# zsc/ARTalk

Hardware: AMD Instinct MI355X
Metric: motion frames/sec (25 fps clips) at batch=32 per GPU (higher is better)
Workload: dtype f32 (operands split into 2 fp16, 3 fp16 MFMA products per fp32 product, fp32 accumulate)

## Files before the change

### artalk_amd/capi.py

```python
from __future__ import annotations

import ctypes as C
import os

from .config import ARTalkConfig

_HERE = os.path.dirname(os.path.abspath(__file__))
LIB_PATH = os.environ.get("ARTALK_LIB") or os.path.join(_HERE, "libartalk_hip.so")

OK, EINVAL, EKEY, EMISSING, EHIP, ESTATE, ECAPACITY, EBUSY = 0, -1, -2, -3, -4, -5, -6, -7
DTYPE_F32, DTYPE_I64 = 0, 1

SYMBOLS = [
    "artalk_create", "artalk_destroy", "artalk_last_error", "artalk_set_tensor", "artalk_finalize_weights",
    "artalk_reserve", "artalk_workspace_bytes", "artalk_weight_bytes", "artalk_infer", "artalk_get_status", "artalk_poll_status", "artalk_last_ticket", "artalk_get_status_of", "artalk_style_encode", "artalk_stream_begin", "artalk_stream_chunk", "artalk_stream_end", "artalk_savgol", "artalk_flame_create", "artalk_flame_verts", "artalk_flame_destroy", "artalk_flame_last_error",
    "artalk_set_profiling", "artalk_get_profile", "artalk_get_kernel_sums", "artalk_set_graphs", "artalk_graph_count", "artalk_set_cu_mask", "artalk_set_audit", "artalk_get_audit", "artalk_calibrate", "artalk_reset_scales", "artalk_get_scales", "artalk_scale_sites", "artalk_get_site_scales", "artalk_set_site_scales", "artalk_set_tap", "artalk_tap_layout", "artalk_set_precision",
    "artalk_op_gemm", "artalk_op_gemm_ex", "artalk_op_gemm_bf16", "artalk_op_gemm_f16s", "artalk_op_pack_split", "artalk_op_gemm_f16s_packed", "artalk_op_release_scratch", "artalk_op_gemm_p8_plan", "artalk_op_create_masked_stream", "artalk_op_destroy_stream", "artalk_op_mfma_f32_peak", "artalk_op_layernorm", "artalk_op_attention", "artalk_op_w2v_front", "artalk_op_resample_mean", "artalk_op_pool_silu",
    "artalk_op_bsq_history",
    "artalk_sessions_reserve", "artalk_session_open", "artalk_session_step", "artalk_session_close", "artalk_session_count",
    "artalk_session_smooth", "artalk_op_savgol_stream", "artalk_op_session_smooth_check",
    "artalk_op_pack_split_ex", "artalk_op_layernorm_ex", "artalk_op_gemm_f16s_packed_ex", "artalk_op_gemm_f16s_ex", "artalk_op_attention_ex", "artalk_op_w2v_front_ex", "artalk_op_pool_silu_ex", "artalk_op_posconv_p8_ex",
    "artalk_op_bsq_history_ex", "artalk_op_ar_bits_next", "artalk_op_vq_embed", "artalk_op_ar_begin", "artalk_op_dec_input", "artalk_op_dec_finish", "artalk_op_enc_input_zero", "artalk_op_style_input", "artalk_op_add_row", "artalk_op_style_finish", "artalk_op_broadcast16", "artalk_op_session_gather", "artalk_op_session_scatter", "artalk_op_absmax",
    "artalk_op_gemm_rows", "artalk_op_layernorm_rows", "artalk_op_attention_rows", "artalk_op_gemm_rows_layout", "artalk_op_rows_dry_run",
    "artalk_op_w2v_front_rows", "artalk_op_pool_silu_rows", "artalk_op_posconv_rows",
    "artalk_op_attention_plan", "artalk_op_attention_rows_cus",
    "artalk_infer_samples", "artalk_set_tail_skip", "artalk_conv_tail_geometry", "artalk_conv_tail_class",
]

(ATTN_F32_64, ATTN_F32_32, ATTN_SHORT, ATTN_F16, ATTN_F16_P8, ATTN_F16_WIDE, ATTN_F16_PP, ATTN_F16_WIDE_AR,
 ATTN_F16_WIDE_AR_P8) = range(9)
ATTN_KERNELS = {
    ATTN_F32_64: "attention_kernel<64>", ATTN_F32_32: "attention_kernel<32>", ATTN_SHORT: "attention_short_kernel",
    ATTN_F16: "attention_f16_kernel<1>", ATTN_F16_P8: "attention_f16_kernel<1,1>", ATTN_F16_WIDE: "attention_f16_wide_kernel",
    ATTN_F16_PP: "attention_f16_pp_kernel", ATTN_F16_WIDE_AR: "attention_f16_wide_ar_kernel<1>",
    ATTN_F16_WIDE_AR_P8: "attention_f16_wide_ar_kernel<1,1,7,128>",
}


class ArtalkConfigStruct(C.Structure):
    _fields_ = [
        ("ar_depth", C.c_int32), ("ar_heads", C.c_int32),
        ("vae_depth", C.c_int32), ("vae_heads", C.c_int32), ("vae_hidden", C.c_int32),
        ("code_dim", C.c_int32), ("motion_dim", C.c_int32),
        ("n_levels", C.c_int32), ("patch_nums", C.c_int32 * 8),
        ("w2v_layers", C.c_int32), ("w2v_hidden", C.c_int32), ("w2v_heads", C.c_int32), ("w2v_ffn", C.c_int32),
        ("w2v_n_conv", C.c_int32), ("w2v_conv_kernel", C.c_int32 * 8), ("w2v_conv_stride", C.c_int32 * 8),
        ("w2v_conv_dim", C.c_int32),
        ("w2v_pos_kernel", C.c_int32), ("w2v_pos_groups", C.c_int32),
        ("w2v_ln_eps", C.c_float),
        ("style_dim", C.c_int32), ("style_heads", C.c_int32), ("style_layers", C.c_int32), ("style_ffn", C.c_int32),
        ("style_len", C.c_int32),
    ]


ROWMAP_IDENTITY = (2 ** 31 - 1, 0, 0)


class GemmRowsArgs(C.Structure):
    _fields_ = [
        ("mode", C.c_int32), ("M", C.c_int32), ("N", C.c_int32), ("K", C.c_int32), ("act", C.c_int32),
        ("A", C.c_void_p), ("lda", C.c_int64), ("a_elems", C.c_int64), ("a_exp", C.c_int32),
        ("W", C.c_void_p), ("ldw", C.c_int64), ("w_elems", C.c_int64),
        ("bias", C.c_void_p), ("bias_elems", C.c_int64),
        ("C", C.c_void_p), ("ldc", C.c_int64), ("c_elems", C.c_int64), ("cmap", C.c_int32 * 3),
        ("gate", C.c_void_p), ("ldg", C.c_int64), ("gate_elems", C.c_int64), ("gmap", C.c_int32 * 3),
        ("R", C.c_void_p), ("ldr", C.c_int64), ("r_elems", C.c_int64),
        ("c_p8", C.c_int32), ("c_exp", C.c_int32),
        ("force_cfg", C.c_int32), ("splitk", C.c_int32),
        ("ngrp", C.c_int32), ("grpW", C.c_int64), ("grpB", C.c_int64), ("grpC", C.c_int64),
        ("status_dev", C.c_void_p),
        ("ln_Y", C.c_void_p), ("ln_ldy", C.c_int64), ("ln_y_elems", C.c_int64),
        ("ln_scale", C.c_void_p), ("ln_shift", C.c_void_p), ("ln_ldm", C.c_int64), ("ln_mod_elems", C.c_int64), ("ln_mmap", C.c_int32 * 3),
        ("ln_eps", C.c_float), ("ln_out_p8", C.c_int32), ("ln_p8_exp", C.c_int32),
        ("used_cfg", C.POINTER(C.c_int32)), ("used_splitk", C.POINTER(C.c_int32)), ("fused_ln", C.POINTER(C.c_int32)),
        ("cus", C.c_int32),
    ]

    def __init__(self, **kw):
        super().__init__()
        self.a_exp = self.c_exp = self.ln_p8_exp = 4
        self.force_cfg, self.splitk, self.ln_eps = -1, 1, 1e-6
        for name in ("cmap", "gmap", "ln_mmap"):
            setattr(self, name, (C.c_int32 * 3)(*ROWMAP_IDENTITY))
        for k, v in kw.items():
            setattr(self, k, (C.c_int32 * 3)(*v) if k in ("cmap", "gmap", "ln_mmap") else v)


def config_struct(cfg: ARTalkConfig) -> ArtalkConfigStruct:
    w = cfg.w2v
    if w.get("feat_extract_norm", "layer") != "layer" or not w.get("do_stable_layer_norm", True) or not w.get("conv_bias", True):
        raise ValueError("only the XLS-R style wav2vec2 (layer-norm conv stack, stable layer norm, conv bias) is supported")
    if len(set(w["conv_dim"])) != 1:
        raise ValueError("conv_dim must be uniform")
    s = ArtalkConfigStruct()
    s.ar_depth, s.ar_heads = cfg.ar_depth, cfg.ar_heads
    s.vae_depth, s.vae_heads, s.vae_hidden = cfg.vae_depth, cfg.vae_heads, cfg.vae_hidden
    s.code_dim, s.motion_dim = cfg.code_dim, cfg.motion_dim
    s.n_levels = len(cfg.patch_nums)
    for i, p in enumerate(cfg.patch_nums):
        s.patch_nums[i] = p
    s.w2v_layers, s.w2v_hidden = w["num_hidden_layers"], w["hidden_size"]
    s.w2v_heads, s.w2v_ffn = w["num_attention_heads"], w["intermediate_size"]
    s.w2v_n_conv = len(w["conv_kernel"])
    for i, (k, st) in enumerate(zip(w["conv_kernel"], w["conv_stride"])):
        s.w2v_conv_kernel[i], s.w2v_conv_stride[i] = k, st
    s.w2v_conv_dim = w["conv_dim"][0]
    s.w2v_pos_kernel, s.w2v_pos_groups = w["num_conv_pos_embeddings"], w["num_conv_pos_embedding_groups"]
    s.w2v_ln_eps = w["layer_norm_eps"]
    s.style_dim, s.style_heads, s.style_layers = cfg.style_dim, cfg.style_heads, cfg.style_layers
    s.style_ffn, s.style_len = cfg.style_ffn, cfg.style_len
    return s


_lib = None


def lib() -> C.CDLL:
    global _lib
    if _lib is not None:
        return _lib
    if not os.path.exists(LIB_PATH):
        raise RuntimeError(
            f"{LIB_PATH} is missing: the HIP extension has not been built "
            "(run `python -c 'import __graft_entry__ as g; g.build()'`). There is no CPU fallback.")
    L = C.CDLL(LIB_PATH)
    vp, i32, i64, f32 = C.c_void_p, C.c_int, C.c_int64, C.c_float
    L.artalk_create.argtypes = [i32, C.POINTER(ArtalkConfigStruct), C.POINTER(vp)]
    L.artalk_create.restype = i32
    L.artalk_destroy.argtypes = [vp]
    L.artalk_destroy.restype = None
    L.artalk_last_error.argtypes = [vp]
    L.artalk_last_error.restype = C.c_char_p
    L.artalk_set_tensor.argtypes = [vp, C.c_char_p, vp, i32, i32, C.POINTER(i64)]
    L.artalk_set_tensor.restype = i32
    L.artalk_finalize_weights.argtypes = [vp]
    L.artalk_finalize_weights.restype = i32
    L.artalk_reserve.argtypes = [vp, i32, i32]
    L.artalk_reserve.restype = i32
    L.artalk_workspace_bytes.argtypes = [vp]
    L.artalk_workspace_bytes.restype = i64
    L.artalk_weight_bytes.argtypes = [vp]
    L.artalk_weight_bytes.restype = i64
    L.artalk_infer.argtypes = [vp, vp, i64, C.POINTER(i64), i32, vp, vp, vp, i64, vp, vp, vp, vp]
    L.artalk_infer.restype = i32
    if hasattr(L, "artalk_infer_samples"):
        L.artalk_infer_samples.argtypes = [vp, vp, i64, C.POINTER(i64), C.POINTER(i64), i32, vp, vp, vp, i64, vp, vp, vp, vp]
        L.artalk_infer_samples.restype = i32
        L.artalk_set_tail_skip.argtypes = [vp, i32]
        L.artalk_set_tail_skip.restype = i32
        pi = C.POINTER(i32)
        L.artalk_conv_tail_geometry.argtypes = [i64, i32, i32, pi, pi, pi, pi, pi, pi]
        L.artalk_conv_tail_geometry.restype = i32
        L.artalk_conv_tail_class.argtypes = [i64, i32]
        L.artalk_conv_tail_class.restype = i64
    L.artalk_get_status.argtypes = [vp, C.POINTER(C.c_int), vp]
    L.artalk_get_status.restype = i32
    L.artalk_poll_status.argtypes = [vp, C.POINTER(C.c_int)]
    L.artalk_poll_status.restype = i32
    L.artalk_last_ticket.argtypes = [vp]
    L.artalk_last_ticket.restype = C.c_longlong
    L.artalk_get_status_of.argtypes = [vp, C.c_longlong, C.POINTER(C.c_int)]
    L.artalk_get_status_of.restype = i32
    L.artalk_style_encode.argtypes = [vp, vp, i32, vp, vp]
    L.artalk_style_encode.restype = i32
    L.artalk_stream_begin.argtypes = [vp, i32, vp, vp, vp]
    L.artalk_stream_begin.restype = i32
    L.artalk_stream_end.argtypes = [vp]
    L.artalk_stream_end.restype = i32
    L.artalk_stream_chunk.argtypes = [vp, vp, i64, vp, i64, vp]
    L.artalk_stream_chunk.restype = i32
    if hasattr(L, "artalk_session_open"):
        L.artalk_sessions_reserve.argtypes = [vp, i32]
        L.artalk_sessions_reserve.restype = i32
        L.artalk_session_open.argtypes = [vp, i32, vp, vp, C.POINTER(i64), vp]
        L.artalk_session_open.restype = i32
        L.artalk_session_step.argtypes = [vp, C.POINTER(i64), i32, vp, i64, vp, i64, vp, vp, vp]
        L.artalk_session_step.restype = i32
        L.artalk_session_close.argtypes = [vp, C.POINTER(i64), i32]
        L.artalk_session_close.restype = i32
        L.artalk_session_count.argtypes = [vp]
        L.artalk_session_count.restype = i32
    if hasattr(L, "artalk_session_smooth"):
        pi32, pu8 = C.POINTER(i32), C.POINTER(C.c_uint8)
        L.artalk_session_smooth.argtypes = [vp, C.POINTER(i64), i32, vp, i64, pi32, pu8, vp, i64, pi32, pi32, vp]
        L.artalk_session_smooth.restype = i32
        L.artalk_op_savgol_stream.argtypes = [vp, vp, i64, pi32, pi32, pu8, vp, i64, i32, vp]
        L.artalk_op_savgol_stream.restype = i32
        L.artalk_op_session_smooth_check.argtypes = [C.POINTER(i64), C.POINTER(i64), pu8, i32, C.POINTER(i64), i32, C.POINTER(i64), i32, i32, i64,
                                                     pi32, pu8, i64, pi32, pi32, C.c_char_p, i32]
        L.artalk_op_session_smooth_check.restype = i32
    L.artalk_flame_create.argtypes = [i32, i32, i32, i32, vp, vp, vp, vp, vp, vp, f32, C.POINTER(vp)]
    L.artalk_flame_create.restype = i32
    L.artalk_flame_verts.argtypes = [vp, vp, vp, i32, vp, vp]
    L.artalk_flame_verts.restype = i32
    L.artalk_flame_destroy.argtypes = [vp]
    L.artalk_flame_destroy.restype = None
    L.artalk_flame_last_error.argtypes = [vp]
    L.artalk_flame_last_error.restype = C.c_char_p
    L.artalk_savgol.argtypes = [vp, vp, vp, i32, vp]
    L.artalk_savgol.restype = i32
    L.artalk_set_profiling.argtypes = [vp, i32]
    L.artalk_set_profiling.restype = i32
    L.artalk_get_profile.argtypes = [vp, C.POINTER(C.c_double), i32]
    L.artalk_get_profile.restype = i32
    if hasattr(L, "artalk_get_kernel_sums"):
        L.artalk_get_kernel_sums.argtypes = [vp, C.POINTER(C.c_double), i32]
        L.artalk_get_kernel_sums.restype = i32
    L.artalk_set_graphs.argtypes = [vp, i32]
    L.artalk_set_graphs.restype = i32
    if hasattr(L, "artalk_graph_count"):
        L.artalk_graph_count.argtypes = [vp, C.POINTER(C.c_longlong)]
        L.artalk_graph_count.restype = i32
    if hasattr(L, "artalk_set_audit"):
        L.artalk_set_audit.argtypes = [vp, i32]
        L.artalk_set_audit.restype = i32
        L.artalk_get_audit.argtypes = [vp, C.c_char_p, i32, C.POINTER(C.c_float), i32]
        L.artalk_get_audit.restype = i32
    if hasattr(L, "artalk_calibrate"):
        L.artalk_calibrate.argtypes = [vp, f32]
        L.artalk_calibrate.restype = i32
        L.artalk_reset_scales.argtypes = [vp]
        L.artalk_reset_scales.restype = i32
        L.artalk_get_scales.argtypes = [vp, C.POINTER(C.c_int), i32]
        L.artalk_get_scales.restype = i32
    if hasattr(L, "artalk_set_site_scales"):
        L.artalk_scale_sites.argtypes = [vp, C.c_char_p, i32]
        L.artalk_scale_sites.restype = i32
        L.artalk_get_site_scales.argtypes = [vp, C.POINTER(C.c_int), i32]
        L.artalk_get_site_scales.restype = i32
        L.artalk_set_site_scales.argtypes = [vp, C.POINTER(C.c_int), i32]
        L.artalk_set_site_scales.restype = i32
    L.artalk_op_gemm.argtypes = [vp, i64, vp, vp, vp, vp, vp, i32, i32, i32, i32, vp]
    L.artalk_op_gemm.restype = i32
    L.artalk_set_precision.argtypes = [vp, i32]
    L.artalk_set_precision.restype = i32
    if hasattr(L, "artalk_op_gemm_bf16"):
        L.artalk_op_gemm_bf16.argtypes = [vp, i64, vp, vp, vp, vp, vp, i32, i32, i32, i32, i32, vp]
        L.artalk_op_gemm_bf16.restype = i32
    L.artalk_op_gemm_f16s.argtypes = [vp, i64, vp, vp, vp, i32, i32, i32, i32, i32, vp]
    L.artalk_op_gemm_f16s.restype = i32
    L.artalk_op_pack_split.argtypes = [vp, vp, i64, i32, vp]
    L.artalk_op_pack_split.restype = i32
    L.artalk_op_gemm_f16s_packed.argtypes = [vp, i32, i64, vp, vp, vp, i32, i32, i32, i32, i32, vp]
    L.artalk_op_gemm_f16s_packed.restype = i32
    if hasattr(L, "artalk_set_tap"):
        L.artalk_set_tap.argtypes = [vp, vp, i32, i32]
        L.artalk_set_tap.restype = i32
        L.artalk_tap_layout.argtypes = [C.POINTER(C.c_int64), i32]
        L.artalk_tap_layout.restype = i32
        L.artalk_op_release_scratch.argtypes = []
        L.artalk_op_release_scratch.restype = i32
    L.artalk_set_cu_mask.argtypes = [vp, vp, i32]
    L.artalk_set_cu_mask.restype = i32
    L.artalk_op_create_masked_stream.argtypes = [vp, i32, C.POINTER(vp)]
    L.artalk_op_create_masked_stream.restype = i32
    L.artalk_op_destroy_stream.argtypes = [vp]
    L.artalk_op_destroy_stream.restype = i32
    L.artalk_op_gemm_p8_plan.argtypes = [i32, i32, i32, i32]
    L.artalk_op_gemm_p8_plan.restype = i32
    L.artalk_op_gemm_ex.argtypes = [vp, i64, vp, vp, vp, i32, i32, i32, i32, i32, vp]
    L.artalk_op_gemm_ex.restype = i32
    L.artalk_op_mfma_f32_peak.argtypes = [vp, i32, i32, i32, C.POINTER(C.c_double), vp]
    L.artalk_op_mfma_f32_peak.restype = i32
    L.artalk_op_layernorm.argtypes = [vp, vp, vp, vp, vp, vp, i32, i32, f32, i32, vp]
    L.artalk_op_layernorm.restype = i32
    L.artalk_op_attention.argtypes = [vp, vp, vp, vp, i32, i32, i32, i32, i32, f32, i32, vp, i32, vp]
    L.artalk_op_attention.restype = i32
    L.artalk_op_w2v_front.argtypes = [vp, i32, i32, vp, vp, vp, vp, vp, vp, vp]
    L.artalk_op_w2v_front.restype = i32
    L.artalk_op_resample_mean.argtypes = [vp, i32, i32, vp, i32, i32, i32, vp, i32, vp]
    L.artalk_op_resample_mean.restype = i32
    L.artalk_op_pool_silu.argtypes = [vp, i32, i32, i32, vp, vp]
    L.artalk_op_pool_silu.restype = i32
    L.artalk_op_bsq_history.argtypes = [vp, vp, vp, vp, i32, vp]
    L.artalk_op_bsq_history.restype = i32
    if hasattr(L, "artalk_op_pack_split_ex"):
        L.artalk_op_pack_split_ex.argtypes = [vp, vp, i64, i32, i32, vp, vp]
        L.artalk_op_pack_split_ex.restype = i32
        L.artalk_op_layernorm_ex.argtypes = [vp, vp, vp, vp, vp, vp, i32, i32, f32, i32, i32, i32, i32, vp, vp]
        L.artalk_op_layernorm_ex.restype = i32
        L.artalk_op_gemm_f16s_packed_ex.argtypes = [vp, i32, i64, vp, vp, vp, i32, i32, i32, i32, i32, i32, i32, vp, vp, vp]
        L.artalk_op_gemm_f16s_packed_ex.restype = i32
        L.artalk_op_gemm_f16s_ex.argtypes = [vp, i64, vp, vp, vp, i32, i32, i32, i32, i32, i32, vp, vp]
        L.artalk_op_gemm_f16s_ex.restype = i32
        L.artalk_op_attention_ex.argtypes = [vp, vp, vp, vp, i32, i32, i32, i32, i32, f32, i32, vp, i32, i32, i32, i32, vp, vp]
        L.artalk_op_attention_ex.restype = i32
        L.artalk_op_w2v_front_ex.argtypes = [vp, i32, i32, vp, vp, vp, vp, vp, vp, i32, i32, vp, vp]
        L.artalk_op_w2v_front_ex.restype = i32
        L.artalk_op_pool_silu_ex.argtypes = [vp, i32, i32, i32, vp, i32, i32, vp, vp]
        L.artalk_op_pool_silu_ex.restype = i32
        L.artalk_op_posconv_p8_ex.argtypes = [vp, vp, vp, vp, vp, i32, i32, i32, i32, i32, vp, vp]
        L.artalk_op_posconv_p8_ex.restype = i32
    if hasattr(L, "artalk_op_ar_bits_next"):
        for name, args in (
                ("bsq_history_ex", [vp, vp, vp, vp, i32, vp, vp]),
                ("ar_bits_next", [vp, vp, vp, vp, i32, i32, vp, vp]),
                ("vq_embed", [vp, i32, vp, vp, vp, vp, i32, i32, vp, vp, i32, vp]),
                ("ar_begin", [vp, vp, vp, vp, i32, vp]),
                ("dec_input", [vp, vp, vp, vp, vp, i32, vp]),
                ("dec_finish", [vp, vp, vp, vp, vp, i64, i32, vp, i32, vp, vp]),
                ("enc_input_zero", [vp, vp, vp, vp, i32, vp]),
                ("style_input", [vp, vp, vp, vp, i32, vp]),
                ("add_row", [vp, vp, i32, i32, vp]),
                ("style_finish", [vp, vp, vp, vp, vp, vp, i32, vp, i64, vp]),
                ("broadcast16", [vp, vp, i64, i32, vp]),
                ("session_gather", [vp, vp, vp, vp, i32, i32, i32, i32, vp]),
                ("session_scatter", [vp, vp, vp, vp, i32, i32, i32, i32, i32, vp]),
# ... 60 lines not shown
```

### artalk_amd/csrc/ar_glue.hip

```cpp
#include "common.h"
#include <cmath>
#include <mutex>
#include <set>

namespace artalk {

constexpr int T100 = 100;
constexpr int CD = 32;
constexpr int NLV = 5;
__constant__ int c_pn[NLV];
__constant__ int c_off[NLV + 1];
__constant__ int c_up_i0[4][T100];
__constant__ int c_up_i1[4][T100];
__constant__ float c_up_w1[4][T100];
__constant__ float c_hq;

static const int h_pn[NLV] = {1, 5, 25, 50, 100};

int init_ms_tables() {
    static std::mutex mu;
    static std::set<int> ready;
    int dev = -1;
    if (hipGetDevice(&dev) != hipSuccess) return -1;
    std::lock_guard<std::mutex> lock(mu);
// ... 38 lines not shown
}

__global__ __launch_bounds__(256) void absmax_kernel(const float* __restrict__ buf, int rows, int cols, long ld, int is_p8,
                                                     unsigned int* __restrict__ slot, int junk_period, int junk_from, float inv_scale) {
    float m = 0.f;
    const long groups = (long)rows * (cols / 8);
    for (long i = (long)blockIdx.x * 256 + threadIdx.x; i < groups; i += (long)gridDim.x * 256) {
        const long r = i / (cols / 8), g8 = i - r * (cols / 8);
        if (junk_period && r % junk_period >= junk_from) continue;
        const float* p = buf + r * ld + g8 * 8;
        if (is_p8) {
            const _Float16* h = reinterpret_cast<const _Float16*>(p);
#pragma unroll
            for (int e = 0; e < 8; ++e) {
                const float v = fabsf((float)h[e]) * inv_scale;
                m = (v != v) ? INFINITY : fmaxf(m, v);
            }
        } else {
#pragma unroll
            for (int e = 0; e < 8; ++e) {
                const float v = fabsf(p[e]);
                m = (v != v) ? INFINITY : fmaxf(m, v);
            }
        }
    }
    m = wave_max(m);
    if ((threadIdx.x & 63) == 0) atomicMax(slot, __float_as_uint(m));
}
void launch_absmax(const float* buf, int rows, int cols, long ld, int is_p8, unsigned int* slot, hipStream_t s, int junk_period, int junk_from, int p8_exp) {
    if (rows <= 0 || cols < 8) return;
    const long groups = (long)rows * (cols / 8);
    const long blocks = (groups + 255) / 256;
    ARTALK_LAUNCH(absmax_kernel, dim3((unsigned)(blocks < 1024 ? blocks : 1024)), dim3(256), 0, s, buf, rows, cols, ld, is_p8, slot, junk_period,
                       junk_from, p8_scale_of(-p8_exp));
}

__global__ __launch_bounds__(256) void ar_begin_kernel(const float* __restrict__ style_cond, const float* __restrict__ lvlpos,
                                                       float* __restrict__ x0, float* __restrict__ fhat, int E) {
    const int b = blockIdx.x;
    for (int n = threadIdx.x; n < E; n += 256) x0[(long)b * E + n] = style_cond[(long)b * E + n] + lvlpos[n];
    for (int i = threadIdx.x; i < T100 * CD; i += 256) fhat[(long)b * T100 * CD + i] = 0.f;
}
void launch_ar_begin(const float* style_cond, const float* lvlpos, float* x0, float* fhat, int B, hipStream_t s) {
    ARTALK_LAUNCH(ar_begin_kernel, dim3(B), dim3(256), 0, s, style_cond, lvlpos, x0, fhat, 768);
}

constexpr int BITS_NT = 1024;
__global__ __launch_bounds__(BITS_NT) void ar_bits_kernel(const float* __restrict__ logits, uint8_t* __restrict__ bits,
                                                      float* __restrict__ fhat, float* __restrict__ nextfeat, int p, int* __restrict__ status) {
    __shared__ float hs[T100 * CD];
    __shared__ float fs[T100 * CD];
    const int b = blockIdx.x, tid = threadIdx.x;
    const int pn = c_pn[p], off = c_off[p];
    for (int idx = tid; idx < pn * CD; idx += BITS_NT) {
        const int i = idx / CD, c = idx % CD;
        const float* l = logits + ((long)b * pn + i) * (2 * CD) + 2 * c;
        const int bit = l[1] > l[0];
        if (status && !(isfinite(l[0]) && isfinite(l[1]))) atomicOr(status, 1);
        bits[((long)b * 181 + off + i) * CD + c] = (uint8_t)bit;
        hs[idx] = bit ? c_hq : -c_hq;
    }
    if (p >= NLV - 1) return;
    __syncthreads();
    float* fg = fhat + (long)b * T100 * CD;
    for (int idx = tid; idx < T100 * CD; idx += BITS_NT) {
        const int t = idx / CD, c = idx % CD;
        const float v = fg[idx] + up_lin(hs, p, t, c);
        fg[idx] = v;
        fs[idx] = v;
    }
    __syncthreads();
    const int pn2 = c_pn[p + 1];
    for (int idx = tid; idx < pn2 * CD; idx += BITS_NT)
        nextfeat[(long)b * pn2 * CD + idx] = area_pool(fs, pn2, idx / CD, idx % CD);
}
void launch_ar_bits_next(const float* logits, uint8_t* bits, float* fhat, float* nextfeat, int B, int level, hipStream_t s, int* status) {
    ARTALK_LAUNCH(ar_bits_kernel, dim3(B), dim3(BITS_NT), 0, s, logits, bits, fhat, nextfeat, level, status);
}

constexpr int VQ_TOK = 16;
__global__ __launch_bounds__(256) void vq_embed_kernel(const float* __restrict__ feat, int n, const float* __restrict__ We,
                                                       const float* __restrict__ be, const float* __restrict__ pos,
                                                       float* __restrict__ X, int xrows, int xoff,
                                                       const float* __restrict__ style_cond, const float* __restrict__ pos0, int E) {
    __shared__ float f[VQ_TOK][CD];
    const int i0 = blockIdx.x * VQ_TOK, b = blockIdx.y, tid = threadIdx.x;
    if (blockIdx.x == 0 && style_cond) {
        for (int e = tid; e < E; e += 256) X[((long)b * xrows) * E + e] = style_cond[(long)b * E + e] + pos0[e];
    }
    const int nt = min(VQ_TOK, n - i0);
    for (int idx = tid; idx < VQ_TOK * CD; idx += 256) f[idx / CD][idx % CD] = idx < nt * CD ? feat[((long)b * n + i0) * CD + idx] : 0.f;
    constexpr int EPT = 3;
    float w[EPT][CD], bias[EPT], pv[EPT][VQ_TOK];
#pragma unroll
    for (int k = 0; k < EPT; ++k) {
        const int e = tid + k * 256;
        const bool ok = e < E;
#pragma unroll
        for (int c4 = 0; c4 < CD / 4; ++c4) {
            f32x4 t = {0.f, 0.f, 0.f, 0.f};
            if (ok) t = *reinterpret_cast<const f32x4*>(We + (long)e * CD + 4 * c4);
            w[k][4 * c4] = t[0]; w[k][4 * c4 + 1] = t[1]; w[k][4 * c4 + 2] = t[2]; w[k][4 * c4 + 3] = t[3];
        }
        bias[k] = ok ? be[e] : 0.f;
#pragma unroll
        for (int t = 0; t < VQ_TOK; ++t) pv[k][t] = (ok && t < nt) ? pos[(long)(i0 + t) * E + e] : 0.f;
    }
    __syncthreads();
#pragma unroll
    for (int k = 0; k < EPT; ++k) {
        const int e = tid + k * 256;
        if (e >= E) break;
#pragma unroll
        for (int t0 = 0; t0 < VQ_TOK; t0 += 4) {
            float acc[4] = {0.f, 0.f, 0.f, 0.f};
#pragma unroll
            for (int c = 0; c < CD; ++c)
#pragma unroll
                for (int u = 0; u < 4; ++u) acc[u] = fmaf(w[k][c], f[t0 + u][c], acc[u]);
#pragma unroll
            for (int u = 0; u < 4; ++u)
                if (t0 + u < nt) X[((long)b * xrows + xoff + i0 + t0 + u) * E + e] = (acc[u] + bias[k]) + pv[k][t0 + u];
        }
    }
}
void launch_vq_embed(const float* feat, int n, const float* We, const float* be, const float* pos, float* X, int xrows,
                     int xoff, const float* style_cond, const float* pos0, int B, hipStream_t s) {
    ARTALK_LAUNCH(vq_embed_kernel, dim3((n + VQ_TOK - 1) / VQ_TOK, B), dim3(256), 0, s, feat, n, We, be, pos, X, xrows, xoff,
                       style_cond, pos0, 768);
}

__global__ __launch_bounds__(256) void dec_input_kernel(const float* __restrict__ prev_fdec, const float* __restrict__ fhat,
                                                        const uint8_t* __restrict__ bits, const float* __restrict__ dpos,
                                                        float* __restrict__ X) {
    const int b = blockIdx.x;
    for (int idx = blockIdx.y * 256 + threadIdx.x; idx < 2 * T100 * CD; idx += gridDim.y * 256) {
        const int t = idx / CD, c = idx % CD;
        float v;
        if (t < T100) {
            v = prev_fdec[(long)b * T100 * CD + idx];
        } else {
            const int tt = t - T100;
            const float h = bits[((long)b * 181 + 81 + tt) * CD + c] ? c_hq : -c_hq;
            v = fhat[(long)b * T100 * CD + tt * CD + c] + h;
        }
        X[(long)b * 2 * T100 * CD + idx] = v + dpos[idx];
    }
}
void launch_dec_input(const float* prev_fdec, const float* fhat, const uint8_t* bits, const float* dpos, float* X, int B,
                      hipStream_t s) {
    ARTALK_LAUNCH(dec_input_kernel, dim3(B, 8), dim3(256), 0, s, prev_fdec, fhat, bits, dpos, X);
}

__global__ __launch_bounds__(256) void dec_finish_kernel(const float* __restrict__ dec, const float* __restrict__ mean,
                                                         const float* __restrict__ stdv, const float* __restrict__ epos,
                                                         float* __restrict__ out, long out_bstride, int chunk,
                                                         float* __restrict__ E, int MD, int EK, int* __restrict__ status) {
    const int b = blockIdx.x;
    for (int idx = blockIdx.y * 256 + threadIdx.x; idx < T100 * EK; idx += gridDim.y * 256) {
        const int t = idx / EK, j = idx % EK;
        float e = 0.f;
        if (j < MD) {
            const float d = dec[((long)b * 2 * T100 + T100 + t) * MD + j];
            const float m = d * stdv[j] + mean[j];
            if (status && !isfinite(m)) atomicOr(status, 4);
            out[(long)b * out_bstride + ((long)chunk * T100 + t) * MD + j] = m;
            e = (m - mean[j]) / stdv[j] + epos[t * MD + j];
        }
        E[((long)b * T100 + t) * EK + j] = e;
    }
}
void launch_dec_finish(const float* dec, const float* mean, const float* stdv, const float* epos, float* out,
                       long out_bstride, int chunk, float* E, int B, hipStream_t s, int* status) {
    ARTALK_LAUNCH(dec_finish_kernel, dim3(B, 10), dim3(256), 0, s, dec, mean, stdv, epos, out, out_bstride, chunk, E, 106, 128, status);
}

__global__ __launch_bounds__(256) void enc_input_zero_kernel(const float* __restrict__ mean, const float* __restrict__ stdv,
                                                             const float* __restrict__ epos, float* __restrict__ E, int MD, int EK) {
    const int b = blockIdx.x;
    for (int idx = threadIdx.x; idx < T100 * EK; idx += 256) {
        const int t = idx / EK, j = idx % EK;
        E[((long)b * T100 + t) * EK + j] = (j < MD) ? ((0.f - mean[j]) / stdv[j] + epos[t * MD + j]) : 0.f;
    }
}
__global__ __launch_bounds__(256) void broadcast16_kernel(const uint4* __restrict__ src, uint4* __restrict__ dst, int n16) {
    uint4* d = dst + (long)blockIdx.y * n16;
    for (int i = blockIdx.x * 256 + threadIdx.x; i < n16; i += gridDim.x * 256) d[i] = src[i];
}
void launch_broadcast16(const void* src, void* dst, long bytes, int B, hipStream_t s) {
    if (B <= 0 || bytes <= 0) return;
    const int n16 = (int)(bytes / 16);
    ARTALK_LAUNCH(broadcast16_kernel, dim3((n16 + 255) / 256 < 8 ? (n16 + 255) / 256 : 8, B), dim3(256), 0, s,
                       reinterpret_cast<const uint4*>(src), reinterpret_cast<uint4*>(dst), n16);
}

void launch_enc_input_zero(const float* mean, const float* stdv, const float* epos, float* E, int B, hipStream_t s) {
    ARTALK_LAUNCH(enc_input_zero_kernel, dim3(B), dim3(256), 0, s, mean, stdv, epos, E, 106, 128);
}

__global__ __launch_bounds__(256) void session_gather_kernel(const uint4* const* __restrict__ slots, SessionRows w) {
    const uint4* __restrict__ src = slots[blockIdx.y];
    const long row = blockIdx.y;
    const int p0 = w.s16, f0 = w.s16 + w.p16, n16 = f0 + w.f16;
    for (int i = blockIdx.x * 256 + threadIdx.x; i < n16; i += gridDim.x * 256) {
        const uint4 v = src[i];
        if (i < p0) w.style[row * w.s16 + i] = v;
        else if (i < f0) w.prev_in[row * w.p16 + (i - p0)] = v;
        else w.prev_fdec[row * w.f16 + (i - f0)] = v;
    }
}
__global__ __launch_bounds__(256) void session_scatter_kernel(uint4* const* __restrict__ slots, SessionRows w, int with_style) {
    uint4* __restrict__ dst = slots[blockIdx.y];
    const long row = blockIdx.y;
    const int p0 = w.s16, f0 = w.s16 + w.p16, n16 = f0 + w.f16;
    for (int i = (with_style ? 0 : p0) + blockIdx.x * 256 + threadIdx.x; i < n16; i += gridDim.x * 256) {
        uint4 v;
        if (i < p0) v = w.style[row * w.s16 + i];
        else if (i < f0) v = w.prev_in[row * w.p16 + (i - p0)];
        else v = w.prev_fdec[row * w.f16 + (i - f0)];
        dst[i] = v;
    }
}
static inline unsigned session_pieces(const SessionRows& w) { return (unsigned)((w.s16 + w.p16 + w.f16 + 1023) / 1024); }
void launch_session_gather(const float* const* slots, const SessionRows& w, int n, hipStream_t s) {
    if (n <= 0) return;
    ARTALK_LAUNCH(session_gather_kernel, dim3(session_pieces(w), n), dim3(256), 0, s, reinterpret_cast<const uint4* const*>(slots), w);
}
void launch_session_scatter(float* const* slots, const SessionRows& w, int n, bool with_style, hipStream_t s) {
    if (n <= 0) return;
    ARTALK_LAUNCH(session_scatter_kernel, dim3(session_pieces(w), n), dim3(256), 0, s, reinterpret_cast<uint4* const*>(slots), w,
                  with_style ? 1 : 0);
}

constexpr int BSQ_NT = 1024;
__global__ __launch_bounds__(BSQ_NT) void bsq_history_kernel(const float* __restrict__ enc_out, uint8_t* __restrict__ hist_bits,
                                                          float* __restrict__ prev_fdec, float* __restrict__ msfeat, int* __restrict__ status) {
    __shared__ float resid[T100 * CD];
    __shared__ float fms[T100 * CD];
    __shared__ float qs[T100 * CD];
    __shared__ float hs[T100 * CD];
    const int b = blockIdx.x, tid = threadIdx.x;
    for (int idx = tid; idx < T100 * CD; idx += BSQ_NT) {
        resid[idx] = enc_out[(long)b * T100 * CD + idx];
        if (status && !isfinite(resid[idx])) atomicOr(status, 2);
        fms[idx] = 0.f;
    }
    __syncthreads();
    int msoff = 0;
    for (int p = 0; p < NLV; ++p) {
        const int pn = c_pn[p], off = c_off[p];
        for (int base = 0; base < pn * CD; base += BSQ_NT) {
            const int idx = base + tid;
            const bool ok = idx < pn * CD;
            const int i = ok ? idx / CD : 0, c = idx % CD;
            float x = 0.f;
            if (ok) x = (pn == T100) ? resid[idx] : area_pool(resid, pn, i, c);
            float ss = x * x;
            ss = group_sum<32>(ss);
            const float z = x / fmaxf(sqrtf(ss), 1e-12f);
            const float zhat = (z > 0.f) ? c_hq : -c_hq;
            const float q = z + (zhat - z);
            const int bit = q > 0.f;
            if (ok) {
                qs[idx] = q;
                hs[idx] = bit ? c_hq : -c_hq;
                hist_bits[((long)b * 181 + off + i) * CD + c] = (uint8_t)bit;
            }
        }
        __syncthreads();
        if (p < NLV - 1) {
            for (int idx = tid; idx < T100 * CD; idx += BSQ_NT) {
                const int t = idx / CD, c = idx % CD;
                resid[idx] -= up_lin(qs, p, t, c);
                fms[idx] += up_lin(hs, p, t, c);
            }
            __syncthreads();
            const int pn2 = c_pn[p + 1];
            for (int idx = tid; idx < pn2 * CD; idx += BSQ_NT)
                msfeat[((long)b * 180 + msoff) * CD + idx] = area_pool(fms, pn2, idx / CD, idx % CD);
            msoff += pn2;
        } else {
            for (int idx = tid; idx < T100 * CD; idx += BSQ_NT) prev_fdec[(long)b * T100 * CD + idx] = fms[idx] + hs[idx];
        }
        __syncthreads();
    }
}
void launch_bsq_history(const float* enc_out, uint8_t* hist_bits, float* prev_fdec, float* msfeat, int B, hipStream_t s, int* status) {
    ARTALK_LAUNCH(bsq_history_kernel, dim3(B), dim3(BSQ_NT), 0, s, enc_out, hist_bits, prev_fdec, msfeat, status);
}

__global__ __launch_bounds__(256) void style_input_kernel(const float* __restrict__ motion, const float* __restrict__ mean,
                                                          const float* __restrict__ stdv, float* __restrict__ X, int rows, int MD, int EK) {
    const long n = (long)rows * EK;
    for (long idx = (long)blockIdx.x * 256 + threadIdx.x; idx < n; idx += (long)gridDim.x * 256) {
        const long row = idx / EK; const int j = idx % EK;
        X[idx] = (j < MD) ? (motion[row * MD + j] - mean[j]) / stdv[j] : 0.f;
    }
}
void launch_style_input(const float* motion, const float* mean, const float* stdv, float* X, int B, hipStream_t s) {
    const int rows = B * 50;
    ARTALK_LAUNCH(style_input_kernel, dim3((rows * 128 + 255) / 256), dim3(256), 0, s, motion, mean, stdv, X, rows, 106, 128);
}

__global__ __launch_bounds__(256) void add_row_kernel(float* __restrict__ X, const float* __restrict__ v, long n, int D) {
    for (long idx = (long)blockIdx.x * 256 + threadIdx.x; idx < n; idx += (long)gridDim.x * 256) X[idx] += v[idx % D];
}
// ... 145 lines not shown
```

### artalk_amd/csrc/engine.hip

```cpp
#include "kernels.h"
#include "../../include/artalk_hip.h"

#include <hip/hip_ext.h>
#include <rocprofiler-sdk-roctx/roctx.h>

#include <algorithm>
#include <cmath>
#include <cstdio>
#include <cstdlib>
#include <cstring>
#include <map>
#include <set>
#include <string>
#include <vector>

using namespace artalk;

namespace artalk {
thread_local KernelTimer* g_ktimer = nullptr;
bool ktimer_events(hipEvent_t* e0, hipEvent_t* e1) {
    KernelTimer* t = g_ktimer;
    if (!t) return false;
    while (t->pool.size() < t->used + 2) {
        hipEvent_t e = nullptr;
        if (hipEventCreate(&e) != hipSuccess) return false;
        t->pool.push_back(e);
    }
    *e0 = t->pool[t->used]; *e1 = t->pool[t->used + 1];
    t->recs.emplace_back(t->bucket, t->used);
    t->used += 2;
    return true;
}
}

namespace {
enum { KB_STYLE = 0, KB_CONV = 1, KB_ENC = 2, KB_ADA = 3, KB_AR_MISC = 4, KB_LEVEL0 = 5, KB_VAE_DEC = 10, KB_REENC = 11, KB_OTHER = 12, KB_N = 13 };

thread_local std::string g_create_error;

constexpr int kSamplesPerChunk = 64000;
constexpr int kE = 768;
constexpr int kCond = 1024;
constexpr int kNTok = 181;
constexpr int kMaxLv = 5;

struct Range {
    explicit Range(const char* name) { roctxRangePushA(name); }
    ~Range() { roctxRangePop(); }
    Range(const Range&) = delete;
    Range& operator=(const Range&) = delete;
};

enum SlotKind { SK_DIRECT, SK_PADK, SK_CONV, SK_HOST, SK_IGNORE };

struct Slot {
    std::vector<int64_t> shape;
    int dtype = ARTALK_DTYPE_F32;
    SlotKind kind = SK_DIRECT;
    float* dst = nullptr;
    int64_t pad_to = 0;
    bool set = false;
    std::vector<float> host;
    std::vector<int64_t> host_i64;
    int64_t numel() const { int64_t n = 1; for (auto d : shape) n *= d; return n; }
};

struct W2VLayer { float *qkv_w, *qkv_b, *out_w, *out_b, *ln1w, *ln1b, *ln2w, *ln2b, *ff1_w, *ff1_b, *ff2_w, *ff2_b; };
struct ARLayer { float *qkv_w, *qkv_b, *proj_w, *proj_b, *ffn1_w, *ffn1_b, *ffn2_w, *ffn2_b, *qscale; };
struct VAELayer { float *lnw, *lnb, *qkv_w, *out_w, *out_b, *m1_w, *m1_b, *m2_w, *m2_b; };
struct VAESide { float *in_w, *in_b, *out_w, *out_b; std::vector<VAELayer> layers; };
struct StyleLayer { float *in_w, *in_b, *out_w, *out_b, *l1_w, *l1_b, *l2_w, *l2_b, *n1w, *n1b, *n2w, *n2b; };

struct SiteExps {
    int conv[8]; int fp_ln, posconv_in;
    struct W2V { int ln1, qkv, attn, ln2, ffn; } w2v[64];
    int silu_cond, hist_tok;
    struct AR { int ln1, attn, ln2, ffn; } ar[32];
    struct VAE { int ln, qkv, attn, resid, mlp; } vae[2][16];
    int vae_enc_in, vae_dec_in, vae_dec_head;
    int style_in; struct ST { int h, attn, h1, ffn; } style[8];
    SiteExps() { int* p = reinterpret_cast<int*>(this); for (size_t i = 0; i < sizeof(SiteExps) / sizeof(int); ++i) p[i] = kActExp; }
};

struct Workspace {
    int maxB = 0, maxC = 0, G = 0;
    long* src_off = nullptr; float *xnorm = nullptr, *convA = nullptr, *convB = nullptr;
    float *h0 = nullptr, *h1 = nullptr, *xln = nullptr, *qkv = nullptr, *att = nullptr, *ffn = nullptr;
    float* silu_cond = nullptr;
    float *ada = nullptr, *style_cond = nullptr, *prev_in = nullptr, *prev_in_p8 = nullptr, *cache = nullptr;
    float *x = nullptr, *xmod = nullptr, *attn_out = nullptr, *ffn_h = nullptr, *logits = nullptr;
    float *fhat = nullptr, *nextfeat = nullptr;
    float* splitk = nullptr; int64_t splitk_floats = 0;
    float* splitk_b[4] = {nullptr, nullptr, nullptr, nullptr};
    uint8_t *bits = nullptr, *hist_bits = nullptr, *has_style = nullptr;
    int* status = nullptr;
    float** sess_slots = nullptr;
    float *prev_fdec = nullptr, *msfeat = nullptr, *dec_x = nullptr, *vh = nullptr, *vln = nullptr, *vqkv = nullptr;
    float *vatt = nullptr, *vmlp = nullptr, *dec_out = nullptr, *enc_in = nullptr, *enc_out = nullptr, *motion_chunk = nullptr;
    float *s_in = nullptr, *s_h = nullptr, *s_qkv = nullptr, *s_att = nullptr, *s_ffn = nullptr, *s_tmp = nullptr;
    int64_t bytes = 0;
};

}

constexpr int64_t slot_carry_off(int code_dim) { return kE + (int64_t)kNTok * kE + 100LL * code_dim; }
constexpr int kOpCodeDim = 32, kOpMotionDim = 106;

struct artalk_model {
    artalk_config cfg{};
    int device = 0;
    std::string err;
    bool finalized = false;
    std::map<std::string, Slot> slots;
    std::vector<void*> allocs;
    std::vector<void*> ws_allocs;
    int64_t weight_bytes = 0;
    struct PackRange { const float* base; int64_t n; unsigned int* packed; uint16_t* bf16; };
    std::vector<PackRange> wranges;
    int precision = 0;
    bool have_bf16 = false;
    int splitk_tiles = 192, splitk_target = 384;
    bool audit = false;
    unsigned int* audit_vals = nullptr;
    std::vector<std::string> audit_names;
    std::map<std::string, int> audit_index;
    std::vector<int*> audit_exp;
    SiteExps ex;
    int scales_changed = 0;
    struct Site { std::string name; int* ex; };
    std::vector<Site> sites;
    std::map<const int*, int> site_of;
    bool stream_scales_ended = false;
    struct InitHistory { uint8_t* bits = nullptr; float *fdec = nullptr, *msfeat = nullptr; bool valid = false; } init_hist[3];
    void invalidate_init_hist() { for (auto& ih : init_hist) ih.valid = false; }
    float* tap = nullptr; int tap_B = 0, tap_maxch = 0, tap_chunk = 0;
    std::vector<uint32_t> cu_mask;
    int n_cus = 0;
    int stream_B = 0;
    static constexpr int kSessBlock = 32;
    struct Sessions {
        std::vector<float*> blocks;
        std::vector<int64_t> owner;
        struct Open { int slot = 0; int64_t seen = 0; bool smooth_done = false; };
        std::map<int64_t, Open> open;
        std::set<int64_t> ended_by_scales;
        int64_t next_id = 1;
        void* smooth_tab = nullptr; int64_t smooth_cap = 0;
    } sess;
    int64_t sess_carry_off() const { return slot_carry_off(cfg.code_dim); }
    int64_t sess_slot_floats() const { return sess_carry_off() + (kSavgolCarry * (int64_t)cfg.motion_dim + 3) / 4 * 4; }
    float* sess_slot(int i) const { return sess.blocks[i / kSessBlock] + (int64_t)(i % kSessBlock) * sess_slot_floats(); }
    Workspace* view = nullptr;
    bool sticky_error = false;
    int n_conv = 0; int conv_T[8]{}; int conv_S[8]{};
    int Tw = 0, Ts = 0;
    struct TailGeo { bool partial = false; int tc = 0; int T[8]{}, S[8]{}; } tail_geo[4];
    bool tail_skip = true;
    int ada_n = 0;
    int pn[kMaxLv]{}, off[kMaxLv + 1]{};
    float *conv0_w = nullptr, *conv_b[8]{}, *conv_lnw[8]{}, *conv_lnb[8]{}, *conv_w[8]{};
    float *fp_lnw = nullptr, *fp_lnb = nullptr, *fp_w = nullptr, *fp_b = nullptr;
    float *pos_w = nullptr, *pos_b = nullptr, *enc_lnw = nullptr, *enc_lnb = nullptr;
    std::vector<W2VLayer> w2v;
    float *ada_w = nullptr, *ada_b = nullptr;
    float *ar_qkv_w = nullptr, *ar_qkv_b = nullptr;
    std::vector<ARLayer> ar;
    float *logits_w = nullptr, *logits_b = nullptr, *vq_w = nullptr, *vq_b = nullptr, *sc_w = nullptr, *sc_b = nullptr;
    float *null_style = nullptr, *lvl_pos = nullptr, *prev_lvl_pos = nullptr;
    float *enc_pos = nullptr, *dec_pos = nullptr, *vae_mean = nullptr, *vae_std = nullptr;
    VAESide enc, dec;
    float *st_mean = nullptr, *st_std = nullptr, *st_pe = nullptr, *st_proj_w = nullptr, *st_proj_b = nullptr;
    std::vector<StyleLayer> style;
    Workspace ws;
    int profiling = 0;
    KernelTimer ktimer;
    bool use_graphs = true;
    bool in_graph_body = false;
    bool in_body = false;
    std::vector<hipEvent_t> ev_pool; size_t ev_used = 0;
    std::vector<std::pair<size_t, double>> dom_events;
    std::vector<std::pair<int, size_t>> marks;
    hipStream_t prof_stream = nullptr;
    hipStream_t side_stream[3] = {nullptr, nullptr, nullptr};
    hipEvent_t fork_ev = nullptr, join_ev[3] = {nullptr, nullptr, nullptr};
    int branches = 0;
    hipStream_t own_stream = nullptr;
    struct GraphEntry { hipGraphExec_t exec = nullptr; long long last_use = 0; };
    std::map<long long, GraphEntry> graphs;
    long long graph_clock = 0, graph_captures = 0;
    static constexpr int kStageSlots = 4;
    struct Stage { long* src = nullptr; uint8_t* has = nullptr; float** slots = nullptr; int4* smooth = nullptr; hipEvent_t done = nullptr; bool used = false; };
    Stage stage[kStageSlots];
    int stage_cap_c = 0, stage_cap_b = 0, stage_next = 0;
    static constexpr int kStatusSlots = 4;
    int* h_status = nullptr; hipEvent_t status_ev[kStatusSlots] = {nullptr, nullptr, nullptr, nullptr}; bool status_pending = false;
    long long ticket = 0;
};

namespace {

#define HIPCHK(m, call)                                                                         \
    do {                                                                                        \
        hipError_t e_ = (call);                                                                 \
        if (e_ != hipSuccess) {                                                                 \
            (m)->err = std::string(#call) + ": " + hipGetErrorString(e_);                       \
            return ARTALK_EHIP;                                                                 \
        }                                                                                       \
    } while (0)

int fail(artalk_model* m, int code, const std::string& msg) { m->err = msg; return code; }
struct ProfilingOff {
    artalk_model* m; int saved;
    explicit ProfilingOff(artalk_model* x) : m(x), saved(x->profiling) { m->profiling = 0; }
    ~ProfilingOff() { m->profiling = saved; }
    ProfilingOff(const ProfilingOff&) = delete;
    ProfilingOff& operator=(const ProfilingOff&) = delete;
};

template <typename T>
T* dalloc_in(std::vector<void*>& pool, int64_t n) {
    void* p = nullptr;
    if (n <= 0) n = 1;
    if (hipMalloc(&p, n * sizeof(T)) != hipSuccess) { pool.push_back(nullptr); return nullptr; }
    (void)hipMemset(p, 0, n * sizeof(T));
    pool.push_back(p);
    return reinterpret_cast<T*>(p);
}
template <typename T>
T* dalloc(artalk_model* m, int64_t n) { return dalloc_in<T>(m->allocs, n); }

float* walloc(artalk_model* m, int64_t n) {
    m->weight_bytes += n * 4;
    float* p = dalloc<float>(m, n);
    m->wranges.push_back({p, n, nullptr, nullptr});
    return p;
}

const unsigned int* packed_of(const artalk_model* m, const float* w) {
    for (const auto& r : m->wranges)
        if (r.packed && w >= r.base && w < r.base + r.n) return r.packed + (w - r.base);
    return nullptr;
}

const void* bf16_of(const artalk_model* m, const float* w) {
    for (const auto& r : m->wranges)
        if (r.bf16 && w >= r.base && w < r.base + r.n) return r.bf16 + (w - r.base);
    return nullptr;
}

int ensure_bf16_copy(artalk_model* m) {
    if (m->have_bf16) return ARTALK_OK;
    int64_t total = 0;
    for (const auto& r : m->wranges) total += (r.n + 63) / 64 * 64;
    uint16_t* base = dalloc<uint16_t>(m, total);
    if (!base) return fail(m, ARTALK_EHIP, "hipMalloc failed for the bf16 weight copy");
    HIPCHK(m, hipDeviceSynchronize());
    int64_t off = 0;
    for (auto& r : m->wranges) {
        r.bf16 = base + off;
        launch_pack_bf16(r.base, r.bf16, r.n, nullptr);
        off += (r.n + 63) / 64 * 64;
    }
    HIPCHK(m, hipDeviceSynchronize());
    for (const auto& r : m->wranges) m->weight_bytes += r.n * 2;
    m->have_bf16 = true;
    return ARTALK_OK;
}

void add_slot(artalk_model* m, const std::string& key, std::vector<int64_t> shape, SlotKind kind, float* dst,
              int64_t pad_to = 0, int dtype = ARTALK_DTYPE_F32) {
    Slot s;
    s.shape = std::move(shape); s.kind = kind; s.dst = dst; s.pad_to = pad_to; s.dtype = dtype;
    m->slots[key] = std::move(s);
}

void add_linear(artalk_model* m, const std::string& p, int out_f, int in_f, float*& w, float*& b, bool bias = true) {
    w = walloc(m, (int64_t)out_f * in_f);
    add_slot(m, p + ".weight", {out_f, in_f}, SK_DIRECT, w);
    if (bias) { b = walloc(m, out_f); add_slot(m, p + ".bias", {out_f}, SK_DIRECT, b); } else b = nullptr;
}
void add_vec(artalk_model* m, const std::string& key, int n, float*& v) {
    v = walloc(m, n);
    add_slot(m, key, {n}, SK_DIRECT, v);
}
void add_ln(artalk_model* m, const std::string& p, int n, float*& w, float*& b) {
    add_vec(m, p + ".weight", n, w);
    add_vec(m, p + ".bias", n, b);
// ... 239 lines not shown
    launch_layernorm(a, s);
}

struct ConvPasses { int np = 0; int off[4]{}, n[4]{}, cls[4]{}; const long* perm = nullptr; const long* tab = nullptr; };

void run_wav2vec(artalk_model* m, const float* audio, int c0, int n, float* out_w2v, hipStream_t s, const ConvPasses* tail = nullptr) {
    const artalk_config& c = m->cfg;
    Workspace& w = m->ws;
    const int CD = c.w2v_conv_dim, Hs = c.w2v_hidden;
    const int p8 = m->precision == 1 ? 1 : 0;
    const int AP = p8 ? LF_A_P8 : 0;
    Range r_w2v("artalk.wav2vec2");
    roctxRangePushA("artalk.wav2vec2.conv_stack");
    kbucket(m, KB_CONV);
    launch_audio_normalize(audio, tail ? tail->perm : w.src_off + c0, w.xnorm, n, kSamplesPerChunk, s);
    SiteExps& ex = m->ex;
    ConvPasses one;
    one.np = 1; one.n[0] = n; one.cls[0] = 3;
    const ConvPasses& ps = tail ? *tail : one;
    auto geo_T = [&](int p) { const artalk_model::TailGeo& tg = m->tail_geo[ps.cls[p]]; return ps.cls[p] != 3 && tg.partial ? tg.T : m->conv_T; };
    auto geo_S = [&](int p) { const artalk_model::TailGeo& tg = m->tail_geo[ps.cls[p]]; return ps.cls[p] != 3 && tg.partial ? tg.S : m->conv_S; };
    auto row0 = [&](int p, int i) { long r = 0; for (int q = 0; q < p; ++q) r += (long)ps.n[q] * geo_S(q)[i]; return r; };
    float* src = w.convA; float* dst = w.convB;
    for (int p = 0; p < ps.np; ++p) {
        const int *T = geo_T(p), *S = geo_S(p);
        float* y = src + row0(p, 0) * CD;
        launch_conv0(w.xnorm + (long)ps.off[p] * kSamplesPerChunk, kSamplesPerChunk, m->conv0_w, m->conv_b[0], m->conv_lnw[0], m->conv_lnb[0], y, ps.n[p],
                     T[0], S[0], s, p8, w.status, ex.conv[0]);
        audit(m, y, ps.n[p] * S[0], CD, CD, p8, s, &ex.conv[0], S[0], T[0]);
    }
    for (int i = 1; i < c.w2v_n_conv; ++i) {
        const int M = (int)row0(ps.np, i), plan_M = M == n * m->conv_S[i] ? 0 : n * m->conv_S[i];
        linear(m, src, (long)c.w2v_conv_stride[i] * CD, m->conv_w[i], m->conv_b[i], dst, CD, M, CD, c.w2v_conv_kernel[i] * CD,
               ACT_NONE, nullptr, s, AP, nullptr, ex.conv[i - 1], kActExp, plan_M);
        for (int p = 0; p < ps.np; p += 2) {
            const int *T = geo_T(p), *S = geo_S(p);
            float* y = dst + row0(p, i) * CD;
            const int Mp = ps.n[p] * S[i], Mq = p + 1 < ps.np ? ps.n[p + 1] * geo_S(p + 1)[i] : 0;
            LnArgs a;
            a.plan_M = plan_M;
            a.out_p8 = (p8 && i + 1 < c.w2v_n_conv) ? 1 : 0; a.p8_exp = ex.conv[i]; a.status = a.out_p8 ? w.status : nullptr;
            a.junk_period = S[i]; a.junk_from = T[i];
            if (Mq) { a.junk_row2 = Mp; a.junk_period2 = geo_S(p + 1)[i]; a.junk_from2 = geo_T(p + 1)[i]; }
            a.X = y; a.ldx = CD; a.Y = y; a.ldy = CD; a.w = m->conv_lnw[i]; a.b = m->conv_lnb[i]; a.M = Mp + Mq; a.D = CD; a.eps = 1e-5f; a.act = ACT_GELU_ERF;
            launch_layernorm(a, s);
            if (i + 1 < c.w2v_n_conv) {
                audit(m, y, Mp, CD, CD, p8, s, &ex.conv[i], S[i], T[i]);
                if (Mq) audit(m, y + (long)Mp * CD, Mq, CD, CD, p8, s, &ex.conv[i], a.junk_period2, a.junk_from2);
            }
        }
        std::swap(src, dst);
    }
    if (tail) {
        launch_conv_tail_gather(src, tail->tab, dst, n, m->Tw, m->Ts, CD, s);
        std::swap(src, dst);
    }
    stage_mark(m, s, PB_CONV);
    roctxRangePop();
    Range r_enc("artalk.wav2vec2.encoder");
    kbucket(m, KB_ENC);
    const int M = n * m->Ts;
    const int JP = m->Ts, JF = m->Tw;
    layernorm(src, dst, m->fp_lnw, m->fp_lnb, M, CD, c.w2v_ln_eps, ACT_NONE, s, p8, w.status, JP, JF, ex.fp_ln);
    audit(m, dst, M, CD, CD, p8, s, &ex.fp_ln, JP, JF);
    linear(m, dst, CD, m->fp_w, m->fp_b, w.h0, Hs, M, Hs, CD, ACT_NONE, nullptr, s, AP, nullptr, ex.fp_ln);
    audit(m, w.h0, M, Hs, Hs, false, s, &ex.posconv_in, JP, JF);
    {
        const int cg = Hs / c.w2v_pos_groups;
        GemmArgs g;
        g.A = w.h0; g.lda = Hs; g.W = m->pos_w; g.ldw = (long)cg * c.w2v_pos_kernel; g.bias = m->pos_b; g.C = w.h1; g.ldc = Hs; g.R = w.h0; g.ldr = Hs;
        g.M = M; g.act = ACT_GELU_ERF; g.a_exp = ex.posconv_in;
        if (p8 && cg == 64 && c.w2v_pos_kernel == 128 && c.w2v_pos_groups == 16 && m->Ts <= 256) {
            g.N = Hs; g.K = cg * c.w2v_pos_kernel; g.Wp = packed_of(m, m->pos_w); g.status = w.status;
            launch_posconv_p8(g, n, m->Tw, m->Ts, s);
        } else {
            g.amode = 1; g.pc_T = m->Tw; g.pc_tstride = m->Ts; g.pc_pad = c.w2v_pos_kernel / 2; g.pc_cin = cg;
            g.N = cg; g.K = cg * c.w2v_pos_kernel;
            g.batch = c.w2v_pos_groups; g.sA = cg; g.sW = (long)cg * cg * c.w2v_pos_kernel; g.sBias = cg; g.sC = cg; g.sR = cg;
            gemm(m, g, s);
        }
    }
    float* h = w.h1;
    const int nh = c.w2v_heads, hd = Hs / nh;
    for (int i = 0; i < c.w2v_layers; ++i) {
        const W2VLayer& L = m->w2v[i];
        SiteExps::W2V& E = ex.w2v[i];
        layernorm(h, w.xln, L.ln1w, L.ln1b, M, Hs, c.w2v_ln_eps, ACT_NONE, s, p8, w.status, JP, JF, E.ln1);
        audit(m, w.xln, M, Hs, Hs, p8, s, &E.ln1, JP, JF);
        linear(m, w.xln, Hs, L.qkv_w, L.qkv_b, w.qkv, 3 * Hs, M, 3 * Hs, Hs, ACT_NONE, nullptr, s, AP | (p8 ? LF_C_P8 : 0), nullptr, E.ln1, E.qkv);
        AttnArgs a;
        a.qkv_p8 = p8; a.qkv_exp = E.qkv; a.o_exp = E.attn;
        a.Q = w.qkv; a.K = w.qkv + Hs; a.V = w.qkv + 2 * Hs;
        a.ldq = a.ldk = a.ldv = 3 * Hs; a.q_bstride = a.k_bstride = a.v_bstride = (long)m->Ts * 3 * Hs;
        a.O = w.att; a.ldo = Hs; a.o_bstride = (long)m->Ts * Hs;
        a.B = n; a.H = nh; a.HD = hd; a.Lq = m->Tw; a.Lk = m->Tw; a.scale = 1.0f / std::sqrt((float)hd);
        audit(m, w.qkv, M, 3 * Hs, 3 * Hs, p8, s, &E.qkv, JP, JF);
        a.out_p8 = p8; a.split16 = p8; a.status = p8 ? w.status : nullptr; a.cus = m->n_cus;
        launch_attention(a, s);
        audit(m, w.att, M, Hs, Hs, p8, s, &E.attn, JP, JF);
        linear(m, w.att, Hs, L.out_w, L.out_b, h, Hs, M, Hs, Hs, ACT_NONE, h, s, AP, nullptr, E.attn);
        layernorm(h, w.xln, L.ln2w, L.ln2b, M, Hs, c.w2v_ln_eps, ACT_NONE, s, p8, w.status, JP, JF, E.ln2);
        audit(m, w.xln, M, Hs, Hs, p8, s, &E.ln2, JP, JF);
        linear(m, w.xln, Hs, L.ff1_w, L.ff1_b, w.ffn, c.w2v_ffn, M, c.w2v_ffn, Hs, ACT_GELU_ERF, nullptr, s, AP | (p8 ? LF_C_P8 : 0), nullptr, E.ln2, E.ffn);
        audit(m, w.ffn, M, c.w2v_ffn, c.w2v_ffn, p8, s, &E.ffn, JP, JF);
        linear(m, w.ffn, c.w2v_ffn, L.ff2_w, L.ff2_b, h, Hs, M, Hs, c.w2v_ffn, ACT_NONE, h, s, AP, nullptr, E.ffn);
    }
    layernorm(h, w.xln, m->enc_lnw, m->enc_lnb, M, Hs, c.w2v_ln_eps, ACT_NONE, s);
    if (out_w2v)
        (void)hipMemcpy2DAsync(out_w2v + (long)c0 * m->Tw * Hs, (size_t)m->Tw * Hs * 4, w.xln, (size_t)m->Ts * Hs * 4,
                               (size_t)m->Tw * Hs * 4, n, hipMemcpyDeviceToDevice, s);
    launch_pool_silu(w.xln, m->Ts, m->Tw, w.silu_cond + (long)c0 * kNTok * kCond, n, m->pn, c.n_levels, kCond, s, p8, w.status, ex.silu_cond);
    audit(m, w.silu_cond + (long)c0 * kNTok * kCond, n * kNTok, kCond, kCond, p8, s, &ex.silu_cond);
    stage_mark(m, s, PB_ENC);
}

void run_style(artalk_model* m, const float* style_motion, int B, hipStream_t s, bool encode = true) {
    const artalk_config& c = m->cfg;
    Workspace& w = m->ws;
    const int S = c.style_dim, L = c.style_len, M = B * L;
    Range r_style("artalk.style_encoder");
    kbucket(m, KB_STYLE);
    if (style_motion && encode) {
        launch_style_input(style_motion, m->st_mean, m->st_std, w.s_in, B, s);
        SiteExps& ex = m->ex;
        audit(m, w.s_in, M, 128, 128, false, s, &ex.style_in);
        linear(m, w.s_in, 128, m->st_proj_w, m->st_proj_b, w.s_h, S, M, S, 128, ACT_NONE, nullptr, s, 0, nullptr, ex.style_in);
        launch_add_row(w.s_h, m->st_pe, M, S, s);
        for (int i = 0; i < c.style_layers; ++i) {
            const StyleLayer& Ly = m->style[i];
            SiteExps::ST& E = ex.style[i];
            audit(m, w.s_h, M, S, S, false, s, &E.h);
            linear(m, w.s_h, S, Ly.in_w, Ly.in_b, w.s_qkv, 3 * S, M, 3 * S, S, ACT_NONE, nullptr, s, 0, nullptr, E.h);
            AttnArgs a;
            a.Q = w.s_qkv; a.K = w.s_qkv + S; a.V = w.s_qkv + 2 * S; a.ldq = a.ldk = a.ldv = 3 * S;
            a.q_bstride = a.k_bstride = a.v_bstride = (long)L * 3 * S;
            a.O = w.s_att; a.ldo = S; a.o_bstride = (long)L * S;
            a.B = B; a.H = c.style_heads; a.HD = S / c.style_heads; a.Lq = L; a.Lk = L;
            a.scale = 1.0f / std::sqrt((float)(S / c.style_heads));
            launch_attention(a, s);
            audit(m, w.s_att, M, S, S, false, s, &E.attn);
            linear(m, w.s_att, S, Ly.out_w, Ly.out_b, w.s_tmp, S, M, S, S, ACT_NONE, w.s_h, s, 0, nullptr, E.attn);
            layernorm(w.s_tmp, w.s_h, Ly.n1w, Ly.n1b, M, S, 1e-5f, ACT_NONE, s);
            audit(m, w.s_h, M, S, S, false, s, &E.h1);
            linear(m, w.s_h, S, Ly.l1_w, Ly.l1_b, w.s_ffn, c.style_ffn, M, c.style_ffn, S, ACT_GELU_ERF, nullptr, s, 0, nullptr, E.h1);
            audit(m, w.s_ffn, M, c.style_ffn, c.style_ffn, false, s, &E.ffn);
            linear(m, w.s_ffn, c.style_ffn, Ly.l2_w, Ly.l2_b, w.s_tmp, S, M, S, c.style_ffn, ACT_NONE, w.s_h, s, 0, nullptr, E.ffn);
            layernorm(w.s_tmp, w.s_h, Ly.n2w, Ly.n2b, M, S, 1e-5f, ACT_NONE, s);
        }
    }
    launch_style_finish(w.s_h, m->sc_w, m->sc_b, m->null_style, style_motion ? w.has_style : nullptr, w.style_cond, B, s,
                        style_motion, (long)L * c.motion_dim);
}

void run_vae_stack(artalk_model* m, const VAESide& S, int B, int T, int split, hipStream_t s) {
    const artalk_config& c = m->cfg;
    Workspace& w = m->view ? *m->view : m->ws;
    const int H = c.vae_hidden, M = B * T, F = H * 3 / 2;
    const int p8 = m->precision == 1 ? 1 : 0;
    const int AP = p8 ? LF_A_P8 : 0;
    const int sd = &S == &m->enc ? 0 : 1;
    for (int i = 0; i < c.vae_depth; ++i) {
        const VAELayer& L = S.layers[i];
        SiteExps::VAE& E = m->ex.vae[sd][i];
        layernorm(w.vh, w.vln, L.lnw, L.lnb, M, H, 1e-5f, ACT_NONE, s, p8, w.status, 0, 0, E.ln);
        audit(m, w.vln, M, H, H, p8, s, &E.ln);
        linear(m, w.vln, H, L.qkv_w, nullptr, w.vqkv, 3 * H, M, 3 * H, H, ACT_NONE, nullptr, s, AP | (p8 ? LF_C_P8 : 0), nullptr, E.ln, E.qkv);
        AttnArgs a;
        a.qkv_p8 = p8; a.qkv_exp = E.qkv; a.o_exp = E.attn;
        a.Q = w.vqkv; a.K = w.vqkv + H; a.V = w.vqkv + 2 * H; a.ldq = a.ldk = a.ldv = 3 * H;
        a.q_bstride = a.k_bstride = a.v_bstride = (long)T * 3 * H;
        a.O = w.vatt; a.ldo = H; a.o_bstride = (long)T * H;
        a.B = B; a.H = c.vae_heads; a.HD = H / c.vae_heads; a.Lq = T; a.Lk = T;
        a.scale = 1.0f / std::sqrt((float)H);
        audit(m, w.vqkv, M, 3 * H, 3 * H, p8, s, &E.qkv);
        a.split_q = split; a.split_k = split; a.out_p8 = p8; a.split16 = p8; a.status = p8 ? w.status : nullptr; a.cus = m->n_cus;
        launch_attention(a, s);
        audit(m, w.vatt, M, H, H, p8, s, &E.attn);
        linear(m, w.vatt, H, L.out_w, L.out_b, w.vh, H, M, H, H, ACT_NONE, w.vh, s, AP, p8 ? w.vln : nullptr, E.attn, E.resid);
        audit(m, p8 ? w.vln : w.vh, M, H, H, p8, s, &E.resid);
        linear(m, p8 ? w.vln : w.vh, H, L.m1_w, L.m1_b, w.vmlp, F, M, F, H, ACT_GELU_TANH, nullptr, s, p8 ? (LF_A_P8 | LF_C_P8) : 0, nullptr, E.resid, E.mlp);
        audit(m, w.vmlp, M, F, F, p8, s, &E.mlp);
        linear(m, w.vmlp, F, L.m2_w, L.m2_b, w.vh, H, M, H, F, ACT_NONE, w.vh, s, AP, nullptr, E.mlp);
    }
}

void run_reencode(artalk_model* m, int B, hipStream_t s) {
    const artalk_config& c = m->cfg;
    Workspace& w = m->view ? *m->view : m->ws;
    const int H = c.vae_hidden, T = 100;
    Range r_re("artalk.vae.reencode_bsq");
    kbucket(m, KB_REENC);
    audit(m, w.enc_in, B * T, 128, 128, false, s, &m->ex.vae_enc_in);
    linear(m, w.enc_in, 128, m->enc.in_w, m->enc.in_b, w.vh, H, B * T, H, 128, ACT_LEAKY02, nullptr, s, 0, nullptr, m->ex.vae_enc_in);
    run_vae_stack(m, m->enc, B, T, 0, s);
    linear(m, w.vh, H, m->enc.out_w, m->enc.out_b, w.enc_out, c.code_dim, B * T, c.code_dim, H, ACT_NONE, nullptr, s, LF_EXACT);
    launch_bsq_history(w.enc_out, w.hist_bits, w.prev_fdec, w.msfeat, B, s, w.status);
    launch_vq_embed(w.msfeat, kNTok - 1, m->vq_w, m->vq_b, m->prev_lvl_pos + kE, w.prev_in, kNTok, 1, w.style_cond,
                    m->prev_lvl_pos, B, s);
}

int run_init_history(artalk_model* m, int B, hipStream_t s) {
    const artalk_config& c = m->cfg;
    struct Restore { artalk_model* m; ~Restore() { kbucket(m, KB_OTHER); } } restore{m};
    Workspace& w = m->ws;
    artalk_model::InitHistory& ih = m->init_hist[m->precision];
    const long nb = (long)kNTok * c.code_dim, nf = 100L * c.code_dim * 4, nm = 180L * c.code_dim * 4;
    if (!ih.valid) {
        if (!ih.bits) {
            ih.bits = dalloc<uint8_t>(m, nb); ih.fdec = dalloc<float>(m, nf / 4); ih.msfeat = dalloc<float>(m, nm / 4);
            if (!ih.bits || !ih.fdec || !ih.msfeat) return fail(m, ARTALK_EHIP, "hipMalloc failed for the initial-history cache");
            HIPCHK(m, hipDeviceSynchronize());
        }
        launch_enc_input_zero(m->vae_mean, m->vae_std, m->enc_pos, w.enc_in, 1, s);
        run_reencode(m, 1, s);
        HIPCHK(m, hipMemcpyAsync(ih.bits, w.hist_bits, nb, hipMemcpyDeviceToDevice, s));
        HIPCHK(m, hipMemcpyAsync(ih.fdec, w.prev_fdec, nf, hipMemcpyDeviceToDevice, s));
        HIPCHK(m, hipMemcpyAsync(ih.msfeat, w.msfeat, nm, hipMemcpyDeviceToDevice, s));
        int flags[4] = {0, 0, 0, 0};
        HIPCHK(m, hipMemcpyAsync(flags, w.status, sizeof(int), hipMemcpyDeviceToHost, s));
        HIPCHK(m, hipStreamSynchronize(s));
        ih.valid = flags[0] == 0;
    }
    launch_broadcast16(ih.bits, w.hist_bits, nb, B, s);
    launch_broadcast16(ih.fdec, w.prev_fdec, nf, B, s);
    launch_broadcast16(ih.msfeat, w.msfeat, nm, B, s);
    launch_vq_embed(w.msfeat, kNTok - 1, m->vq_w, m->vq_b, m->prev_lvl_pos + kE, w.prev_in, kNTok, 1, w.style_cond, m->prev_lvl_pos, B, s);
    return ARTALK_OK;
}

void run_chunk_body(artalk_model* m, int B, hipStream_t s, int n_reencode = -1) {
    struct BodyScope { artalk_model* m; BodyScope(artalk_model* x) : m(x) { m->in_body = true; } ~BodyScope() { m->in_body = false; } } scope(m);
    const artalk_config& c = m->cfg;
    Workspace& w = m->view ? *m->view : m->ws;
    const long ldada = m->ada_n;
    const long cache_l = (long)w.maxB * 2 * kNTok * 3 * kE;
    const int p8 = m->precision == 1 ? 1 : 0;
    kbucket(m, KB_AR_MISC);
    tap_copy(m, TAP_PREV_IN, 0, w.prev_in, kNTok, kE, B, s);
    roctxRangePushA("artalk.ar.history_kv");
    SiteExps& ex = m->ex;
    if (p8) launch_pack_split(w.prev_in, reinterpret_cast<unsigned int*>(w.prev_in_p8), (long)B * kNTok * kE, false, s, w.status, ex.hist_tok);
    audit(m, p8 ? w.prev_in_p8 : w.prev_in, B * kNTok, kE, kE, p8, s, &ex.hist_tok);
    {
        GemmArgs g;
        g.A = p8 ? w.prev_in_p8 : w.prev_in; g.a_packed = p8; g.a_exp = ex.hist_tok;
        g.lda = kE; g.W = m->ar_qkv_w + (long)kE * kE; g.ldw = kE; g.bias = m->ar_qkv_b + kE;
        g.C = w.cache + kE; g.ldc = 3 * kE; g.cmap = rowmap(kNTok, 2 * kNTok, 0);
        g.M = B * kNTok; g.N = c.ar_depth * 2 * kE; g.K = kE;
        g.ngrp = 2 * kE; g.grpW = (long)3 * kE * kE; g.grpB = 3 * kE; g.grpC = cache_l;
        g.Wp = packed_of(m, g.W);
        if (p8 && gemm_p8_eligible(g)) {
            gemm(m, g, s);
        } else {
            for (int l = 0; l < c.ar_depth; ++l) {
                const ARLayer& L = m->ar[l];
                GemmArgs q = g;
                q.Wp = nullptr; q.ngrp = 0; q.grpW = q.grpB = q.grpC = 0;
                q.W = L.qkv_w + (long)kE * kE; q.bias = L.qkv_b + kE; q.C = w.cache + l * cache_l + kE; q.N = 2 * kE;
                gemm(m, q, s);
            }
        }
    }
    roctxRangePop();
    launch_ar_begin(w.style_cond, m->lvl_pos, w.x, w.fhat, B, s);
    static const char* const kLevelName[kMaxLv] = {"artalk.ar.scale_step0", "artalk.ar.scale_step1", "artalk.ar.scale_step2",
                                                   "artalk.ar.scale_step3", "artalk.ar.scale_step4"};
    for (int p = 0; p < c.n_levels; ++p) {
        Range r_lv(kLevelName[p]);
        kbucket(m, KB_LEVEL0 + p);
        const int pn = m->pn[p], off = m->off[p], M = B * pn;
        const RowMap amap = rowmap(pn, kNTok, off);
        auto ln_args = [&](int l, int which) {
            LnArgs n;
            n.X = w.x; n.ldx = kE; n.Y = w.xmod; n.ldy = kE; n.ldm = ldada; n.mmap = amap; n.M = M; n.D = kE; n.eps = 1e-6f;
            n.status = p8 ? w.status : nullptr;
            if (l < c.ar_depth) {
                const float* ada = w.ada + (long)l * 6 * kE;
                n.scale = ada + (2 + which) * kE; n.shift = ada + (4 + which) * kE; n.out_p8 = p8;
                n.p8_exp = which == 0 ? ex.ar[l].ln1 : ex.ar[l].ln2;
            } else {
                const float* hada = w.ada + (long)c.ar_depth * 6 * kE;
                n.scale = hada; n.shift = hada + kE; n.out_p8 = 0;
            }
            return n;
        };
        bool have_ln = false;
        for (int l = 0; l < c.ar_depth; ++l) {
            const ARLayer& L = m->ar[l];
            const float* ada = w.ada + (long)l * 6 * kE;
            float* cache = w.cache + l * cache_l;
            SiteExps::AR& E = ex.ar[l];
            if (l == 0) tap_copy(m, TAP_BLK0_IN, off, w.x, pn, kE, B, s);
            if (!have_ln) launch_layernorm(ln_args(l, 0), s);
            audit(m, w.xmod, M, kE, kE, p8, s, &E.ln1);
            GemmArgs q;
            q.A = w.xmod; q.lda = kE; q.W = L.qkv_w; q.ldw = kE; q.bias = L.qkv_b; q.C = cache; q.ldc = 3 * kE;
            q.cmap = rowmap(pn, 2 * kNTok, kNTok + off); q.M = M; q.N = 3 * kE; q.K = kE; q.a_packed = p8; q.a_exp = E.ln1;
            gemm(m, q, s);
            AttnArgs a;
            a.Q = cache + (long)(kNTok + off) * 3 * kE; a.K = cache + kE; a.V = cache + 2 * kE;
            a.ldq = a.ldk = a.ldv = 3 * kE; a.q_bstride = a.k_bstride = a.v_bstride = (long)2 * kNTok * 3 * kE;
            a.O = w.attn_out; a.ldo = kE; a.o_bstride = (long)pn * kE;
            a.B = B; a.H = c.ar_heads; a.HD = kE / c.ar_heads; a.Lq = pn; a.Lk = kNTok + off + pn; a.scale = 1.0f;
            a.l2norm = 1; a.qscale = L.qscale; a.out_p8 = p8; a.split16 = p8; a.status = p8 ? w.status : nullptr; a.o_exp = E.attn;
            launch_attention(a, s);
            audit(m, w.attn_out, M, kE, kE, p8, s, &E.attn);
            GemmArgs pj;
            pj.A = w.attn_out; pj.lda = kE; pj.W = L.proj_w; pj.ldw = kE; pj.bias = L.proj_b; pj.C = w.x; pj.ldc = kE;
            pj.gate = ada; pj.ldg = ldada; pj.gmap = amap; pj.R = w.x; pj.ldr = kE; pj.M = M; pj.N = kE; pj.K = kE; pj.a_packed = p8; pj.a_exp = E.attn;
            const LnArgs n2 = ln_args(l, 1);
            if (!gemm(m, pj, s, &n2)) launch_layernorm(n2, s);
            audit(m, w.xmod, M, kE, kE, p8, s, &E.ln2);
            linear(m, w.xmod, kE, L.ffn1_w, L.ffn1_b, w.ffn_h, 4 * kE, M, 4 * kE, kE, ACT_GELU_TANH, nullptr, s, p8 ? (LF_A_P8 | LF_C_P8) : 0, nullptr, E.ln2, E.ffn);
            audit(m, w.ffn_h, M, 4 * kE, 4 * kE, p8, s, &E.ffn);
            GemmArgs f2;
            f2.A = w.ffn_h; f2.lda = 4 * kE; f2.W = L.ffn2_w; f2.ldw = 4 * kE; f2.bias = L.ffn2_b; f2.C = w.x; f2.ldc = kE;
            f2.gate = ada + kE; f2.ldg = ldada; f2.gmap = amap; f2.R = w.x; f2.ldr = kE; f2.M = M; f2.N = kE; f2.K = 4 * kE; f2.a_packed = p8; f2.a_exp = E.ffn;
            const LnArgs nn = ln_args(l + 1, 0);
            have_ln = gemm(m, f2, s, &nn);
            if (l == 0) tap_copy(m, TAP_BLK0_OUT, off, w.x, pn, kE, B, s);
            if (l == c.ar_depth - 1) tap_copy(m, TAP_BLKL_OUT, off, w.x, pn, kE, B, s);
        }
        if (!have_ln) launch_layernorm(ln_args(c.ar_depth, 0), s);
        linear(m, w.xmod, kE, m->logits_w, m->logits_b, w.logits, 2 * c.code_dim, M, 2 * c.code_dim, kE, ACT_NONE, nullptr, s, LF_EXACT);
        tap_copy(m, TAP_LOGITS, off, w.logits, pn, 2 * c.code_dim, B, s);
        launch_ar_bits_next(w.logits, w.bits, w.fhat, w.nextfeat, B, p, s, w.status);
        if (p + 1 < c.n_levels)
            launch_vq_embed(w.nextfeat, m->pn[p + 1], m->vq_w, m->vq_b, m->lvl_pos + (long)m->off[p + 1] * kE, w.x, m->pn[p + 1], 0,
                            nullptr, nullptr, B, s);
    }
    stage_mark(m, s, PB_AR);
    const int H = c.vae_hidden;
    roctxRangePushA("artalk.vae.decode");
    kbucket(m, KB_VAE_DEC);
    launch_dec_input(w.prev_fdec, w.fhat, w.bits, m->dec_pos, w.dec_x, B, s);
    audit(m, w.dec_x, B * 200, c.code_dim, c.code_dim, false, s, &ex.vae_dec_in);
    linear(m, w.dec_x, c.code_dim, m->dec.in_w, m->dec.in_b, w.vh, H, B * 200, H, c.code_dim, ACT_LEAKY02, nullptr, s, 0, nullptr, ex.vae_dec_in);
    run_vae_stack(m, m->dec, B, 200, 100, s);
    audit(m, w.vh, B * 200, H, H, false, s, &ex.vae_dec_head);
    linear(m, w.vh, H, m->dec.out_w, m->dec.out_b, w.dec_out, c.motion_dim, B * 200, c.motion_dim, H, ACT_NONE, nullptr, s, 0, nullptr, ex.vae_dec_head);
    tap_copy(m, TAP_DEC_OUT, 0, w.dec_out, 200, c.motion_dim, B, s);
    launch_dec_finish(w.dec_out, m->vae_mean, m->vae_std, m->enc_pos, w.motion_chunk, 100L * c.motion_dim, 0, w.enc_in, B, s, w.status);
    roctxRangePop();
    if (n_reencode < 0 || n_reencode > B) n_reencode = B;
    if (n_reencode > 0) run_reencode(m, n_reencode, s);
    stage_mark(m, s, PB_VAE);
}

Workspace clip_view(const artalk_model* m, int b0, int branch) {
    const artalk_config& c = m->cfg;
    Workspace v = m->ws;
    const long b = b0;
    v.ada += b * kNTok * m->ada_n; v.style_cond += b * kE; v.prev_in += b * kNTok * kE; v.prev_in_p8 += b * kNTok * kE;
    v.cache += b * 2 * kNTok * 3 * kE;
    v.x += b * 100 * kE; v.xmod += b * 100 * kE; v.attn_out += b * 100 * kE; v.ffn_h += b * 100 * 4 * kE;
    v.logits += b * 100 * 2 * c.code_dim; v.fhat += b * 100 * c.code_dim; v.nextfeat += b * 100 * c.code_dim;
    v.bits += b * kNTok * c.code_dim; v.hist_bits += b * kNTok * c.code_dim;
    v.prev_fdec += b * 100 * c.code_dim; v.msfeat += b * 180 * c.code_dim; v.dec_x += b * 200 * c.code_dim;
    const long H = c.vae_hidden;
    v.vh += b * 200 * H; v.vln += b * 200 * H; v.vqkv += b * 200 * 3 * H; v.vatt += b * 200 * H; v.vmlp += b * 200 * H * 3 / 2;
    v.dec_out += b * 200 * c.motion_dim; v.enc_in += b * 100 * 128; v.enc_out += b * 100 * c.code_dim;
    v.motion_chunk += b * 100 * c.motion_dim;
    v.splitk = m->ws.splitk_b[branch];
    return v;
}

int ensure_side_streams(artalk_model* m, int n) {
    if (!m->fork_ev) HIPCHK(m, hipEventCreateWithFlags(&m->fork_ev, hipEventDisableTiming));
    for (int i = 0; i < n && i < 3; ++i) {
        if (m->side_stream[i]) continue;
        if (m->cu_mask.empty()) HIPCHK(m, hipStreamCreateWithFlags(&m->side_stream[i], hipStreamNonBlocking));
        else HIPCHK(m, hipExtStreamCreateWithCUMask(&m->side_stream[i], (uint32_t)m->cu_mask.size(), m->cu_mask.data()));
        HIPCHK(m, hipEventCreateWithFlags(&m->join_ev[i], hipEventDisableTiming));
    }
    return ARTALK_OK;
}
int body_branches(const artalk_model* m, int B) {
    const int want = m->branches > 0 ? m->branches : (B >= 8 ? 2 : 1);
    return B >= 2 * want ? want : (B >= 8 ? 2 : 1);
}
bool body_uses_graphs(const artalk_model* m) { return m->use_graphs && m->profiling < 2 && !m->audit && !m->tap; }
void drop_graphs(artalk_model* m) {
    for (auto& g : m->graphs) (void)hipGraphExecDestroy(g.second.exec);
    m->graphs.clear();
}
constexpr size_t kMaxGraphs = 96;
int evict_graphs(artalk_model* m, const long long* keep, int n_keep) {
    while (m->graphs.size() >= kMaxGraphs) {
        auto victim = m->graphs.end();
        for (auto it = m->graphs.begin(); it != m->graphs.end(); ++it) {
            bool pinned = false;
            for (int i = 0; i < n_keep; ++i) pinned |= it->first == keep[i];
            if (!pinned && (victim == m->graphs.end() || it->second.last_use < victim->second.last_use)) victim = it;
        }
        if (victim == m->graphs.end()) break;
        HIPCHK(m, hipDeviceSynchronize());
        (void)hipGraphExecDestroy(victim->second.exec);
        m->graphs.erase(victim);
    }
    return ARTALK_OK;
}
struct BodyGroups { bool graphs; int n; int b0[5]; int nre[4]; long long key[4]; };
BodyGroups plan_body(const artalk_model* m, int B, int n_next) {
    BodyGroups g;
    if (n_next < 0 || n_next > B) n_next = B;
    g.graphs = body_uses_graphs(m) && B <= 4095;
    const bool whole = m->audit || m->tap || m->profiling == 2 || (body_uses_graphs(m) && !g.graphs);
    g.n = whole ? 1 : body_branches(m, B);
    for (int h = 0; h <= g.n; ++h) g.b0[h] = (int)((long)B * h / g.n);
    for (int h = 0; h < g.n; ++h) {
        const int gsz = g.b0[h + 1] - g.b0[h];
        const int need = std::max(0, std::min(n_next - g.b0[h], gsz));
        g.nre[h] = g.graphs ? std::min(gsz, (need + 7) / 8 * 8) : need;
        g.key[h] = ((long long)(((B * 8 + g.n) * 4 + h) * 3 + m->precision)) * 4096 + g.nre[h];
    }
    return g;
}
int run_body(artalk_model* m, int B, hipStream_t s, int n_next) {
    const BodyGroups g = plan_body(m, B, n_next);
    const bool fork = g.n > 1 && m->profiling != 3;
    if (fork) { if (int rc = ensure_side_streams(m, g.n - 1)) return rc; }
    hipStream_t st[4] = {s, s, s, s};
    for (int h = 1; fork && h < g.n; ++h) st[h] = m->side_stream[h - 1];
    Workspace views[4];
    for (int h = 0; h < g.n; ++h) views[h] = clip_view(m, g.b0[h], h);
    auto launch_group = [&](int h) { m->view = &views[h]; run_chunk_body(m, g.b0[h + 1] - g.b0[h], st[h], g.nre[h]); m->view = nullptr; };
    for (int h = 0; g.graphs && h < g.n; ++h) {
        auto hit = m->graphs.find(g.key[h]);
        if (hit != m->graphs.end()) { hit->second.last_use = ++m->graph_clock; continue; }
        if (int rc = evict_graphs(m, g.key, g.n)) return rc;
        hipGraph_t graph = nullptr;
        hipGraphExec_t exec = nullptr;
        HIPCHK(m, hipStreamBeginCapture(st[h], hipStreamCaptureModeThreadLocal));
        m->in_graph_body = true;
        launch_group(h);
        m->in_graph_body = false;
        HIPCHK(m, hipStreamEndCapture(st[h], &graph));
        HIPCHK(m, hipGraphInstantiate(&exec, graph, nullptr, nullptr, 0));
        (void)hipGraphDestroy(graph);
        m->graphs.emplace(g.key[h], artalk_model::GraphEntry{exec, ++m->graph_clock});
        ++m->graph_captures;
    }
    if (fork) {
        HIPCHK(m, hipEventRecord(m->fork_ev, s));
        for (int h = 1; h < g.n; ++h) HIPCHK(m, hipStreamWaitEvent(st[h], m->fork_ev, 0));
    }
    for (int h = 0; h < g.n; ++h) {
        if (g.graphs) HIPCHK(m, hipGraphLaunch(m->graphs[g.key[h]].exec, st[h]));
        else launch_group(h);
    }
    for (int h = 1; fork && h < g.n; ++h) {
        HIPCHK(m, hipEventRecord(m->join_ev[h - 1], st[h]));
        HIPCHK(m, hipStreamWaitEvent(s, m->join_ev[h - 1], 0));
    }
    return ARTALK_OK;
}

void free_stage(artalk_model* m) {
    for (auto& st : m->stage) {
        if (st.src) (void)hipHostFree(st.src);
        if (st.has) (void)hipHostFree(st.has);
        if (st.slots) (void)hipHostFree(st.slots);
        if (st.smooth) (void)hipHostFree(st.smooth);
        st.src = nullptr; st.has = nullptr; st.slots = nullptr; st.smooth = nullptr; st.used = false;
    }
    m->stage_cap_c = m->stage_cap_b = 0;
}
int ensure_stage(artalk_model* m, int maxB, int maxC) {
    if (!m->h_status) {
        HIPCHK(m, hipHostMalloc(reinterpret_cast<void**>(&m->h_status), artalk_model::kStatusSlots * sizeof(int), hipHostMallocDefault));
        std::memset(m->h_status, 0, artalk_model::kStatusSlots * sizeof(int));
        for (auto& e : m->status_ev) HIPCHK(m, hipEventCreateWithFlags(&e, hipEventDisableTiming));
    }
    if (maxB <= m->stage_cap_b && maxC <= m->stage_cap_c) return ARTALK_OK;
    for (auto& st : m->stage) if (st.used) HIPCHK(m, hipEventSynchronize(st.done));
    free_stage(m);
    for (auto& st : m->stage) {
        HIPCHK(m, hipHostMalloc(reinterpret_cast<void**>(&st.src), (size_t)3 * maxC * sizeof(long), hipHostMallocDefault));
        HIPCHK(m, hipHostMalloc(reinterpret_cast<void**>(&st.has), (size_t)maxB, hipHostMallocDefault));
        HIPCHK(m, hipHostMalloc(reinterpret_cast<void**>(&st.slots), (size_t)maxB * sizeof(float*), hipHostMallocDefault));
        HIPCHK(m, hipHostMalloc(reinterpret_cast<void**>(&st.smooth), (size_t)maxB * sizeof(int4), hipHostMallocDefault));
        if (!st.done) HIPCHK(m, hipEventCreateWithFlags(&st.done, hipEventDisableTiming));
    }
    m->stage_cap_b = maxB; m->stage_cap_c = maxC;
    return ARTALK_OK;
}
int next_stage(artalk_model* m, artalk_model::Stage** out) {
    artalk_model::Stage& st = m->stage[m->stage_next];
    m->stage_next = (m->stage_next + 1) % artalk_model::kStageSlots;
    if (st.used) HIPCHK(m, hipEventSynchronize(st.done));
    *out = &st;
    return ARTALK_OK;
}
int publish_status(artalk_model* m, hipStream_t s) {
    const int slot = (int)(m->ticket % artalk_model::kStatusSlots);
    if (m->ticket >= artalk_model::kStatusSlots) HIPCHK(m, hipEventSynchronize(m->status_ev[slot]));
    HIPCHK(m, hipMemcpyAsync(m->h_status + slot, m->ws.status, sizeof(int), hipMemcpyDeviceToHost, s));
    HIPCHK(m, hipEventRecord(m->status_ev[slot], s));
    ++m->ticket;
    m->status_pending = true;
    HIPCHK(m, hipGetLastError());
    return ARTALK_OK;
}

int reserve(artalk_model* m, int maxB, int maxC) {
    const artalk_config& c = m->cfg;
    if (maxB <= m->ws.maxB && maxC <= m->ws.maxC) return ensure_stage(m, m->ws.maxB, m->ws.maxC);
    maxB = std::max(maxB, m->ws.maxB); maxC = std::max(maxC, m->ws.maxC);
    (void)hipDeviceSynchronize();
    drop_graphs(m);
    for (void* p : m->ws_allocs) if (p) (void)hipFree(p);
    m->ws_allocs.clear();
    m->ws = Workspace();
    m->stream_B = 0; m->stream_scales_ended = false;
    m->status_pending = false;
    Workspace& w = m->ws;
    const int CD = c.w2v_conv_dim, Hs = c.w2v_hidden;
    w.maxB = maxB; w.maxC = maxC; w.G = std::min(maxC, 96);
    auto F = [&](int64_t n) { w.bytes += n * 4; return dalloc_in<float>(m->ws_allocs, n); };
    const int G = w.G;
    w.src_off = dalloc_in<long>(m->ws_allocs, (int64_t)3 * maxC);
    w.xnorm = F((int64_t)G * kSamplesPerChunk);
    w.convA = F(((int64_t)G * m->conv_S[0] + 16) * CD);
    w.convB = F(((int64_t)G * m->conv_S[1] + 16) * CD);
    const int64_t M = (int64_t)G * m->Ts;
    w.h0 = F(M * Hs); w.h1 = F(M * Hs); w.xln = F(M * Hs); w.qkv = F(M * 3 * Hs); w.att = F(M * Hs); w.ffn = F(M * c.w2v_ffn);
    w.silu_cond = F((int64_t)maxC * kNTok * kCond);
    w.ada = F((int64_t)maxB * kNTok * m->ada_n);
    w.style_cond = F((int64_t)maxB * kE);
    w.prev_in = F((int64_t)maxB * kNTok * kE); w.prev_in_p8 = F((int64_t)maxB * kNTok * kE);
    w.cache = F((int64_t)c.ar_depth * maxB * 2 * kNTok * 3 * kE);
    w.x = F((int64_t)maxB * 100 * kE); w.xmod = F((int64_t)maxB * 100 * kE); w.attn_out = F((int64_t)maxB * 100 * kE);
    w.ffn_h = F((int64_t)maxB * 100 * 4 * kE); w.logits = F((int64_t)maxB * 100 * 2 * c.code_dim);
    w.splitk_floats = (int64_t)8 << 20; w.splitk = F(w.splitk_floats); w.splitk_b[0] = w.splitk;
    for (int i = 1; i < 4; ++i) w.splitk_b[i] = F(w.splitk_floats);
    w.fhat = F((int64_t)maxB * 100 * c.code_dim); w.nextfeat = F((int64_t)maxB * 100 * c.code_dim);
    w.bits = dalloc_in<uint8_t>(m->ws_allocs, (int64_t)maxB * kNTok * c.code_dim);
    w.hist_bits = dalloc_in<uint8_t>(m->ws_allocs, (int64_t)maxB * kNTok * c.code_dim);
    w.has_style = dalloc_in<uint8_t>(m->ws_allocs, maxB);
    w.status = dalloc_in<int>(m->ws_allocs, 4);
    w.sess_slots = dalloc_in<float*>(m->ws_allocs, maxB);
    w.prev_fdec = F((int64_t)maxB * 100 * c.code_dim); w.msfeat = F((int64_t)maxB * 180 * c.code_dim);
    const int H = c.vae_hidden;
    w.dec_x = F((int64_t)maxB * 200 * c.code_dim); w.vh = F((int64_t)maxB * 200 * H); w.vln = F((int64_t)maxB * 200 * H);
    w.vqkv = F((int64_t)maxB * 200 * 3 * H); w.vatt = F((int64_t)maxB * 200 * H); w.vmlp = F((int64_t)maxB * 200 * H * 3 / 2);
    w.dec_out = F((int64_t)maxB * 200 * c.motion_dim); w.enc_in = F((int64_t)maxB * 100 * 128);
    w.enc_out = F((int64_t)maxB * 100 * c.code_dim); w.motion_chunk = F((int64_t)maxB * 100 * c.motion_dim);
    const int S = c.style_dim, SL = c.style_len;
    w.s_in = F((int64_t)maxB * SL * 128); w.s_h = F((int64_t)maxB * SL * S); w.s_qkv = F((int64_t)maxB * SL * 3 * S);
    w.s_att = F((int64_t)maxB * SL * S); w.s_ffn = F((int64_t)maxB * SL * c.style_ffn); w.s_tmp = F((int64_t)maxB * SL * S);
    for (void* p : m->ws_allocs)
        if (!p) return fail(m, ARTALK_EHIP, "hipMalloc failed while reserving workspace");
    HIPCHK(m, hipDeviceSynchronize());
    return ensure_stage(m, maxB, maxC);
}

void build_site_table(artalk_model* m) {
    const artalk_config& c = m->cfg;
    SiteExps& ex = m->ex;
    auto add = [m](std::string name, int* e) {
        m->site_of.emplace(e, (int)m->sites.size());
        m->sites.push_back({std::move(name), e});
    };
    for (int i = 0; i + 1 < c.w2v_n_conv; ++i) add("w2v.conv" + std::to_string(i) + ".ln_gelu", &ex.conv[i]);
    add("w2v.feature_projection.ln", &ex.fp_ln);
    add("w2v.posconv.input(fp32 A)", &ex.posconv_in);
    for (int i = 0; i < c.w2v_layers; ++i) {
        const std::string p = "w2v.layer" + std::to_string(i);
        SiteExps::W2V& E = ex.w2v[i];
        add(p + ".ln1", &E.ln1); add(p + ".qkv", &E.qkv); add(p + ".attn_out", &E.attn); add(p + ".ln2", &E.ln2); add(p + ".ffn_hidden", &E.ffn);
    }
    add("ar.silu_cond", &ex.silu_cond);
    add("ar.history_tokens", &ex.hist_tok);
    for (int l = 0; l < c.ar_depth; ++l) {
        const std::string p = "ar.block" + std::to_string(l);
        SiteExps::AR& E = ex.ar[l];
        add(p + ".ln1_mod", &E.ln1); add(p + ".attn_out", &E.attn); add(p + ".ln2_mod", &E.ln2); add(p + ".ffn_hidden", &E.ffn);
    }
    for (int sd = 0; sd < 2; ++sd)
        for (int i = 0; i < c.vae_depth; ++i) {
            const std::string p = std::string(sd == 0 ? "vae.encoder.layer" : "vae.decoder.layer") + std::to_string(i);
            SiteExps::VAE& E = ex.vae[sd][i];
            add(p + ".ln", &E.ln); add(p + ".qkv", &E.qkv); add(p + ".attn_out", &E.attn); add(p + ".residual", &E.resid); add(p + ".mlp_hidden", &E.mlp);
        }
    add("vae.encoder.input(fp32 A)", &ex.vae_enc_in);
    add("vae.decoder.input(fp32 A)", &ex.vae_dec_in);
    add("vae.decoder.output_head(fp32 A)", &ex.vae_dec_head);
    add("style.input(fp32 A)", &ex.style_in);
    for (int i = 0; i < c.style_layers; ++i) {
        const std::string p = "style.layer" + std::to_string(i);
        SiteExps::ST& E = ex.style[i];
        add(p + ".in(fp32 A)", &E.h); add(p + ".attn_out(fp32 A)", &E.attn); add(p + ".norm1(fp32 A)", &E.h1); add(p + ".ffn_hidden(fp32 A)", &E.ffn);
    }
}

void end_sessions_by_scales(artalk_model* m) {
    for (const auto& kv : m->sess.open) { m->sess.ended_by_scales.insert(kv.first); m->sess.owner[kv.second.slot] = 0; }
    m->sess.open.clear();
}
int commit_scales(artalk_model* m, const SiteExps& next) {
    const int* a = reinterpret_cast<const int*>(&m->ex);
    const int* b = reinterpret_cast<const int*>(&next);
    int changed = 0;
    for (size_t i = 0; i < sizeof(SiteExps) / sizeof(int); ++i) changed += a[i] != b[i];
    if (changed) {
        (void)hipSetDevice(m->device); (void)hipDeviceSynchronize();
        drop_graphs(m);
        m->invalidate_init_hist();
        if (m->stream_B > 0) { m->stream_B = 0; m->stream_scales_ended = true; }
        end_sessions_by_scales(m);
        m->ex = next;
    }
    m->scales_changed = 0;
    for (size_t i = 0; i < sizeof(SiteExps) / sizeof(int); ++i) m->scales_changed += a[i] != kActExp;
    return changed;
}

int call_stream(artalk_model* m, void* stream, hipStream_t* s) {
    (void)hipSetDevice(m->device);
    if (!stream && !m->own_stream) HIPCHK(m, hipStreamCreate(&m->own_stream));
    *s = stream ? (hipStream_t)stream : m->own_stream;
    return ARTALK_OK;
}
int check_has_style(artalk_model* m, const float* style_motion_dev, const uint8_t* has_style, int B, bool* encode) {
    *encode = false;
    for (int b = 0; style_motion_dev && has_style && b < B; ++b) {
        if (has_style[b] > 2) return fail(m, ARTALK_EINVAL, "has_style entries must be 0, 1 or 2");
        *encode |= has_style[b] == 1;
    }
    return ARTALK_OK;
}
int begin_clips(artalk_model* m, hipStream_t s, int B, const float* style_motion_dev, const uint8_t* has_style, bool encode_style,
                artalk_model::Stage* stg) {
    Workspace& w = m->ws;
    if (!has_style) style_motion_dev = nullptr;
    if (style_motion_dev) {
        std::memcpy(stg->has, has_style, (size_t)B);
        HIPCHK(m, hipMemcpyAsync(w.has_style, stg->has, B, hipMemcpyHostToDevice, s));
    }
    HIPCHK(m, hipEventRecord(stg->done, s));
    stg->used = true;
    HIPCHK(m, hipMemsetAsync(w.status, 0, 4 * sizeof(int), s));
    stage_mark(m, s, PB_OTHER);
    run_style(m, style_motion_dev, B, s, encode_style);
    stage_mark(m, s, PB_STYLE);
    return ARTALK_OK;
}
int chunk_step(artalk_model* m, hipStream_t s, int cond_row0, int Bn, int n_next, int tap_chunk, float* out_motion_dev, int64_t out_stride) {
    Workspace& w = m->ws;
    m->tap_chunk = tap_chunk;
    roctxRangePushA("artalk.ar.adaln_table");
    kbucket(m, KB_ADA);
    linear(m, w.silu_cond + (long)cond_row0 * kNTok * kCond, kCond, m->ada_w, m->ada_b, w.ada, m->ada_n, Bn * kNTok, m->ada_n, kCond,
           ACT_NONE, nullptr, s, m->precision == 1 ? LF_A_P8 : 0, nullptr, m->ex.silu_cond);
    roctxRangePop();
    stage_mark(m, s, PB_ADA);
    if (body_uses_graphs(m)) {
        Range r_body("artalk.body.graph");
        if (int rc = run_body(m, Bn, s, n_next)) return rc;
        stage_mark(m, s, PB_AR);
    } else {
        if (int rc = run_body(m, Bn, s, n_next)) return rc;
    }
    const size_t mrow = (size_t)100 * m->cfg.motion_dim * 4;
    HIPCHK(m, hipMemcpy2DAsync(out_motion_dev, (size_t)out_stride * 4, w.motion_chunk, mrow, mrow, Bn, hipMemcpyDeviceToDevice, s));
    return ARTALK_OK;
}

SessionRows session_rows(const artalk_model* m) {
    const Workspace& w = m->ws;
    SessionRows r;
    r.style = reinterpret_cast<uint4*>(w.style_cond); r.prev_in = reinterpret_cast<uint4*>(w.prev_in); r.prev_fdec = reinterpret_cast<uint4*>(w.prev_fdec);
    r.s16 = kE / 4; r.p16 = kNTok * kE / 4; r.f16 = 100 * m->cfg.code_dim / 4;
    return r;
}
int grow_sessions(artalk_model* m, int64_t n_slots) {
    artalk_model::Sessions& ss = m->sess;
    if (m->cfg.code_dim % 4) return fail(m, ARTALK_EINVAL, "sessions need a code_dim that is a multiple of 4 (16-byte rows)");
    while ((int64_t)ss.owner.size() < n_slots) {
        void* p = nullptr;
        HIPCHK(m, hipMalloc(&p, (size_t)artalk_model::kSessBlock * m->sess_slot_floats() * sizeof(float)));
        ss.blocks.push_back(static_cast<float*>(p));
        ss.owner.resize(ss.owner.size() + artalk_model::kSessBlock, 0);
    }
    if (ss.smooth_cap < (int64_t)ss.owner.size()) {
        if (ss.smooth_tab) (void)hipFree(ss.smooth_tab);
        ss.smooth_tab = nullptr; ss.smooth_cap = 0;
        HIPCHK(m, hipMalloc(&ss.smooth_tab, ss.owner.size() * (sizeof(float*) + sizeof(int4))));
        ss.smooth_cap = (int64_t)ss.owner.size();
    }
    return ARTALK_OK;
}

void smooth_span(int64_t seen, int nf, bool last, int* first, int* count) {
    const int64_t f = seen > kSavgolLag ? seen - kSavgolLag : 0;
    *first = (int)f;
    *count = (int)((last ? seen + nf : seen + nf - kSavgolLag) - f);
}
int smooth_row_range(const std::string& who, int nf, bool last, std::string* err) {
    if (nf < 0 || nf > 100) { *err = who + ": n_frames " + std::to_string(nf) + " is outside 0..100"; return ARTALK_EINVAL; }
    if (nf < 100 && !last) { *err = who + ": fewer than 100 frames (" + std::to_string(nf) + ") without `last`"; return ARTALK_EINVAL; }
    return ARTALK_OK;
}
int smooth_row_length(const std::string& who, int64_t seen, int nf, bool last, std::string* err) {
    if (seen < 0 || seen > INT_MAX - 2 * kSavgolMaxOut) { *err = who + ": frame count out of range"; return ARTALK_EINVAL; }
    if (last && seen + nf < kSavgolCarry) { *err = who + ": savgol (mode='interp') needs window_length <= T (T >= 9)"; return ARTALK_EINVAL; }
    return ARTALK_OK;
}
int smooth_stride_check(const char* fn, bool have_raw, bool need_raw, int64_t raw_stride, int64_t out_stride, int D, std::string* err) {
    if (need_raw && !have_raw) { *err = std::string(fn) + ": no raw frames given"; return ARTALK_EINVAL; }
    if (need_raw && raw_stride < 100LL * D) { *err = std::string(fn) + ": raw_stride is below 100 x " + std::to_string(D); return ARTALK_EINVAL; }
    if (out_stride < (int64_t)kSavgolMaxOut * D) { *err = std::string(fn) + ": out_stride is below 104 x " + std::to_string(D); return ARTALK_EINVAL; }
    return ARTALK_OK;
}
int smooth_check(artalk_model::Sessions& ss, const int64_t* ids, int n, bool have_raw, int64_t raw_stride, const int* n_frames,
                 const uint8_t* last, int64_t out_stride, int D, std::vector<artalk_model::Sessions::Open*>* st, std::string* err) {
    st->assign((size_t)n, nullptr);
    std::set<int64_t> listed;
    for (int i = 0; i < n; ++i) {
        const auto it = ss.open.find(ids[i]);
        if (it == ss.open.end()) {
            if (ss.ended_by_scales.count(ids[i])) {
                *err = "session " + std::to_string(ids[i]) + ": the site scales changed since artalk_session_open; open the session again";
                return ARTALK_ESTATE;
            }
            *err = "artalk_session_smooth: " + std::to_string(ids[i]) + " is not an open session";
            return ARTALK_EINVAL;
        }
        if (!listed.insert(ids[i]).second) { *err = "artalk_session_smooth: session " + std::to_string(ids[i]) + " is listed twice"; return ARTALK_EINVAL; }
        (*st)[i] = &it->second;
    }
    bool need_raw = false;
    for (int i = 0; i < n; ++i) {
        const int nf = n_frames ? n_frames[i] : 100;
        const bool lst = last && last[i];
        const std::string who = "artalk_session_smooth: session " + std::to_string(ids[i]);
        if (int rc = smooth_row_range(who, nf, lst, err)) return rc;
        if ((*st)[i]->smooth_done) { *err = who + " has been smoothed to its end (a `last` call was made)"; return ARTALK_ESTATE; }
        if (int rc = smooth_row_length(who, (*st)[i]->seen, nf, lst, err)) return rc;
        need_raw |= nf > 0;
    }
    return smooth_stride_check("artalk_session_smooth", have_raw, need_raw, raw_stride, out_stride, D, err);
}
int stage_session_slots(artalk_model* m, hipStream_t s, artalk_model::Stage* stg, const int* slot, int n) {
    for (int i = 0; i < n; ++i) stg->slots[i] = m->sess_slot(slot[i]);
    HIPCHK(m, hipMemcpyAsync(m->ws.sess_slots, stg->slots, (size_t)n * sizeof(float*), hipMemcpyHostToDevice, s));
    return ARTALK_OK;
}

}

extern "C" {

const char* artalk_last_error(const artalk_model* m) { return m ? m->err.c_str() : g_create_error.c_str(); }

int artalk_conv_tail_geometry(int64_t valid, int samples_per_chunk, int n_conv, const int* kernel, const int* stride, int* t_const, int* Tp,
                              int* Sp, int* samples_read) {
    if (!kernel || !stride || !t_const || !Tp || !Sp || !samples_read || n_conv < 2 || n_conv > 8 || samples_per_chunk <= 0 || valid < 1 ||
        valid > samples_per_chunk)
        return ARTALK_EINVAL;
    int T[8], J = 1, t = samples_per_chunk;
    for (int i = 0; i < n_conv; ++i) {
        if (kernel[i] <= 0 || stride[i] <= 0 || (i > 0 && stride[i] != 2) || t < kernel[i]) return ARTALK_EINVAL;
        t = (t - kernel[i]) / stride[i] + 1; T[i] = t;
        J *= stride[i];
        t_const[i] = (int)((valid + J - 1) / J);
    }
    const int L = n_conv - 1;
    const bool partial = t_const[L] < T[L] - 1;
    Tp[L] = partial ? t_const[L] + 1 : T[L];
    Sp[L] = Tp[L] + 1;
    for (int i = L; i > 0; --i) {
        Tp[i - 1] = partial ? (Tp[i] - 1) * stride[i] + kernel[i] : T[i - 1];
        Sp[i - 1] = 2 * Sp[i];
        if (Tp[i - 1] > Sp[i - 1] || Tp[i - 1] > T[i - 1]) return ARTALK_EINVAL;
    }
    *samples_read = partial ? (Tp[0] - 1) * stride[0] + kernel[0] : samples_per_chunk;
    return partial ? 1 : 0;
}
int64_t artalk_conv_tail_class(int64_t valid, int samples_per_chunk) {
    if (samples_per_chunk <= 0 || valid < 1 || valid > samples_per_chunk) return ARTALK_EINVAL;
    if (samples_per_chunk % 4) return samples_per_chunk;
    const int64_t q = samples_per_chunk / 4;
    return (valid + q - 1) / q * q;
}

int artalk_create(int device_id, const artalk_config* cfg, artalk_model** out) {
    if (!cfg || !out) { g_create_error = "null argument"; return ARTALK_EINVAL; }
    const artalk_config& c = *cfg;
    static const int want_pn[5] = {1, 5, 25, 50, 100};
    bool ok = c.n_levels == 5 && c.code_dim == 32 && c.motion_dim == 106 && c.vae_hidden == 512 && c.w2v_hidden == kCond &&
              c.w2v_conv_dim == 512 && c.w2v_n_conv >= 2 && c.w2v_n_conv <= 8 && c.ar_heads * 64 == kE && c.vae_heads * 64 == c.vae_hidden &&
              c.w2v_heads * 64 == c.w2v_hidden && c.style_dim == 128 && c.style_heads * 32 == c.style_dim && c.style_len == 50 &&
              c.w2v_conv_kernel[0] == 10 && c.w2v_conv_stride[0] == 5 && c.w2v_ffn % 32 == 0 && c.style_ffn % 32 == 0 &&
              c.w2v_layers >= 1 && c.w2v_layers <= 64 && c.ar_depth >= 1 && c.ar_depth <= 32 && c.vae_depth >= 1 && c.vae_depth <= 16 && c.style_layers >= 1 && c.style_layers <= 8;
    for (int i = 0; ok && i < 5; ++i) ok = c.patch_nums[i] == want_pn[i];
    if (!ok) { g_create_error = "unsupported configuration (kernels are specialised for assets/config.json + XLS-R-300M widths)"; return ARTALK_EINVAL; }
    if (hipSetDevice(device_id) != hipSuccess) { g_create_error = "hipSetDevice failed"; return ARTALK_EHIP; }
    artalk_model* m = new artalk_model();
    m->cfg = c; m->device = device_id;
    int T = kSamplesPerChunk;
    for (int i = 0; i < c.w2v_n_conv; ++i) { T = (T - c.w2v_conv_kernel[i]) / c.w2v_conv_stride[i] + 1; m->conv_T[i] = T; }
    m->n_conv = c.w2v_n_conv; m->Tw = T; m->Ts = T + 1;
// ... 17 lines not shown
    if (init_ms_tables() != 0) { g_create_error = "uploading the interpolation tables to the device failed"; delete m; return ARTALK_EHIP; }
    attention_prepare();
    gemm_p8_prepare();
    build_site_table(m);
    const int rc = build_registry(m);
    if (rc != ARTALK_OK) { g_create_error = m->err; artalk_destroy(m); return rc; }
    *out = m;
    return ARTALK_OK;
}

void artalk_destroy(artalk_model* m) {
    if (!m) return;
    (void)hipSetDevice(m->device);
    (void)hipDeviceSynchronize();
    drop_graphs(m);
    for (auto e : m->ev_pool) (void)hipEventDestroy(e);
    for (auto e : m->ktimer.pool) (void)hipEventDestroy(e);
    if (m->own_stream) (void)hipStreamDestroy(m->own_stream);
    for (int i = 0; i < 3; ++i) {
        if (m->side_stream[i]) (void)hipStreamDestroy(m->side_stream[i]);
        if (m->join_ev[i]) (void)hipEventDestroy(m->join_ev[i]);
    }
    if (m->fork_ev) (void)hipEventDestroy(m->fork_ev);
    free_stage(m);
    for (auto& st : m->stage) if (st.done) (void)hipEventDestroy(st.done);
    if (m->h_status) (void)hipHostFree(m->h_status);
    for (auto& e : m->status_ev) if (e) (void)hipEventDestroy(e);
    for (void* p : m->allocs) if (p) (void)hipFree(p);
    for (void* p : m->ws_allocs) if (p) (void)hipFree(p);
    for (float* p : m->sess.blocks) if (p) (void)hipFree(p);
    if (m->sess.smooth_tab) (void)hipFree(m->sess.smooth_tab);
    delete m;
}

int artalk_set_tensor(artalk_model* m, const char* key, const void* host_ptr, int dtype, int ndim, const int64_t* shape) {
    if (!m || !key || !host_ptr || !shape) return ARTALK_EINVAL;
    if (m->finalized) return fail(m, ARTALK_ESTATE, "weights are final after artalk_finalize_weights (derived layouts and packed copies exist); create a new model");
    auto it = m->slots.find(key);
    if (it == m->slots.end()) return fail(m, ARTALK_EKEY, std::string("Unexpected key in state_dict: ") + key);
    Slot& s = it->second;
    bool same = (int)s.shape.size() == ndim && dtype == s.dtype;
    for (int i = 0; same && i < ndim; ++i) same = s.shape[i] == shape[i];
    if (!same) return fail(m, ARTALK_EINVAL, std::string("size mismatch for ") + key);
    (void)hipSetDevice(m->device);
    const int64_t n = s.numel();
    if (dtype == ARTALK_DTYPE_I64) {
        s.host_i64.assign((const int64_t*)host_ptr, (const int64_t*)host_ptr + n);
        s.set = true;
        return ARTALK_OK;
    }
    const float* src = (const float*)host_ptr;
    if (s.kind == SK_HOST || n <= 4096) s.host.assign(src, src + n);
    int rc = ARTALK_OK;
    switch (s.kind) {
        case SK_DIRECT: rc = upload(m, s.dst, src, n); break;
        case SK_PADK: {
            const int64_t o = s.shape[0], in = s.shape[1];
            std::vector<float> t((size_t)o * s.pad_to, 0.f);
            for (int64_t r = 0; r < o; ++r) std::memcpy(&t[r * s.pad_to], src + r * in, in * sizeof(float));
            rc = upload(m, s.dst, t.data(), (int64_t)t.size());
            break;
        }
        case SK_CONV: {
            const int64_t o = s.shape[0], ci = s.shape[1], k = s.shape[2];
            std::vector<float> t((size_t)n);
            for (int64_t a = 0; a < o; ++a)
                for (int64_t b = 0; b < ci; ++b)
                    for (int64_t d = 0; d < k; ++d) t[(a * k + d) * ci + b] = src[(a * ci + b) * k + d];
            rc = upload(m, s.dst, t.data(), n);
            break;
        }
        default: break;
    }
    if (rc == ARTALK_OK) s.set = true;
    return rc;
}

int artalk_finalize_weights(artalk_model* m) {
    if (!m) return ARTALK_EINVAL;
    (void)hipSetDevice(m->device);
    std::string missing;
    int nmiss = 0;
    for (auto& kv : m->slots)
        if (!kv.second.set) { if (nmiss++ < 8) missing += (missing.empty() ? "" : ", ") + kv.first; }
    if (nmiss) return fail(m, ARTALK_EMISSING, "Missing key(s) in state_dict: " + missing + (nmiss > 8 ? ", ..." : ""));
    const artalk_config& c = m->cfg;
    {
        const Slot& li = m->slots["lvl_idx"]; const Slot& le = m->slots["lvl_embed.weight"];
        const Slot& pe = m->slots["pos_embed"]; const Slot& ppe = m->slots["prev_pos_embed"];
        std::vector<float> a((size_t)kNTok * kE), b((size_t)kNTok * kE);
        int tok = 0;
        for (int p = 0; p < c.n_levels; ++p)
            for (int i = 0; i < c.patch_nums[p]; ++i, ++tok)
                if (li.host_i64[tok] != p) return fail(m, ARTALK_EINVAL, "lvl_idx does not match V_PATCH_NUMS");
        for (int t = 0; t < kNTok; ++t)
            for (int e = 0; e < kE; ++e) {
                const float lv = le.host[(size_t)li.host_i64[t] * kE + e];
                a[(size_t)t * kE + e] = lv + pe.host[(size_t)t * kE + e];
                b[(size_t)t * kE + e] = lv + ppe.host[(size_t)t * kE + e];
            }
        if (int rc = upload(m, m->lvl_pos, a.data(), (int64_t)a.size())) return rc;
        if (int rc = upload(m, m->prev_lvl_pos, b.data(), (int64_t)b.size())) return rc;
        const Slot& mk = m->slots["attn_bias_for_masking"];
        for (int q = 0; q < kNTok; ++q)
            for (int k = 0; k < 2 * kNTok; ++k) {
                const float v = mk.host[(size_t)q * 2 * kNTok + k];
                const bool vis = k < kNTok || li.host_i64[q] >= li.host_i64[k - kNTok];
                if (vis ? (v != 0.f) : !(std::isinf(v) && v < 0)) return fail(m, ARTALK_EINVAL, "attn_bias_for_masking is not the level-causal mask");
            }
        const Slot& vm = m->slots["basic_vae.attn_mask"];
        for (int q = 0; q < 200; ++q)
            for (int k = 0; k < 200; ++k) {
                const float v = vm.host[(size_t)q * 200 + k];
                const bool vis = !(q < 100 && k >= 100);
                if (vis ? (v != 0.f) : !(std::isinf(v) && v < 0)) return fail(m, ARTALK_EINVAL, "basic_vae.attn_mask is not the expected mask");
            }
    }
    for (int i = 0; i < c.ar_depth; ++i) {
        const Slot& sm = m->slots["attn_blocks." + std::to_string(i) + ".attn.scale_mul_1H11"];
        std::vector<float> q(c.ar_heads);
        for (int h = 0; h < c.ar_heads; ++h) q[h] = std::exp(std::min(sm.host[h], (float)std::log(100.0)));
        if (int rc = upload(m, m->ar[i].qscale, q.data(), c.ar_heads)) return rc;
    }
    {
        const Slot& pe = m->slots["style_encoder.PE.pe"];
        if (int rc = upload(m, m->st_pe, pe.host.data() + (size_t)c.style_len * c.style_dim, c.style_dim)) return rc;
    }
    {
        const std::string pc = "audio_encoder.encoder.pos_conv_embed.conv.parametrizations.weight.";
        const Slot& g = m->slots[pc + "original0"]; const Slot& v = m->slots[pc + "original1"];
        const int64_t O = v.shape[0], I = v.shape[1], K = v.shape[2];
        std::vector<double> nrm(K, 0.0);
        for (int64_t o = 0; o < O; ++o)
            for (int64_t i = 0; i < I; ++i)
                for (int64_t k = 0; k < K; ++k) { const double x = v.host[(o * I + i) * K + k]; nrm[k] += x * x; }
        std::vector<float> t((size_t)O * I * K);
        for (int64_t k = 0; k < K; ++k) {
            const float nk = (float)std::sqrt(nrm[k]);
            for (int64_t o = 0; o < O; ++o)
                for (int64_t i = 0; i < I; ++i) t[(o * K + k) * I + i] = v.host[(o * I + i) * K + k] * (g.host[k] / nk);
        }
        if (int rc = upload(m, m->pos_w, t.data(), (int64_t)t.size())) return rc;
    }
    for (auto& kv : m->slots) { std::vector<float>().swap(kv.second.host); }
    for (auto& r : m->wranges) {
        if (r.n < 1024 || r.packed) continue;
        r.packed = dalloc<unsigned int>(m, r.n);
        if (!r.packed) return fail(m, ARTALK_EHIP, "hipMalloc failed for packed weights");
        launch_pack_split(r.base, r.packed, r.n, true, nullptr);
    }
    HIPCHK(m, hipDeviceSynchronize());
    if (m->precision == 2) { if (int rc = ensure_bf16_copy(m)) return rc; }
    m->finalized = true;
    return ARTALK_OK;
}

int artalk_reserve(artalk_model* m, int max_batch, int max_total_chunks) {
    if (!m || max_batch <= 0 || max_total_chunks < max_batch) return ARTALK_EINVAL;
    (void)hipSetDevice(m->device);
    return reserve(m, max_batch, max_total_chunks);
}
int64_t artalk_workspace_bytes(const artalk_model* m) { return m ? m->ws.bytes : 0; }
int64_t artalk_weight_bytes(const artalk_model* m) { return m ? m->weight_bytes : 0; }

int artalk_set_profiling(artalk_model* m, int level) { if (!m || level < 0 || level > 3) return ARTALK_EINVAL; m->profiling = level; return ARTALK_OK; }
int artalk_set_precision(artalk_model* m, int mode) {
    if (!m || mode < 0 || mode > 2) return ARTALK_EINVAL;
    if (mode == 2 && m->finalized) {
        (void)hipSetDevice(m->device);
        if (int rc = ensure_bf16_copy(m)) return rc;
    }
    m->precision = mode;
    return ARTALK_OK;
}
int artalk_set_tail_skip(artalk_model* m, int on) { if (!m) return ARTALK_EINVAL; m->tail_skip = on != 0; return ARTALK_OK; }
int artalk_set_graphs(artalk_model* m, int enable) {
    if (!m) return ARTALK_EINVAL;
    m->use_graphs = (enable & 0xff) != 0;
    const int br = (enable >> 8) & 0xff;
    if (br >= 0 && br <= 4) m->branches = br; else return ARTALK_EINVAL;
    if ((enable >> 16) & 0xffff) {
        m->splitk_tiles = ((enable >> 16) & 0xff) * 16; m->splitk_target = ((enable >> 24) & 0xff) * 16;
    }
    (void)hipSetDevice(m->device); (void)hipDeviceSynchronize();
    drop_graphs(m);
    m->invalidate_init_hist();
    return ARTALK_OK;
}
int artalk_graph_count(const artalk_model* m, long long* captures) {
    if (!m) return ARTALK_EINVAL;
    if (captures) *captures = m->graph_captures;
    return (int)m->graphs.size();
}

int artalk_set_audit(artalk_model* m, int enable) {
    if (!m) return ARTALK_EINVAL;
    (void)hipSetDevice(m->device);
    if (enable && !m->audit_vals) {
        HIPCHK(m, hipMalloc(reinterpret_cast<void**>(&m->audit_vals), kAuditSlots * sizeof(unsigned int)));
        m->allocs.push_back(m->audit_vals);
    }
    if (enable) {
        HIPCHK(m, hipDeviceSynchronize());
        HIPCHK(m, hipMemset(m->audit_vals, 0, kAuditSlots * sizeof(unsigned int)));
        m->audit_names.clear(); m->audit_index.clear(); m->audit_exp.clear();
    }
    m->audit = enable != 0;
    return ARTALK_OK;
}
int artalk_calibrate(artalk_model* m, float headroom) {
    if (!m || !(headroom >= 1.0f)) return ARTALK_EINVAL;
    if (!m->audit_vals || m->audit_names.empty()) { m->err = "artalk_calibrate: no audit data (artalk_set_audit(1), then artalk_infer in f32 mode)"; return ARTALK_ESTATE; }
    (void)hipSetDevice(m->device);
    if (hipDeviceSynchronize() != hipSuccess) return ARTALK_EHIP;
    const int n = (int)m->audit_names.size();
    std::vector<unsigned int> bits((size_t)n);
    if (hipMemcpy(bits.data(), m->audit_vals, n * sizeof(unsigned int), hipMemcpyDeviceToHost) != hipSuccess) return ARTALK_EHIP;
    SiteExps next = m->ex;
    int* const base = reinterpret_cast<int*>(&m->ex);
    int* const nbase = reinterpret_cast<int*>(&next);
    for (int i = 0; i < n; ++i) {
        if (!m->audit_exp[i]) continue;
        int* ex = nbase + (m->audit_exp[i] - base);
        float mx;
        std::memcpy(&mx, &bits[i], sizeof(float));
        if (!std::isfinite(mx)) { m->err = "artalk_calibrate: site " + m->audit_names[i] + " is not finite (calibrate in f32 mode)"; return ARTALK_EINVAL; }
        if (mx <= 0.f) continue;
        int e = *ex;
        while (e > -8 && (double)mx * std::ldexp(1.0, e) * headroom > 65504.0) --e;
        if ((double)mx * std::ldexp(1.0, e) > 65504.0) { m->err = "artalk_calibrate: site " + m->audit_names[i] + " exceeds every supported scale"; return ARTALK_EINVAL; }
        *ex = e;
    }
    return commit_scales(m, next);
}
int artalk_reset_scales(artalk_model* m) {
    if (!m) return ARTALK_EINVAL;
    (void)hipSetDevice(m->device); (void)hipDeviceSynchronize();
    if (m->scales_changed) end_sessions_by_scales(m);
    m->ex = SiteExps();
    m->scales_changed = 0;
    drop_graphs(m);
    m->invalidate_init_hist();
    return ARTALK_OK;
}
int artalk_get_scales(artalk_model* m, int* exps, int max_n) {
    if (!m || !exps || max_n <= 0) return ARTALK_EINVAL;
    const int n = std::min<int>((int)m->audit_names.size(), max_n);
    for (int i = 0; i < n; ++i) exps[i] = m->audit_exp[i] ? *m->audit_exp[i] : kActExp;
    return n;
}
int artalk_scale_sites(const artalk_model* m, char* names_buf, int buf_len) {
    if (!m) return ARTALK_EINVAL;
    const int n = (int)m->sites.size();
    if (!names_buf) return n;
    int need = 0;
    for (const auto& st : m->sites) need += (int)st.name.size() + 1;
    if (buf_len < need) { const_cast<artalk_model*>(m)->err = "artalk_scale_sites: names need " + std::to_string(need) + " bytes"; return ARTALK_EINVAL; }
    int pos = 0;
    for (const auto& st : m->sites) { std::memcpy(names_buf + pos, st.name.c_str(), st.name.size() + 1); pos += (int)st.name.size() + 1; }
    return n;
}
int artalk_get_site_scales(artalk_model* m, int* exps, int n) {
    if (!m || !exps) return ARTALK_EINVAL;
    if (n != (int)m->sites.size()) return fail(m, ARTALK_EINVAL, "artalk_get_site_scales: n must equal the site count " + std::to_string(m->sites.size()));
    for (int i = 0; i < n; ++i) exps[i] = *m->sites[i].ex;
    return ARTALK_OK;
}
int artalk_set_site_scales(artalk_model* m, const int* exps, int n) {
    if (!m || !exps) return ARTALK_EINVAL;
    if (n != (int)m->sites.size()) return fail(m, ARTALK_EINVAL, "artalk_set_site_scales: n must equal the site count " + std::to_string(m->sites.size()));
    for (int i = 0; i < n; ++i)
        if (exps[i] < -8 || exps[i] > kActExp)
            return fail(m, ARTALK_EINVAL, "artalk_set_site_scales: exponent " + std::to_string(exps[i]) + " of site " + m->sites[i].name + " is outside [-8, 4]");
    SiteExps next = m->ex;
    int* const base = reinterpret_cast<int*>(&m->ex);
    int* const nbase = reinterpret_cast<int*>(&next);
    for (int i = 0; i < n; ++i) nbase[m->sites[i].ex - base] = exps[i];
    return commit_scales(m, next);
}
int artalk_get_audit(artalk_model* m, char* names_buf, int buf_len, float* values, int max_n) {
    if (!m || !names_buf || !values || buf_len <= 0 || max_n <= 0) return ARTALK_EINVAL;
    if (!m->audit_vals) return 0;
    (void)hipSetDevice(m->device);
    if (hipDeviceSynchronize() != hipSuccess) return ARTALK_EHIP;
    const int n = std::min<int>((int)m->audit_names.size(), max_n);
    std::vector<unsigned int> bits((size_t)std::max(n, 1));
    if (n && hipMemcpy(bits.data(), m->audit_vals, n * sizeof(unsigned int), hipMemcpyDeviceToHost) != hipSuccess) return ARTALK_EHIP;
    int pos = 0, written = 0;
    for (int i = 0; i < n; ++i) {
        const std::string& nm = m->audit_names[i];
        if (pos + (int)nm.size() + 1 > buf_len) break;
        std::memcpy(names_buf + pos, nm.c_str(), nm.size() + 1);
        pos += (int)nm.size() + 1;
        std::memcpy(&values[i], &bits[i], sizeof(float));
        ++written;
    }
    return written;
}

int artalk_set_tap(artalk_model* m, float* tap_dev, int max_batch, int max_chunks) {
    if (!m || max_batch < 0 || max_chunks < 0) return ARTALK_EINVAL;
    (void)hipSetDevice(m->device); (void)hipDeviceSynchronize();
    m->tap = tap_dev; m->tap_B = tap_dev ? max_batch : 0; m->tap_maxch = tap_dev ? max_chunks : 0; m->tap_chunk = 0;
    return ARTALK_OK;
}
int artalk_tap_layout(int64_t* out, int n) {
    if (!out || n < 7) return ARTALK_EINVAL;
    const int64_t v[7] = {TAP_BLK0_IN, TAP_BLK0_OUT, TAP_BLKL_OUT, TAP_PREV_IN, TAP_LOGITS, TAP_DEC_OUT, TAP_SLOT};
    for (int i = 0; i < 7; ++i) out[i] = v[i];
    return ARTALK_OK;
}

int artalk_set_cu_mask(artalk_model* m, const uint32_t* mask, int n_words) {
    if (!m || n_words < 0 || (n_words > 0 && !mask)) return ARTALK_EINVAL;
    (void)hipSetDevice(m->device); (void)hipDeviceSynchronize();
    m->cu_mask.assign(mask, mask + n_words);
    int n = 0;
    for (uint32_t w : m->cu_mask) n += __builtin_popcount(w);
    if (n_words > 0 && n < 8) { m->cu_mask.clear(); m->n_cus = 0; return fail(m, ARTALK_EINVAL, "a CU partition needs at least 8 compute units"); }
    int dev_cus = 0;
    if (hipDeviceGetAttribute(&dev_cus, hipDeviceAttributeMultiprocessorCount, m->device) == hipSuccess && dev_cus > 0) n = std::min(n, dev_cus);
    m->n_cus = n;
    for (int i = 0; i < 3; ++i) {
        if (m->side_stream[i]) { (void)hipStreamDestroy(m->side_stream[i]); m->side_stream[i] = nullptr; }
        if (m->join_ev[i]) { (void)hipEventDestroy(m->join_ev[i]); m->join_ev[i] = nullptr; }
    }
    drop_graphs(m);
    m->invalidate_init_hist();
    return ARTALK_OK;
}

int artalk_infer(artalk_model* m, const float* audio_dev, int64_t audio_clip_stride, const int64_t* n_chunks, int B,
                 const float* style_motion_dev, const uint8_t* has_style, float* out_motion_dev, int64_t out_clip_stride,
                 uint8_t* out_bits_dev, uint8_t* out_hist_bits_dev, float* out_w2v_dev, void* stream) {
    return artalk_infer_samples(m, audio_dev, audio_clip_stride, n_chunks, nullptr, B, style_motion_dev, has_style, out_motion_dev, out_clip_stride,
                                out_bits_dev, out_hist_bits_dev, out_w2v_dev, stream);
}

int artalk_infer_samples(artalk_model* m, const float* audio_dev, int64_t audio_clip_stride, const int64_t* n_chunks, const int64_t* n_samples,
                         int B, const float* style_motion_dev, const uint8_t* has_style, float* out_motion_dev, int64_t out_clip_stride,
                         uint8_t* out_bits_dev, uint8_t* out_hist_bits_dev, float* out_w2v_dev, void* stream) {
    if (!m || !audio_dev || !n_chunks || !out_motion_dev || B <= 0) return ARTALK_EINVAL;
    if (!m->finalized) return fail(m, ARTALK_ESTATE, "artalk_infer before artalk_finalize_weights");
    for (int b = 0; n_samples && b < B; ++b)
        if (n_chunks[b] > 0 && (n_samples[b] < 1 || n_samples[b] > n_chunks[b] * kSamplesPerChunk))
            return fail(m, ARTALK_EINVAL, "n_samples[" + std::to_string(b) + "] must be in 1 .. n_chunks * " + std::to_string(kSamplesPerChunk));
    hipStream_t s;
    if (int rc = call_stream(m, stream, &s)) return rc;
    const artalk_config& c = m->cfg;
    int64_t C = 0, maxch = n_chunks[0];
    for (int b = 0; b < B; ++b) {
        if (n_chunks[b] <= 0 || (b > 0 && n_chunks[b] > n_chunks[b - 1])) return fail(m, ARTALK_EINVAL, "n_chunks must be positive and non-increasing");
        C += n_chunks[b];
    }
    bool encode_style;
    if (int rc = check_has_style(m, style_motion_dev, has_style, B, &encode_style)) return rc;
    if (m->tap && (B > m->tap_B || maxch > m->tap_maxch)) return fail(m, ARTALK_EINVAL, "the tap buffer (artalk_set_tap) is smaller than this call");
    if (B > m->ws.maxB || C > m->ws.maxC) { if (int rc = reserve(m, B, (int)C)) return rc; }
    Workspace& w = m->ws;
    artalk_model::Stage* stg = nullptr;
    if (int rc = next_stage(m, &stg)) return rc;
    long* src = stg->src;
    std::vector<int> base((size_t)maxch + 1, 0), Bj((size_t)maxch, 0);
    {
        int idx = 0;
        for (int64_t j = 0; j < maxch; ++j) {
            base[j] = idx;
            for (int b = 0; b < B && n_chunks[b] > j; ++b) { src[idx++] = (long)b * audio_clip_stride + (long)j * kSamplesPerChunk; Bj[j]++; }
        }
        base[maxch] = idx;
    }
    std::vector<ConvPasses> passes;
    bool any_tail = false;
    if (n_samples && m->tail_skip) {
        std::vector<int> cls((size_t)C, 3);
        for (int64_t j = 0, idx = 0; j < maxch; ++j)
            for (int b = 0; b < B && n_chunks[b] > j; ++b, ++idx) {
                const int64_t v = std::min<int64_t>(n_samples[b] - j * kSamplesPerChunk, kSamplesPerChunk);
                const int64_t bound = v >= 1 ? artalk_conv_tail_class(v, kSamplesPerChunk) : 0;
                const int q = bound >= 1 && kSamplesPerChunk % 4 == 0 ? (int)(bound / (kSamplesPerChunk / 4)) : 4;
                cls[idx] = m->tail_geo[q - 1].partial ? q - 1 : 3;
            }
        const int last = m->n_conv - 1;
        for (int c0 = 0; c0 < C; c0 += w.G) {
            const int n = (int)std::min<int64_t>(w.G, C - c0);
            ConvPasses cp;
            static const int order[4] = {3, 0, 1, 2};
            int pos = 0;
            long row0 = 0;
            for (int k = 0; k < 4; ++k) {
                const int cl = order[k], off = pos;
                const artalk_model::TailGeo& tg = m->tail_geo[cl];
                const long rows = cl == 3 ? m->Ts : tg.S[last], tc = cl == 3 ? m->Tw - 1 : tg.tc;
                for (int i = 0; i < n; ++i)
                    if (cls[c0 + i] == cl) {
                        src[C + c0 + pos] = src[c0 + i];
                        src[2 * C + c0 + i] = (row0 + (pos - off) * rows) | (tc << 32);
                        ++pos;
                    }
                if (pos > off) { cp.off[cp.np] = off; cp.n[cp.np] = pos - off; cp.cls[cp.np] = cl; ++cp.np; row0 += (pos - off) * rows; }
            }
            if (cp.np == 1 && cp.cls[0] == 3) cp.np = 0;
            else { cp.perm = w.src_off + C + c0; cp.tab = w.src_off + 2 * C + c0; any_tail = true; }
            passes.push_back(cp);
        }
    }
    HIPCHK(m, hipMemcpyAsync(w.src_off, src, (any_tail ? 3 : 1) * C * sizeof(long), hipMemcpyHostToDevice, s));
    m->stream_B = 0; m->stream_scales_ended = false;
    m->ev_used = 0; m->dom_events.clear(); m->marks.clear(); m->prof_stream = s;
    struct TimerScope { bool on; TimerScope(artalk_model* x) : on(x->profiling == 3) { if (on) { x->ktimer.used = 0; x->ktimer.recs.clear(); x->ktimer.bucket = KB_OTHER; g_ktimer = &x->ktimer; } }
                        ~TimerScope() { if (on) g_ktimer = nullptr; } } timer_scope(m);
    if (int rc = begin_clips(m, s, B, style_motion_dev, has_style, encode_style, stg)) return rc;
    for (int c0 = 0, gi = 0; c0 < C; c0 += w.G, ++gi)
        run_wav2vec(m, audio_dev, c0, (int)std::min<int64_t>(w.G, C - c0), out_w2v_dev, s, !passes.empty() && passes[gi].np ? &passes[gi] : nullptr);
    if (int rc = run_init_history(m, B, s)) return rc;
    const size_t bits_row = (size_t)kNTok * c.code_dim;
    if (out_hist_bits_dev)
        HIPCHK(m, hipMemcpy2DAsync(out_hist_bits_dev, (size_t)(maxch + 1) * bits_row, w.hist_bits, bits_row, bits_row, B,
                                   hipMemcpyDeviceToDevice, s));
    stage_mark(m, s, PB_VAE);
    for (int64_t j = 0; j < maxch; ++j) {
        const int Bn = Bj[j];
        const int n_next = out_hist_bits_dev ? Bn : (j + 1 < maxch ? Bj[j + 1] : 0);
        if (int rc = chunk_step(m, s, base[j], Bn, n_next, (int)j, out_motion_dev + j * 100 * c.motion_dim, out_clip_stride)) return rc;
        if (out_bits_dev)
            HIPCHK(m, hipMemcpy2DAsync(out_bits_dev + j * bits_row, (size_t)maxch * bits_row, w.bits, bits_row, bits_row, Bn,
                                       hipMemcpyDeviceToDevice, s));
        if (out_hist_bits_dev)
            HIPCHK(m, hipMemcpy2DAsync(out_hist_bits_dev + (j + 1) * bits_row, (size_t)(maxch + 1) * bits_row, w.hist_bits, bits_row,
                                       bits_row, Bn, hipMemcpyDeviceToDevice, s));
    }
    stage_mark(m, s, PB_OTHER);
    if (int rc = publish_status(m, s)) return rc;
    if (m->sticky_error) { m->sticky_error = false; return ARTALK_ESTATE; }
    return ARTALK_OK;
}

int artalk_style_encode(artalk_model* m, const float* style_motion_dev, int n, float* out_cond_dev, void* stream) {
    if (!m || !style_motion_dev || !out_cond_dev || n <= 0) return ARTALK_EINVAL;
    if (!m->finalized) return fail(m, ARTALK_ESTATE, "artalk_style_encode before artalk_finalize_weights");
    hipStream_t s;
    if (int rc = call_stream(m, stream, &s)) return rc;
    if (m->stream_B > 0) return fail(m, ARTALK_ESTATE, "artalk_style_encode during a streaming session (it shares the workspace)");
    if (n > m->ws.maxB) { if (int rc = reserve(m, n, std::max(n, m->ws.maxC))) return rc; }
    Workspace& w = m->ws;
    HIPCHK(m, hipMemsetAsync(w.has_style, 1, n, s));
    {
        ProfilingOff quiet(m);
        run_style(m, style_motion_dev, n, s, true);
    }
    HIPCHK(m, hipMemcpyAsync(out_cond_dev, w.style_cond, (size_t)n * kE * sizeof(float), hipMemcpyDeviceToDevice, s));
    HIPCHK(m, hipGetLastError());
    return ARTALK_OK;
}

int artalk_stream_begin(artalk_model* m, int B, const float* style_motion_dev, const uint8_t* has_style, void* stream) {
    if (!m || B <= 0) return ARTALK_EINVAL;
    if (!m->finalized) return fail(m, ARTALK_ESTATE, "artalk_stream_begin before artalk_finalize_weights");
    bool encode_style;
    if (int rc = check_has_style(m, style_motion_dev, has_style, B, &encode_style)) return rc;
    hipStream_t s;
    if (int rc = call_stream(m, stream, &s)) return rc;
    if (B > m->ws.maxB || B > m->ws.maxC) { if (int rc = reserve(m, B, B)) return rc; }
    if (int rc = ensure_stage(m, m->ws.maxB, m->ws.maxC)) return rc;
    artalk_model::Stage* stg = nullptr;
    if (int rc = next_stage(m, &stg)) return rc;
    {
        ProfilingOff quiet(m);
        if (int rc = begin_clips(m, s, B, style_motion_dev, has_style, encode_style, stg)) return rc;
        if (int rc = run_init_history(m, B, s)) return rc;
    }
    m->stream_B = B; m->stream_scales_ended = false;
    if (int rc = publish_status(m, s)) return rc;
    return ARTALK_OK;
}

int artalk_stream_chunk(artalk_model* m, const float* audio_dev, int64_t chunk_stride, float* out_motion_dev, int64_t out_stride,
                        void* stream) {
    if (!m || !audio_dev || !out_motion_dev) return ARTALK_EINVAL;
    if (m->stream_B <= 0)
        return fail(m, ARTALK_ESTATE, m->stream_scales_ended ? "the site scales changed since artalk_stream_begin; begin again"
                                                             : "artalk_stream_chunk before artalk_stream_begin");
    hipStream_t s;
    if (int rc = call_stream(m, stream, &s)) return rc;
    const int B = m->stream_B;
    Workspace& w = m->ws;
    if (B > w.maxB) return fail(m, ARTALK_ESTATE, "workspace was re-reserved since artalk_stream_begin; begin again");
    artalk_model::Stage* stg = nullptr;
    if (int rc = next_stage(m, &stg)) return rc;
    for (int b = 0; b < B; ++b) stg->src[b] = (long)b * chunk_stride;
    HIPCHK(m, hipMemcpyAsync(w.src_off, stg->src, B * sizeof(long), hipMemcpyHostToDevice, s));
    HIPCHK(m, hipEventRecord(stg->done, s));
    stg->used = true;
    ProfilingOff quiet(m);
    for (int c0 = 0; c0 < B; c0 += w.G) run_wav2vec(m, audio_dev, c0, std::min(w.G, B - c0), nullptr, s);
    if (int rc = chunk_step(m, s, 0, B, B, m->tap_maxch, out_motion_dev, out_stride)) return rc;
    if (int rc = publish_status(m, s)) return rc;
    return ARTALK_OK;
}

int artalk_stream_end(artalk_model* m) {
    if (!m) return ARTALK_EINVAL;
    m->stream_B = 0; m->stream_scales_ended = false;
    return ARTALK_OK;
}

int artalk_sessions_reserve(artalk_model* m, int max_sessions) {
    if (!m || max_sessions <= 0) return ARTALK_EINVAL;
    (void)hipSetDevice(m->device);
    return grow_sessions(m, max_sessions);
}

int artalk_session_count(const artalk_model* m) { return m ? (int)m->sess.open.size() : ARTALK_EINVAL; }

int artalk_session_open(artalk_model* m, int n, const float* style_motion_dev, const uint8_t* has_style, int64_t* ids_out, void* stream) {
    if (!m || n <= 0 || !ids_out) return ARTALK_EINVAL;
    if (!m->finalized) return fail(m, ARTALK_ESTATE, "artalk_session_open before artalk_finalize_weights");
    bool encode_style;
    if (int rc = check_has_style(m, style_motion_dev, has_style, n, &encode_style)) return rc;
    hipStream_t s;
    if (int rc = call_stream(m, stream, &s)) return rc;
    artalk_model::Sessions& ss = m->sess;
    if (int rc = grow_sessions(m, (int64_t)ss.open.size() + n)) return rc;
    if (n > m->ws.maxB || n > m->ws.maxC) { if (int rc = reserve(m, n, n)) return rc; }
    if (int rc = ensure_stage(m, m->ws.maxB, m->ws.maxC)) return rc;
    std::vector<int> slot;
    for (int i = 0; i < (int)ss.owner.size() && (int)slot.size() < n; ++i)
        if (!ss.owner[i]) slot.push_back(i);
    artalk_model::Stage* stg = nullptr;
    if (int rc = next_stage(m, &stg)) return rc;
    if (int rc = stage_session_slots(m, s, stg, slot.data(), n)) return rc;
    m->stream_B = 0; m->stream_scales_ended = false;
    {
        ProfilingOff quiet(m);
        if (int rc = begin_clips(m, s, n, style_motion_dev, has_style, encode_style, stg)) return rc;
        if (int rc = run_init_history(m, n, s)) return rc;
    }
    launch_session_scatter(m->ws.sess_slots, session_rows(m), n, true, s);
    if (int rc = publish_status(m, s)) return rc;
    for (int i = 0; i < n; ++i) {
        ids_out[i] = ss.next_id++;
        ss.owner[slot[i]] = ids_out[i];
        ss.open.emplace(ids_out[i], artalk_model::Sessions::Open{slot[i]});
    }
    return ARTALK_OK;
}

int artalk_session_step(artalk_model* m, const int64_t* ids, int n, const float* audio_dev, int64_t chunk_stride, float* out_motion_dev,
                        int64_t out_stride, uint8_t* out_bits_dev, uint8_t* out_hist_bits_dev, void* stream) {
    if (!m || !ids || n <= 0 || !audio_dev || !out_motion_dev) return ARTALK_EINVAL;
    artalk_model::Sessions& ss = m->sess;
    std::vector<int> slot((size_t)n);
    std::set<int64_t> seen;
    for (int i = 0; i < n; ++i) {
        const auto it = ss.open.find(ids[i]);
        if (it == ss.open.end()) {
            if (ss.ended_by_scales.count(ids[i]))
                return fail(m, ARTALK_ESTATE, "session " + std::to_string(ids[i]) + ": the site scales changed since artalk_session_open; open the session again");
            return fail(m, ARTALK_EINVAL, "artalk_session_step: " + std::to_string(ids[i]) + " is not an open session");
        }
        if (!seen.insert(ids[i]).second) return fail(m, ARTALK_EINVAL, "artalk_session_step: session " + std::to_string(ids[i]) + " is listed twice");
        slot[i] = it->second.slot;
    }
    hipStream_t s;
    if (int rc = call_stream(m, stream, &s)) return rc;
    if (n > m->ws.maxB || n > m->ws.maxC) { if (int rc = reserve(m, n, n)) return rc; }
    Workspace& w = m->ws;
    artalk_model::Stage* stg = nullptr;
    if (int rc = next_stage(m, &stg)) return rc;
    for (int b = 0; b < n; ++b) stg->src[b] = (long)b * chunk_stride;
    HIPCHK(m, hipMemcpyAsync(w.src_off, stg->src, n * sizeof(long), hipMemcpyHostToDevice, s));
    if (int rc = stage_session_slots(m, s, stg, slot.data(), n)) return rc;
    HIPCHK(m, hipEventRecord(stg->done, s));
    stg->used = true;
    m->stream_B = 0; m->stream_scales_ended = false;
    HIPCHK(m, hipMemsetAsync(w.status, 0, 4 * sizeof(int), s));
    const SessionRows rows = session_rows(m);
    ProfilingOff quiet(m);
    launch_session_gather(w.sess_slots, rows, n, s);
    for (int c0 = 0; c0 < n; c0 += w.G) run_wav2vec(m, audio_dev, c0, std::min(w.G, n - c0), nullptr, s);
    if (int rc = chunk_step(m, s, 0, n, n, m->tap_maxch, out_motion_dev, out_stride)) return rc;
    launch_session_scatter(w.sess_slots, rows, n, false, s);
    const size_t bits_n = (size_t)n * kNTok * m->cfg.code_dim;
    if (out_bits_dev) HIPCHK(m, hipMemcpyAsync(out_bits_dev, w.bits, bits_n, hipMemcpyDeviceToDevice, s));
    if (out_hist_bits_dev) HIPCHK(m, hipMemcpyAsync(out_hist_bits_dev, w.hist_bits, bits_n, hipMemcpyDeviceToDevice, s));
    if (int rc = publish_status(m, s)) return rc;
    return ARTALK_OK;
}

int artalk_session_close(artalk_model* m, const int64_t* ids, int n) {
    if (!m || !ids || n <= 0) return ARTALK_EINVAL;
    artalk_model::Sessions& ss = m->sess;
    std::set<int64_t> seen;
    for (int i = 0; i < n; ++i)
        if ((!ss.open.count(ids[i]) && !ss.ended_by_scales.count(ids[i])) || !seen.insert(ids[i]).second)
            return fail(m, ARTALK_EINVAL, "artalk_session_close: " + std::to_string(ids[i]) + " is not an open session (or is listed twice)");
    for (int i = 0; i < n; ++i) {
        const auto it = ss.open.find(ids[i]);
        if (it != ss.open.end()) { ss.owner[it->second.slot] = 0; ss.open.erase(it); }
        ss.ended_by_scales.erase(ids[i]);
    }
    return ARTALK_OK;
}

int artalk_session_smooth(artalk_model* m, const int64_t* ids, int n, const float* raw_dev, int64_t raw_stride, const int* n_frames,
                          const uint8_t* last, float* out_dev, int64_t out_stride, int* first_out, int* count_out, void* stream) {
    if (!m || !ids || n <= 0 || !out_dev || !first_out || !count_out) return ARTALK_EINVAL;
    artalk_model::Sessions& ss = m->sess;
    std::vector<artalk_model::Sessions::Open*> st;
    std::string err;
    if (int rc = smooth_check(ss, ids, n, raw_dev != nullptr, raw_stride, n_frames, last, out_stride, m->cfg.motion_dim, &st, &err)) return fail(m, rc, err);
    hipStream_t s;
    if (int rc = call_stream(m, stream, &s)) return rc;
    if (n > m->stage_cap_b) { if (int rc = ensure_stage(m, n, m->stage_cap_c)) return rc; }
    artalk_model::Stage* stg = nullptr;
    if (int rc = next_stage(m, &stg)) return rc;
    for (int i = 0; i < n; ++i) {
        stg->slots[i] = m->sess_slot(st[i]->slot);
        stg->smooth[i] = make_int4((int)st[i]->seen, n_frames ? n_frames[i] : 100, last && last[i] ? 1 : 0, 0);
    }
    float** slots_dev = static_cast<float**>(ss.smooth_tab);
    int4* meta_dev = reinterpret_cast<int4*>(slots_dev + ss.smooth_cap);
    HIPCHK(m, hipMemcpyAsync(slots_dev, stg->slots, (size_t)n * sizeof(float*), hipMemcpyHostToDevice, s));
    HIPCHK(m, hipMemcpyAsync(meta_dev, stg->smooth, (size_t)n * sizeof(int4), hipMemcpyHostToDevice, s));
    HIPCHK(m, hipEventRecord(stg->done, s));
    stg->used = true;
    launch_savgol_stream(slots_dev, meta_dev, (long)m->sess_carry_off(), raw_dev, (long)raw_stride, out_dev, (long)out_stride, n,
                         m->cfg.motion_dim, s);
    HIPCHK(m, hipGetLastError());
    for (int i = 0; i < n; ++i) {
        const int nf = n_frames ? n_frames[i] : 100;
        const bool lst = last && last[i];
        smooth_span(st[i]->seen, nf, lst, &first_out[i], &count_out[i]);
        st[i]->seen += nf;
        st[i]->smooth_done = lst;
    }
    return ARTALK_OK;
}

int artalk_get_status(artalk_model* m, int* flags, void* stream) {
    (void)stream;
    if (!m || !flags) return ARTALK_EINVAL;
    if (!m->status_pending) { *flags = 0; return ARTALK_OK; }
    (void)hipSetDevice(m->device);
    const int slot = (int)((m->ticket - 1) % artalk_model::kStatusSlots);
    HIPCHK(m, hipEventSynchronize(m->status_ev[slot]));
    *flags = m->h_status[slot];
    return ARTALK_OK;
}
// ... 864 lines not shown
```

### artalk_amd/csrc/kernels.h

```cpp
#pragma once
#include <hip/hip_runtime.h>
#include <climits>
#include <cstdint>

#include <hip/hip_ext.h>
#include <utility>
#include <vector>

namespace artalk {

struct KernelTimer {
    int bucket = 0;
    std::vector<hipEvent_t> pool; size_t used = 0;
    std::vector<std::pair<int, size_t>> recs;
};
extern thread_local KernelTimer* g_ktimer;
bool ktimer_events(hipEvent_t* e0, hipEvent_t* e1);
#define ARTALK_LAUNCH(kernel, grid, block, lds, stream, ...)                                                          \
    do {                                                                                                              \
        hipEvent_t kt_e0_ = nullptr, kt_e1_ = nullptr;                                                                \
        if (artalk::g_ktimer && artalk::ktimer_events(&kt_e0_, &kt_e1_))                                              \
            hipExtLaunchKernelGGL(kernel, grid, block, lds, stream, kt_e0_, kt_e1_, 0, __VA_ARGS__);                  \
        else                                                                                                          \
            hipLaunchKernelGGL(kernel, grid, block, lds, stream, __VA_ARGS__);                                        \
    } while (0)

struct RowMap {
    int rpb;
    int bstride;
    int off;
};
static inline RowMap rowmap_identity() { return RowMap{INT_MAX, 0, 0}; }
static inline RowMap rowmap(int rows_per_batch, int batch_stride_rows, int row_off) {
    return RowMap{rows_per_batch, batch_stride_rows, row_off};
}

enum Act { ACT_NONE = 0, ACT_GELU_ERF = 1, ACT_GELU_TANH = 2, ACT_LEAKY02 = 3 };
constexpr int kActExp = 4;

struct GemmArgs {
    const float* A = nullptr; long lda = 0;
    const float* W = nullptr; long ldw = 0;
    const unsigned int* Wp = nullptr;
    const void* Wb = nullptr;
    int c_p8 = 0;
    int a_packed = 0;
    int a_exp = 4, c_exp = 4;
    int exact = 0;
    const float* bias = nullptr;
    float* C = nullptr; long ldc = 0; RowMap cmap = {INT_MAX, 0, 0};
    float* c2 = nullptr;
    const float* gate = nullptr; long ldg = 0; RowMap gmap = {INT_MAX, 0, 0};
    const float* R = nullptr; long ldr = 0;
    int M = 0, N = 0, K = 0;
    int act = ACT_NONE;
    int batch = 1; long sA = 0, sW = 0, sBias = 0, sC = 0, sR = 0;
    int amode = 0; int pc_T = 0, pc_tstride = 0, pc_pad = 0, pc_cin = 0;
    int splitk = 1; float* partial = nullptr;
    int ngrp = 0; long grpW = 0, grpB = 0, grpC = 0;
    int res_lds = 0;
    int w_nt = 0;
    int cus = 0;
    int force_cfg = -1;
    int graph_tag = 0;
    int* status = nullptr;
};
void launch_gemm(const GemmArgs& g, hipStream_t s);
void launch_splitk_reduce(const GemmArgs& g, hipStream_t s);
struct LnArgs;
bool splitk_reduce_ln_eligible(const GemmArgs& g, const LnArgs& ln);
void launch_splitk_reduce_ln(const GemmArgs& g, const LnArgs& ln, hipStream_t s);
int gemm_config(const GemmArgs& g);
int gemm_tile_count(const GemmArgs& g);
void launch_pack_split(const float* w, unsigned int* out, long n, bool is_weight, hipStream_t s, int* status = nullptr, int p8_exp = kActExp);
bool gemm_p8_eligible(const GemmArgs& g);
void gemm_p8_prepare();
void launch_gemm_bf16(const GemmArgs& g, hipStream_t s);
int gemm_bf16_config(const GemmArgs& g);
int gemm_bf16_tile_count(const GemmArgs& g);
void launch_pack_bf16(const float* in, void* out, long n, hipStream_t s);

struct GemmPolicy {
    int precision = 0;
    bool reg_staged = false;
    float* slabs = nullptr; int64_t slab_floats = 0;
    int splitk_tiles = 0, splitk_target = 0;
};
enum GemmPath { GEMM_F32 = 0, GEMM_F16S = 1, GEMM_P8 = 2, GEMM_BF16 = 3 };
enum P8Class { P8_NONE = 0, P8_BIG, P8_GROUPS, P8_SMALL };
int gemm_p8_class(int cfg);
struct GemmPlan {
    int path = GEMM_F32;
    int cfg = -1;
    bool c2_fused = false;
    bool dominant = false;
    bool fused_ln = false;
};
GemmPlan plan_gemm(GemmArgs& g, const GemmPolicy& p, const LnArgs* fuse_ln);
void run_gemm(const GemmArgs& g, const GemmPlan& plan, const LnArgs* fuse_ln, hipStream_t s);
void launch_posconv_p8(const GemmArgs& g, int n_chunks, int T, int Ts, hipStream_t s);
static inline double gemm_flops(const GemmArgs& g) { return 2.0 * g.M * (double)g.N * g.K * g.batch; }

struct LnArgs {
    const float* X = nullptr; long ldx = 0;
    float* Y = nullptr; long ldy = 0;
    const float* w = nullptr; const float* b = nullptr;
    const float* scale = nullptr; const float* shift = nullptr;
    long ldm = 0; RowMap mmap = {INT_MAX, 0, 0};
    int M = 0, D = 0; float eps = 1e-5f; int act = ACT_NONE;
    int out_p8 = 0;
    int p8_exp = 4;
    int* status = nullptr;
    int junk_period = 0, junk_from = 0;
    int junk_row2 = 0, junk_period2 = 0, junk_from2 = 0;
    int plan_M = 0;
};
void launch_layernorm(const LnArgs& a, hipStream_t s);
struct AttnArgs {
    const float* Q = nullptr; long ldq = 0, q_bstride = 0;
    const float* K = nullptr; long ldk = 0, k_bstride = 0;
    const float* V = nullptr; long ldv = 0, v_bstride = 0;
    float* O = nullptr; long ldo = 0, o_bstride = 0;
    int B = 0, H = 0, HD = 64, Lq = 0, Lk = 0;
    float scale = 1.f;
    int l2norm = 0; const float* qscale = nullptr;
    int split_q = 0, split_k = 0;
    int out_p8 = 0;
    int split16 = 0;
    int qkv_p8 = 0;
    int qkv_exp = 4, o_exp = 4;
    int* status = nullptr;
    int cus = 0;
};
enum AttnKernel {
    ATTN_NONE = -1,
    ATTN_F32_64 = 0,
    ATTN_F32_32 = 1,
    ATTN_SHORT = 2,
    ATTN_F16 = 3,
    ATTN_F16_P8 = 4,
    ATTN_F16_WIDE = 5,
    ATTN_F16_PP = 6,
    ATTN_F16_WIDE_AR = 7,
    ATTN_F16_WIDE_AR_P8 = 8,
};
AttnKernel plan_attention(const AttnArgs& a, int n_cu);
AttnKernel launch_attention(const AttnArgs& a, hipStream_t s);
void attention_prepare();

void launch_audio_normalize(const float* audio, const long* src_off, float* xnorm, int n_chunks, int n, hipStream_t s);
void launch_conv0(const float* xnorm, int n, const float* w , const float* bias, const float* lnw,
                  const float* lnb, float* Y, int n_chunks, int T, int row_stride, hipStream_t s, int out_p8 = 0, int* status = nullptr, int p8_exp = kActExp);
void launch_conv_tail_gather(const float* X, const long* tab, float* Y, int n_chunks, int Tw, int Ts, int D, hipStream_t s);
void launch_pool_silu(const float* X, int x_tstride, int T, float* Y, int n_chunks, const int* patch_nums, int n_lvls,
                      int D, hipStream_t s, int out_p8 = 0, int* status = nullptr, int p8_exp = kActExp);

void launch_ar_bits_next(const float* logits, uint8_t* bits, float* fhat, float* nextfeat, int B, int level, hipStream_t s,
                         int* status = nullptr);
void launch_vq_embed(const float* feat, int n, const float* We, const float* be, const float* pos, float* X, int xrows,
                     int xoff, const float* style_cond, const float* pos0, int B, hipStream_t s);
void launch_ar_begin(const float* style_cond, const float* lvlpos, float* x0, float* fhat, int B, hipStream_t s);
void launch_dec_input(const float* prev_fdec, const float* fhat, const uint8_t* bits, const float* dpos, float* X,
                      int B, hipStream_t s);
void launch_dec_finish(const float* dec , const float* mean, const float* stdv, const float* epos,
                       float* out, long out_bstride, int chunk, float* E, int B, hipStream_t s, int* status = nullptr);
void launch_enc_input_zero(const float* mean, const float* stdv, const float* epos, float* E, int B, hipStream_t s);
void launch_broadcast16(const void* src, void* dst, long bytes, int B, hipStream_t s);
struct SessionRows {
    uint4* style; uint4* prev_in; uint4* prev_fdec;
    int s16, p16, f16;
};
void launch_session_gather(const float* const* slots, const SessionRows& w, int n, hipStream_t s);
void launch_session_scatter(float* const* slots, const SessionRows& w, int n, bool with_style, hipStream_t s);
void launch_bsq_history(const float* enc_out, uint8_t* hist_bits, float* prev_fdec, float* msfeat, int B, hipStream_t s,
                        int* status = nullptr);
void launch_style_input(const float* motion, const float* mean, const float* stdv, float* X, int B, hipStream_t s);
void launch_style_finish(const float* feat , const float* Ws, const float* bs, const float* null_cond,
                         const uint8_t* has_style, float* style_cond, int B, hipStream_t s, const float* cached = nullptr,
                         long cached_stride = 0);
void launch_add_row(float* X, const float* v, int M, int D, hipStream_t s);
void launch_savgol(const float* in, float* out, int T, int D, hipStream_t s);
constexpr int kSavgolLag = 4, kSavgolCarry = 9, kSavgolMaxOut = 104;
void launch_savgol_stream(float* const* slots, const int4* meta, long carry_off, const float* raw, long raw_stride, float* out,
                          long out_stride, int n, int D, hipStream_t s);

double launch_mfma_f32_peak(float* out, int blocks, int iters, int nacc, hipStream_t s);
void launch_resample_mean(const float* x, int nch, int n, const float* taps, int orig, int nw, int width, float* out, int n_out,
                          hipStream_t s);
void launch_flame_pose(const float* pose, float* rot, float* feat, int T, int ldf, hipStream_t s);
void launch_flame_joints(const float* vs, const float* jreg, float* J, int T, int V, hipStream_t s);
void launch_flame_skin(const float* vposed, const float* rot, const float* J, const int* parents, const float* weights, float* out,
                       int T, int V, float scale, hipStream_t s);
void launch_absmax(const float* buf, int rows, int cols, long ld, int is_p8, unsigned int* slot, hipStream_t s, int junk_period = 0,
                   int junk_from = 0, int p8_exp = kActExp);
int init_ms_tables();

}
```

### artalk_amd/model.py

```python
from __future__ import annotations

import ctypes as C
import math
from typing import List, Optional, Sequence

import numpy as np
import torch

from . import capi
from .config import ARTalkConfig

SCALES_FORMAT = "artalk-site-scales/1"
SCALE_EXP_MIN, SCALE_EXP_MAX = -8, 4


def check_scales(sites, names: Sequence[str]) -> List[int]:
    if not isinstance(sites, dict):
        raise ValueError("site scales must be a {site name: exponent} dict")
    missing = [n for n in names if n not in sites]
    extra = [n for n in sites if n not in set(names)]
    if missing or extra:
        raise ValueError("the site scales do not match this model's site table ({} missing, e.g. {}; {} extra, e.g. {}): they belong to "
                         "another architecture".format(len(missing), missing[:3], len(extra), extra[:3]))
    exps = []
# ... 170 lines not shown
        return self

    def reserve(self, max_batch: int, max_total_chunks: int):
        rc = capi.lib().artalk_reserve(self._h, int(max_batch), int(max_total_chunks))
        if rc != capi.OK:
            raise RuntimeError("artalk_reserve failed: " + self._err())
        self._reserved = (int(max_batch), int(max_total_chunks))

    def status(self, wait: bool = True) -> Optional[int]:
        f = C.c_int(0)
        if wait:
            rc = capi.lib().artalk_get_status(self._h, C.byref(f), None)
        else:
            rc = capi.lib().artalk_poll_status(self._h, C.byref(f))
            if rc == capi.EBUSY:
                return None
        if rc != capi.OK:
            raise RuntimeError("artalk status query failed: " + self._err())
        return int(f.value)

    _status = status

    def last_ticket(self) -> int:
        return int(capi.lib().artalk_last_ticket(self._h))

    def status_of(self, ticket: int) -> int:
        f = C.c_int(0)
        if capi.lib().artalk_get_status_of(self._h, C.c_longlong(ticket), C.byref(f)) != capi.OK:
            raise RuntimeError("artalk status query failed: " + self._err())
        return int(f.value)

    def calibrate(self, audios, style_motions=None, headroom: float = 4.0) -> int:
        L = capi.lib()
        prec, chk = self._precision, self.check_finite
        try:
            self.set_precision("f32")
            self.check_finite = False
            if L.artalk_set_audit(self._h, 1) != capi.OK:
                raise RuntimeError("artalk_set_audit failed: " + self._err())
            self.inference_batch(audios, style_motions, check=False)
            changed = int(L.artalk_calibrate(self._h, C.c_float(float(headroom))))
            if changed < 0:
                raise RuntimeError("artalk_calibrate failed: " + self._err())
        finally:
            L.artalk_set_audit(self._h, 0)
            self.check_finite = chk
            self.set_precision(prec)
        self._style_cache = {}
        self._sync_sessions()
        self._calibrations = getattr(self, "_calibrations", 0) + 1
        self._headroom = float(headroom)
        return changed

    def _site_names(self) -> List[str]:
        if getattr(self, "_site_table", None) is None:
            L = capi.lib()
            n = int(L.artalk_scale_sites(self._h, None, 0))
            if n < 0:
                raise RuntimeError("artalk_scale_sites failed: " + self._err())
            buf = C.create_string_buffer(n * 64 + 1024)
            if L.artalk_scale_sites(self._h, buf, len(buf)) != n:
                raise RuntimeError("artalk_scale_sites failed: " + self._err())
            self._site_table = [x.decode() for x in buf.raw.split(b"\0")[:n]]
        return self._site_table

    def _read_site_exps(self) -> List[int]:
        names = self._site_names()
        arr = (C.c_int * len(names))()
        if capi.lib().artalk_get_site_scales(self._h, arr, len(names)) != capi.OK:
            raise RuntimeError("artalk_get_site_scales failed: " + self._err())
        return [int(v) for v in arr]

    def _write_site_exps(self, exps: Sequence[int]) -> int:
        arr = (C.c_int * len(exps))(*exps)
        changed = int(capi.lib().artalk_set_site_scales(self._h, arr, len(exps)))
        if changed < 0:
            raise RuntimeError("artalk_set_site_scales failed: " + self._err())
        return changed

    def scales(self) -> dict:
        if not self._loaded:
            raise RuntimeError("load_state_dict must be called before scales")
        return dict(zip(self._site_names(), self._read_site_exps()))

    def load_scales(self, src) -> int:
        if not self._loaded:
            raise RuntimeError("load_state_dict must be called before load_scales")
        headroom = None
        if isinstance(src, dict):
            sites = src
        else:
            doc = read_scales_file(src)
            sites, headroom = doc["sites"], doc.get("headroom")
        exps = check_scales(sites, self._site_names())
        changed = self._write_site_exps(exps)
        if changed:
            self._n_streams = 0
            self._style_cache = {}
            self._sync_sessions()
        if not isinstance(src, dict) or changed:
            self._headroom = headroom
        return changed

    def save_scales(self, path):
        import dataclasses
        import json
        doc = {"format": SCALES_FORMAT, "sites": self.scales(), "config": dataclasses.asdict(self.cfg), "headroom": self._headroom}
        with open(path, "w") as f:
            json.dump(doc, f, indent=1)

    def reset_scales(self):
        if capi.lib().artalk_reset_scales(self._h) != capi.OK:
            raise RuntimeError("artalk_reset_scales failed: " + self._err())
        self._headroom = None
        self._sync_sessions()

    def _trip_to_f32(self, what: str):
        import warnings
        warnings.warn(f"artalk_amd: non-finite result in f16x3 mode ({what}); re-running in f32 mode and staying there "
                      "(set_precision('f16x3') switches back)")
        self.set_precision("f32")
        self._latched_f32 = True

    def workspace_bytes(self):
        return int(capi.lib().artalk_workspace_bytes(self._h))

    def weight_bytes(self):
        return int(capi.lib().artalk_weight_bytes(self._h))

    def set_profiling(self, level: int):
        capi.lib().artalk_set_profiling(self._h, int(level))

    def set_precision(self, mode):
        names = {0: "f32", 1: "f16x3", 2: "bf16"}
        code = {"f32": 0, "f16x3": 1, "bf16": 2}.get(mode, mode)
        if code not in names:
            raise ValueError(f"precision mode must be 'f32', 'f16x3' or 'bf16' (got {mode!r})")
        code = int(code)
        self._precision = names[code]
        self._latched_f32 = False
        if self._h is not None and self._loaded:
            rc = capi.lib().artalk_set_precision(self._h, int(code))
            if rc == capi.EINVAL:
                raise ValueError("precision mode must be 'f32', 'f16x3' or 'bf16'")
            if rc != capi.OK:
                raise RuntimeError(f"artalk_set_precision({code}) failed ({rc}): {self._err()}")

    def set_graphs(self, on: bool, branches: int = 0, splitk_tiles: int = 0, splitk_target: int = 0):
        capi.lib().artalk_set_graphs(self._h, int(bool(on)) | (int(branches) << 8) | ((splitk_tiles // 16) << 16) | ((splitk_target // 16) << 24))

    def set_tail_skip(self, on: bool):
        if capi.lib().artalk_set_tail_skip(self._h, int(bool(on))) != capi.OK:
            raise RuntimeError("artalk_set_tail_skip failed")

    def graph_count(self):
        n = C.c_longlong(0)
        held = capi.lib().artalk_graph_count(self._h, C.byref(n))
        return int(held), int(n.value)

    def set_cu_mask(self, words: Optional[Sequence[int]]):
        if not self._loaded:
            raise RuntimeError("load_state_dict must be called before set_cu_mask")
        L = capi.lib()
        self.stream_end()
        with torch.cuda.device(self._device):
            torch.cuda.synchronize()
            old = getattr(self, "_masked_handle", None)
            if old is not None:
                self._stream = None
                L.artalk_op_destroy_stream(C.c_void_p(old))
                self._masked_handle = None
            if words is None:
                if L.artalk_set_cu_mask(self._h, None, 0) != capi.OK:
                    raise RuntimeError("artalk_set_cu_mask failed: " + self._err())
                self._stream = None
                return
            arr = (C.c_uint32 * len(words))(*[int(w) & 0xFFFFFFFF for w in words])
            if L.artalk_set_cu_mask(self._h, C.cast(arr, C.c_void_p), len(words)) != capi.OK:
                raise RuntimeError("artalk_set_cu_mask failed: " + self._err())
            out = C.c_void_p()
            if L.artalk_op_create_masked_stream(C.cast(arr, C.c_void_p), len(words), C.byref(out)) != capi.OK:
                raise RuntimeError("hipExtStreamCreateWithCUMask failed")
            self._masked_handle = out.value
            self._stream = torch.cuda.ExternalStream(out.value, device=self._device)

    def get_profile(self):
        out = (C.c_double * 10)()
        rc = capi.lib().artalk_get_profile(self._h, out, 10)
        if rc != capi.OK:
            raise RuntimeError("artalk_get_profile failed: " + self._err())
        keys = ["style_ms", "w2v_conv_ms", "w2v_encoder_ms", "ada_ms", "ar_ms", "vae_ms", "total_ms",
                "dom_launches", "dom_ms", "dom_flop"]
        return dict(zip(keys, list(out)))

    def get_kernel_sums(self):
        out = (C.c_double * 14)()
        if capi.lib().artalk_get_kernel_sums(self._h, out, 14) != capi.OK:
            raise RuntimeError("artalk_get_kernel_sums failed: " + self._err())
        keys = ["style", "w2v_conv", "w2v_encoder", "ada", "ar_history_kv", "level0", "level1", "level2", "level3", "level4", "vae_decode",
                "reencode", "other", "kernels"]
        return dict(zip(keys, list(out)))

    def _style_key(self, s: torch.Tensor):
        if not s.is_cuda:
            return ("host", hash(s.detach().to(torch.float32).contiguous().numpy().tobytes()), self._precision)
        return ("dev", s.data_ptr(), s._version, tuple(s.stride()), s.dtype, str(s.device), self._precision)

    def _style_rows(self, style_motions, order, B):
        if style_motions is None or not any(s is not None for s in style_motions):
            return None, None
        dev = self._device
        L, D = self.cfg.style_len, self.cfg.motion_dim
        style_t = torch.zeros(B, L, D, dtype=torch.float32, device=dev)
        has = (C.c_uint8 * B)()
        keys = {}
        for pos, i in enumerate(order):
            s = style_motions[i]
            if s is None:
                continue
            assert tuple(s.shape) == (L, D), f"Invalid style_motion shape: {tuple(s.shape)}."
            if self.style_cache_size > 0:
                keys[pos] = self._style_key(s)
            else:
                style_t[pos] = s.to(device=dev, dtype=torch.float32)
                has[pos] = 1
        if keys:
            new = {}
            for pos, k in keys.items():
                if k not in self._style_cache and k not in new:
                    new[k] = style_motions[order[pos]]
            if new:
                clips = torch.stack([v.to(device=dev, dtype=torch.float32) for v in new.values()])
                cond = torch.empty(len(new), self.cfg.embed_dim, dtype=torch.float32, device=dev)
                self._stream.wait_stream(torch.cuda.current_stream())
                rc = capi.lib().artalk_style_encode(self._h, capi.ptr(clips), len(new), capi.ptr(cond), C.c_void_p(self._stream.cuda_stream))
                if rc != capi.OK:
                    raise RuntimeError("artalk_style_encode failed: " + self._err())
                torch.cuda.current_stream().wait_stream(self._stream)
                clips.record_stream(self._stream)
                cond.record_stream(self._stream)
                for j, (k, v) in enumerate(new.items()):
                    self._style_cache[k] = (v, cond[j])
                while len(self._style_cache) > self.style_cache_size:
                    self._style_cache.pop(next(iter(self._style_cache)))
            flat = style_t.view(B, L * D)
            for pos, k in keys.items():
                hit = self._style_cache.get(k) or (None, None)
                if hit[1] is None:
                    style_t[pos] = style_motions[order[pos]].to(device=dev, dtype=torch.float32)
                    has[pos] = 1
                else:
                    flat[pos, :self.cfg.embed_dim] = hit[1]
                    has[pos] = 2
        return style_t, has

    @torch.no_grad()
    def stream_begin(self, n_streams: int, style_motions: Optional[Sequence[Optional[torch.Tensor]]] = None):
        if not self._loaded:
            raise RuntimeError("load_state_dict must be called before inference")
        dev = self._device
        with torch.cuda.device(dev):
            if self._stream is None:
                self._stream = torch.cuda.Stream(device=dev)
            caller = torch.cuda.current_stream()
            self._stream.wait_stream(caller)
            self.stream_end()
            style_t, has = self._style_rows(style_motions, list(range(n_streams)), n_streams)
            self._stream.wait_stream(caller)
            rc = capi.lib().artalk_stream_begin(self._h, int(n_streams), capi.ptr(style_t),
                                                C.cast(has, C.c_void_p) if has is not None else None, C.c_void_p(self._stream.cuda_stream))
            caller.wait_stream(self._stream)
            if style_t is not None:
                style_t.record_stream(self._stream)
        if rc != capi.OK:
            raise RuntimeError("artalk_stream_begin failed: " + self._err())
        self._n_streams = int(n_streams)
        self._stream_style = style_motions
        self._stream_fed = [0] * self._n_streams

    @torch.no_grad()
    def stream_chunk(self, audio_chunks: torch.Tensor, n_valid: Optional[Sequence[int]] = None):
        B = getattr(self, "_n_streams", 0)
        if B <= 0:
            raise RuntimeError("stream_chunk before stream_begin")
        assert audio_chunks.shape == (B, self.cfg.samples_per_chunk), f"expected ({B}, {self.cfg.samples_per_chunk}) samples"
        dev = self._device
        with torch.cuda.device(dev):
            x = audio_chunks.to(device=dev, dtype=torch.float32).contiguous()
            out = torch.empty(B, 100, self.cfg.motion_dim, dtype=torch.float32, device=dev)
            caller = torch.cuda.current_stream()
            self._stream.wait_stream(caller)
            rc = capi.lib().artalk_stream_chunk(self._h, capi.ptr(x), x.stride(0), capi.ptr(out), out.stride(0),
                                                C.c_void_p(self._stream.cuda_stream))
            caller.wait_stream(self._stream)
            x.record_stream(self._stream)
            out.record_stream(self._stream)
        if rc != capi.OK:
            raise RuntimeError("artalk_stream_chunk failed: " + self._err())
        if self._precision == "f16x3" and self.check_finite and self.status() != 0:
            self.stream_end()
            if self.auto_calibrate:
                try:
                    changed = self.calibrate([x[b] for b in range(B)], self._stream_style)
                except RuntimeError:
                    changed = 0
                if changed > 0:
# ... 339 lines not shown
```

### include/artalk_hip.h

```cpp
#ifndef ARTALK_HIP_H
#define ARTALK_HIP_H

#include <stdint.h>

#ifdef __cplusplus
extern "C" {
#endif

#define ARTALK_OK 0
#define ARTALK_EINVAL (-1)
#define ARTALK_EKEY (-2)
#define ARTALK_EMISSING (-3)
#define ARTALK_EHIP (-4)
#define ARTALK_ESTATE (-5)
#define ARTALK_ECAPACITY (-6)
#define ARTALK_EBUSY (-7)

#define ARTALK_DTYPE_F32 0
#define ARTALK_DTYPE_I64 1

typedef struct artalk_model artalk_model;

typedef struct artalk_config {
    int32_t ar_depth, ar_heads;
    int32_t vae_depth, vae_heads, vae_hidden;
    int32_t code_dim, motion_dim;
    int32_t n_levels; int32_t patch_nums[8];
    int32_t w2v_layers, w2v_hidden, w2v_heads, w2v_ffn;
    int32_t w2v_n_conv; int32_t w2v_conv_kernel[8]; int32_t w2v_conv_stride[8]; int32_t w2v_conv_dim;
    int32_t w2v_pos_kernel, w2v_pos_groups;
    float w2v_ln_eps;
    int32_t style_dim, style_heads, style_layers, style_ffn, style_len;
} artalk_config;

int artalk_create(int device_id, const artalk_config* cfg, artalk_model** out);
void artalk_destroy(artalk_model* m);
const char* artalk_last_error(const artalk_model* m);

int artalk_set_tensor(artalk_model* m, const char* key, const void* host_ptr, int dtype, int ndim, const int64_t* shape);
int artalk_finalize_weights(artalk_model* m);

int artalk_reserve(artalk_model* m, int max_batch, int max_total_chunks);
int64_t artalk_workspace_bytes(const artalk_model* m);
int64_t artalk_weight_bytes(const artalk_model* m);

int artalk_infer(artalk_model* m, const float* audio_dev, int64_t audio_clip_stride, const int64_t* n_chunks, int B,
                 const float* style_motion_dev, const uint8_t* has_style, float* out_motion_dev, int64_t out_clip_stride,
                 uint8_t* out_bits_dev, uint8_t* out_hist_bits_dev, float* out_w2v_dev, void* stream);

int artalk_infer_samples(artalk_model* m, const float* audio_dev, int64_t audio_clip_stride, const int64_t* n_chunks,
                         const int64_t* n_samples, int B, const float* style_motion_dev, const uint8_t* has_style, float* out_motion_dev,
                         int64_t out_clip_stride, uint8_t* out_bits_dev, uint8_t* out_hist_bits_dev, float* out_w2v_dev, void* stream);
int artalk_set_tail_skip(artalk_model* m, int on);
int artalk_conv_tail_geometry(int64_t valid, int samples_per_chunk, int n_conv, const int* kernel, const int* stride, int* t_const,
                              int* Tp, int* Sp, int* samples_read);
int64_t artalk_conv_tail_class(int64_t valid, int samples_per_chunk);

int artalk_style_encode(artalk_model* m, const float* style_motion_dev, int n, float* out_cond_dev, void* stream);

int artalk_stream_end(artalk_model* m);
int artalk_stream_begin(artalk_model* m, int B, const float* style_motion_dev, const uint8_t* has_style, void* stream);
int artalk_stream_chunk(artalk_model* m, const float* audio_dev, int64_t chunk_stride, float* out_motion_dev, int64_t out_stride,
                        void* stream);

int artalk_sessions_reserve(artalk_model* m, int max_sessions);
int artalk_session_open(artalk_model* m, int n, const float* style_motion_dev, const uint8_t* has_style, int64_t* ids_out, void* stream);
int artalk_session_step(artalk_model* m, const int64_t* ids, int n, const float* audio_dev, int64_t chunk_stride, float* out_motion_dev,
                        int64_t out_stride, uint8_t* out_bits_dev, uint8_t* out_hist_bits_dev, void* stream);
int artalk_session_close(artalk_model* m, const int64_t* ids, int n);
int artalk_session_count(const artalk_model* m);
int artalk_session_smooth(artalk_model* m, const int64_t* ids, int n, const float* raw_dev, int64_t raw_stride, const int* n_frames,
                          const uint8_t* last, float* out_dev, int64_t out_stride, int* first_out, int* count_out, void* stream);

typedef struct artalk_flame artalk_flame;
int artalk_flame_create(int device_id, int V, int NB, int P, const float* v_template, const float* shapedirs, const float* posedirs_t,
                        const float* J_regressor, const int32_t* parents, const float* lbs_weights, float scale, artalk_flame** out);
int artalk_flame_verts(artalk_flame* f, const float* betas_dev, const float* full_pose_dev, int T, float* out_dev, void* stream);
void artalk_flame_destroy(artalk_flame* f);
const char* artalk_flame_last_error(const artalk_flame* f);

int artalk_get_status(artalk_model* m, int* flags, void* stream);
int artalk_poll_status(artalk_model* m, int* flags);
long long artalk_last_ticket(artalk_model* m);
int artalk_get_status_of(artalk_model* m, long long ticket, int* flags);

int artalk_savgol(artalk_model* m, const float* in_dev, float* out_dev, int T, void* stream);

int artalk_set_profiling(artalk_model* m, int level);
int artalk_get_profile(artalk_model* m, double* out, int n);
int artalk_get_kernel_sums(artalk_model* m, double* out, int n);
int artalk_set_precision(artalk_model* m, int mode);
int artalk_set_graphs(artalk_model* m, int enable);
int artalk_graph_count(const artalk_model* m, long long* captures);
int artalk_set_audit(artalk_model* m, int enable);
int artalk_get_audit(artalk_model* m, char* names_buf, int buf_len, float* values, int max_n);
int artalk_calibrate(artalk_model* m, float headroom);
int artalk_reset_scales(artalk_model* m);
int artalk_get_scales(artalk_model* m, int* exps, int max_n);
int artalk_scale_sites(const artalk_model* m, char* names_buf, int buf_len);
int artalk_get_site_scales(artalk_model* m, int* exps, int n);
int artalk_set_site_scales(artalk_model* m, const int* exps, int n);
int artalk_set_tap(artalk_model* m, float* tap_dev, int max_batch, int max_chunks);
int artalk_tap_layout(int64_t* out, int n);
int artalk_set_cu_mask(artalk_model* m, const uint32_t* mask, int n_words);

int artalk_op_gemm(const float* A, int64_t lda, const float* W, const float* bias, const float* gate, const float* R,
                   float* C, int M, int N, int K, int act, void* stream);
int artalk_op_gemm_ex(const float* A, int64_t lda, const float* W, const float* bias, float* C, int M, int N, int K, int act,
                      int force_cfg, void* stream);
int artalk_op_mfma_f32_peak(float* out_dev, int blocks, int iters, int nacc, double* flops, void* stream);
int artalk_op_gemm_f16s(const float* A, int64_t lda, const float* W, const float* bias, float* C, int M, int N, int K, int act,
                        int force_cfg, void* stream);
int artalk_op_gemm_bf16(const float* A, int64_t lda, const float* W, const float* bias, const float* gate, const float* R, float* C,
                        int M, int N, int K, int act, int force_cfg, void* stream);
int artalk_op_pack_split(const float* in, void* out_u32, int64_t n, int is_weight, void* stream);
int artalk_op_gemm_f16s_packed(const void* A, int a_packed, int64_t lda, const void* Wp, const float* bias, float* C, int M, int N,
                               int K, int act, int force_cfg, void* stream);
int artalk_op_release_scratch(void);
int artalk_op_gemm_p8_plan(int M, int N, int K, int residual);
int artalk_op_create_masked_stream(const uint32_t* mask, int n_words, void** out_stream);
int artalk_op_destroy_stream(void* stream);
int artalk_op_layernorm(const float* X, float* Y, const float* w, const float* b, const float* scale, const float* shift,
                        int M, int D, float eps, int act, void* stream);
int artalk_op_attention(const float* Q, const float* K, const float* V, float* O, int B, int H, int HD, int Lq, int Lk,
                        float scale, int l2norm, const float* qscale, int split, void* stream);
int artalk_op_w2v_front(const float* audio, int C, int n, const float* w, const float* bias, const float* lnw,
                        const float* lnb, float* xnorm_out, float* Y, void* stream);
int artalk_op_resample_mean(const float* x, int nch, int n, const float* taps, int orig, int nw, int width, float* out, int n_out,
                            void* stream);
int artalk_op_pool_silu(const float* X, int C, int T, int D, float* Y, void* stream);
int artalk_op_pack_split_ex(const float* in, void* out_u32, int64_t n, int is_weight, int p8_exp, int* status_dev, void* stream);
int artalk_op_layernorm_ex(const float* X, float* Y, const float* w, const float* b, const float* scale, const float* shift,
                           int M, int D, float eps, int act, int p8_exp, int junk_period, int junk_from, int* status_dev, void* stream);
int artalk_op_gemm_f16s_packed_ex(const void* A, int a_packed, int64_t lda, const void* Wp, const float* bias, float* C, int M, int N,
                                  int K, int act, int force_cfg, int a_exp, int c_exp, void* c2_u32, int* status_dev, void* stream);
int artalk_op_gemm_f16s_ex(const float* A, int64_t lda, const float* W, const float* bias, float* C, int M, int N, int K, int act,
                           int force_cfg, int a_exp, int* status_dev, void* stream);
int artalk_op_attention_ex(const float* Q, const float* K, const float* V, float* O, int B, int H, int HD, int Lq, int Lk,
                           float scale, int l2norm, const float* qscale, int split, int qkv_exp, int o_exp, int out_p8,
                           int* status_dev, void* stream);
int artalk_op_w2v_front_ex(const float* audio, int C, int n, const float* w, const float* bias, const float* lnw,
                           const float* lnb, float* xnorm_out, float* Y, int out_p8, int p8_exp, int* status_dev, void* stream);
int artalk_op_pool_silu_ex(const float* X, int C, int T, int D, float* Y, int out_p8, int p8_exp, int* status_dev, void* stream);
int artalk_op_posconv_p8_ex(const float* X, const void* Wp, const float* bias, const float* R, float* C, int n_chunks, int T, int Ts,
                            int act, int a_exp, int* status_dev, void* stream);
int artalk_op_bsq_history(const float* enc_out, uint8_t* hist_bits, float* prev_fdec, float* msfeat, int B, void* stream);
int artalk_op_bsq_history_ex(const float* enc_out, uint8_t* hist_bits, float* prev_fdec, float* msfeat, int B, int* status_dev,
                             void* stream);
int artalk_op_ar_bits_next(const float* logits, uint8_t* bits, float* fhat, float* nextfeat, int B, int level, int* status_dev,
                           void* stream);
int artalk_op_vq_embed(const float* feat, int n, const float* We, const float* be, const float* pos, float* X, int xrows, int xoff,
                       const float* style_cond, const float* pos0, int B, void* stream);
int artalk_op_ar_begin(const float* style_cond, const float* lvlpos, float* x0, float* fhat, int B, void* stream);
int artalk_op_dec_input(const float* prev_fdec, const float* fhat, const uint8_t* bits, const float* dpos, float* X, int B, void* stream);
int artalk_op_dec_finish(const float* dec, const float* mean, const float* std_, const float* epos, float* out, int64_t out_bstride,
                         int chunk, float* E, int B, int* status_dev, void* stream);
int artalk_op_enc_input_zero(const float* mean, const float* std_, const float* epos, float* E, int B, void* stream);
int artalk_op_style_input(const float* motion, const float* mean, const float* std_, float* X, int B, void* stream);
int artalk_op_add_row(float* X, const float* v, int M, int D, void* stream);
int artalk_op_style_finish(const float* feat, const float* Ws, const float* bs, const float* null_cond, const uint8_t* has_style,
                           float* style_cond, int B, const float* cached, int64_t cached_stride, void* stream);
int artalk_op_broadcast16(const void* src, void* dst, int64_t bytes, int B, void* stream);
int artalk_op_session_gather(const float* const* slots_dev, float* style, float* prev_in, float* prev_fdec, int s16, int p16, int f16, int n,
                             void* stream);
int artalk_op_session_scatter(float* const* slots_dev, const float* style, const float* prev_in, const float* prev_fdec, int s16, int p16,
                              int f16, int n, int with_style, void* stream);
int artalk_op_savgol_stream(float* const* slots_dev, const float* raw, int64_t raw_stride, const int* seen, const int* n_frames,
                            const uint8_t* last, float* out, int64_t out_stride, int n, void* stream);
int artalk_op_session_smooth_check(const int64_t* open_ids, const int64_t* open_seen, const uint8_t* open_done, int n_open,
                                   const int64_t* ended_ids, int n_ended, const int64_t* ids, int n, int have_raw, int64_t raw_stride,
                                   const int* n_frames, const uint8_t* last, int64_t out_stride, int* first_out, int* count_out, char* msg,
                                   int msg_len);
int artalk_op_absmax(const float* buf, int rows, int cols, int64_t ld, int is_p8, int p8_exp, int junk_period, int junk_from,
                     unsigned int* slot_dev, void* stream);
typedef struct artalk_op_gemm_rows_args {
    int32_t mode, M, N, K, act;
    const void* A; int64_t lda, a_elems; int32_t a_exp;
    const float* W; int64_t ldw, w_elems;
    const float* bias; int64_t bias_elems;
    void* C; int64_t ldc, c_elems; int32_t cmap[3];
    const float* gate; int64_t ldg, gate_elems; int32_t gmap[3];
    const float* R; int64_t ldr, r_elems;
    int32_t c_p8, c_exp;
    int32_t force_cfg, splitk;
    int32_t ngrp; int64_t grpW, grpB, grpC;
    int32_t* status_dev;
    void* ln_Y; int64_t ln_ldy, ln_y_elems;
    const float* ln_scale; const float* ln_shift; int64_t ln_ldm, ln_mod_elems; int32_t ln_mmap[3];
    float ln_eps; int32_t ln_out_p8, ln_p8_exp;
    int32_t* used_cfg; int32_t* used_splitk; int32_t* fused_ln;
    int32_t cus;
} artalk_op_gemm_rows_args;
int artalk_op_gemm_rows(const artalk_op_gemm_rows_args* a, void* stream);
int artalk_op_gemm_rows_layout(int64_t* out, int n);
int artalk_op_rows_dry_run(int enable);
int artalk_op_layernorm_rows(const float* X, float* Y, const float* w, const float* b, const float* scale, const float* shift, int M,
                             int D, float eps, int act, int p8_exp, int junk_period, int junk_from, int* status_dev, int64_t ldx,
                             int64_t ldy, int64_t ldm, const int32_t* mmap, int64_t x_elems, int64_t y_elems, int64_t mod_elems,
                             void* stream);
int artalk_op_attention_rows(const float* Q, const float* K, const float* V, float* O, int B, int H, int HD, int Lq, int Lk,
                             float scale, int l2norm, const float* qscale, int split, int qkv_exp, int o_exp, int out_p8,
                             int* status_dev, int64_t ldq, int64_t ldk, int64_t ldv, int64_t ldo, int64_t q_bstride, int64_t k_bstride,
                             int64_t v_bstride, int64_t o_bstride, int64_t q_elems, int64_t k_elems, int64_t v_elems, int64_t o_elems,
                             void* stream);
#define ARTALK_ATTN_F32_64 0
#define ARTALK_ATTN_F32_32 1
// ... 27 lines not shown
```

Measured before the change: 104,500.

## Cache decoder history K/V for first chunk and decode only current half

For the first chunk, the VAE decoder's history half (100 frames) comes from a fixed initial history that is identical across clips. The change precomputes that half's per-layer K|V once per batch-group size and stores it. The first chunk then runs the decoder stack only on the 100 current rows, attending over the cached history keys. This removes about half of the first chunk's decoder work. In exchange it adds extra graph variants, extra workspace, a device sync during the fill, and cache invalidation logic.

```diff
diff --git a/artalk_amd/capi.py b/artalk_amd/capi.py
--- a/artalk_amd/capi.py
+++ b/artalk_amd/capi.py
@@ -25,6 +25,7 @@
     "artalk_op_w2v_front_rows", "artalk_op_pool_silu_rows", "artalk_op_posconv_rows",
     "artalk_op_attention_plan", "artalk_op_attention_rows_cus",
     "artalk_infer_samples", "artalk_set_tail_skip", "artalk_conv_tail_geometry", "artalk_conv_tail_class",
+    "artalk_set_decoder_split", "artalk_decoder_split_info",
 ]
 
 (ATTN_F32_64, ATTN_F32_32, ATTN_SHORT, ATTN_F16, ATTN_F16_P8, ATTN_F16_WIDE, ATTN_F16_PP, ATTN_F16_WIDE_AR,
@@ -153,6 +154,11 @@
         L.artalk_conv_tail_geometry.restype = i32
         L.artalk_conv_tail_class.argtypes = [i64, i32]
         L.artalk_conv_tail_class.restype = i64
+    if hasattr(L, "artalk_set_decoder_split"):
+        L.artalk_set_decoder_split.argtypes = [vp, i32]
+        L.artalk_set_decoder_split.restype = i32
+        L.artalk_decoder_split_info.argtypes = [vp, C.POINTER(i32), C.POINTER(i32), C.POINTER(i32)]
+        L.artalk_decoder_split_info.restype = i32
     L.artalk_get_status.argtypes = [vp, C.POINTER(C.c_int), vp]
     L.artalk_get_status.restype = i32
     L.artalk_poll_status.argtypes = [vp, C.POINTER(C.c_int)]
diff --git a/artalk_amd/csrc/ar_glue.hip b/artalk_amd/csrc/ar_glue.hip
--- a/artalk_amd/csrc/ar_glue.hip
+++ b/artalk_amd/csrc/ar_glue.hip
@@ -214,6 +214,38 @@
     ARTALK_LAUNCH(dec_input_kernel, dim3(B, 8), dim3(256), 0, s, prev_fdec, fhat, bits, dpos, X);
 }
 
+__global__ __launch_bounds__(256) void dec_input_half_kernel(const float* __restrict__ prev_fdec, const float* __restrict__ fhat,
+                                                             const uint8_t* __restrict__ bits, const float* __restrict__ dpos,
+                                                             float* __restrict__ X, int cur, const uint4* __restrict__ kv_src,
+                                                             uint4* __restrict__ kv_dst, long kv_lstride, int H) {
+    const int b = blockIdx.x;
+    if (blockIdx.y >= 8) {
+        const int l = (blockIdx.y - 8) >> 2, q = (blockIdx.y - 8) & 3;
+        const int w16 = 2 * H / 4;
+        const uint4* src = kv_src + (long)l * T100 * w16;
+        uint4* dst = kv_dst + ((long)l * kv_lstride + (long)b * 2 * T100 * 3 * H + H) / 4;
+        for (int i = q * 256 + threadIdx.x; i < T100 * w16; i += 4 * 256) dst[(long)(i / w16) * (3 * H / 4) + i % w16] = src[i];
+        return;
+    }
+    for (int idx = blockIdx.y * 256 + threadIdx.x; idx < T100 * CD; idx += 8 * 256) {
+        float v;
+        if (!cur) {
+            v = prev_fdec[(long)b * T100 * CD + idx];
+        } else {
+            const int tt = idx / CD, c = idx % CD;
+            const float h = bits[((long)b * 181 + 81 + tt) * CD + c] ? c_hq : -c_hq;
+            v = fhat[(long)b * T100 * CD + tt * CD + c] + h;
+        }
+        X[(long)b * T100 * CD + idx] = v + dpos[cur * T100 * CD + idx];
+    }
+}
+void launch_dec_input_half(const float* prev_fdec, const float* fhat, const uint8_t* bits, const float* dpos, float* X, int cur, int B,
+                           hipStream_t s, const float* kv_src, float* kv_dst, long kv_lstride, int H, int n_layers) {
+    if (!kv_src) n_layers = 0;
+    ARTALK_LAUNCH(dec_input_half_kernel, dim3(B, 8 + 4 * n_layers), dim3(256), 0, s, prev_fdec, fhat, bits, dpos, X, cur,
+                  reinterpret_cast<const uint4*>(kv_src), reinterpret_cast<uint4*>(kv_dst), kv_lstride, H);
+}
+
 __global__ __launch_bounds__(256) void dec_finish_kernel(const float* __restrict__ dec, const float* __restrict__ mean,
                                                          const float* __restrict__ stdv, const float* __restrict__ epos,
                                                          float* __restrict__ out, long out_bstride, int chunk,
diff --git a/artalk_amd/csrc/engine.hip b/artalk_amd/csrc/engine.hip
--- a/artalk_amd/csrc/engine.hip
+++ b/artalk_amd/csrc/engine.hip
@@ -97,6 +97,7 @@
     float** sess_slots = nullptr;
     float *prev_fdec = nullptr, *msfeat = nullptr, *dec_x = nullptr, *vh = nullptr, *vln = nullptr, *vqkv = nullptr;
     float *vatt = nullptr, *vmlp = nullptr, *dec_out = nullptr, *enc_in = nullptr, *enc_out = nullptr, *motion_chunk = nullptr;
+    float* dkv = nullptr;
     float *s_in = nullptr, *s_h = nullptr, *s_qkv = nullptr, *s_att = nullptr, *s_ffn = nullptr, *s_tmp = nullptr;
     int64_t bytes = 0;
 };
@@ -132,7 +133,16 @@
     std::map<const int*, int> site_of;
     bool stream_scales_ended = false;
     struct InitHistory { uint8_t* bits = nullptr; float *fdec = nullptr, *msfeat = nullptr; bool valid = false; } init_hist[3];
-    void invalidate_init_hist() { for (auto& ih : init_hist) ih.valid = false; }
+    struct HistKV { int group = 0; float* kv = nullptr; bool valid = false; };
+    static constexpr size_t kMaxHistKV = 16;
+    std::vector<HistKV> hist_kv[3];
+    bool decoder_split = true;
+    bool hist_initial = false;
+    bool body_hist_cached = false;
+    void invalidate_init_hist() {
+        for (auto& ih : init_hist) ih.valid = false;
+        for (auto& v : hist_kv) for (auto& e : v) e.valid = false;
+    }
     float* tap = nullptr; int tap_B = 0, tap_maxch = 0, tap_chunk = 0;
     std::vector<uint32_t> cu_mask;
     int n_cus = 0;
@@ -678,35 +688,67 @@
                         style_motion, (long)L * c.motion_dim);
 }
 
-void run_vae_stack(artalk_model* m, const VAESide& S, int B, int T, int split, hipStream_t s) {
+struct StackRows {
+    int plan_M = 0;
+    int rows = 0;
+    int row0 = 0;
+    float* qkv = nullptr;
+    long qkv_layer = 0;
+    float* kv_out = nullptr;
+};
+
+void run_vae_stack(artalk_model* m, const VAESide& S, int B, int T, int split, hipStream_t s, const StackRows* f = nullptr) {
     const artalk_config& c = m->cfg;
     Workspace& w = m->view ? *m->view : m->ws;
-    const int H = c.vae_hidden, M = B * T, F = H * 3 / 2;
+    const int R = f && f->rows ? f->rows : T;
+    const bool part = R != T;
+    const int H = c.vae_hidden, M = B * R, F = H * 3 / 2;
+    const int plan_M = f ? f->plan_M : 0;
     const int p8 = m->precision == 1 ? 1 : 0;
     const int AP = p8 ? LF_A_P8 : 0;
     const int sd = &S == &m->enc ? 0 : 1;
     for (int i = 0; i < c.vae_depth; ++i) {
         const VAELayer& L = S.layers[i];
         SiteExps::VAE& E = m->ex.vae[sd][i];
-        layernorm(w.vh, w.vln, L.lnw, L.lnb, M, H, 1e-5f, ACT_NONE, s, p8, w.status, 0, 0, E.ln);
+        const bool last = i + 1 == c.vae_depth;
+        {
+            LnArgs n;
+            n.X = w.vh; n.ldx = H; n.Y = w.vln; n.ldy = H; n.w = L.lnw; n.b = L.lnb; n.M = M; n.D = H; n.eps = 1e-5f; n.plan_M = plan_M;
+            n.out_p8 = p8; n.p8_exp = E.ln; n.status = p8 ? w.status : nullptr;
+            launch_layernorm(n, s);
+        }
         audit(m, w.vln, M, H, H, p8, s, &E.ln);
-        linear(m, w.vln, H, L.qkv_w, nullptr, w.vqkv, 3 * H, M, 3 * H, H, ACT_NONE, nullptr, s, AP | (p8 ? LF_C_P8 : 0), nullptr, E.ln, E.qkv);
+        float* qkv = f && f->qkv ? f->qkv + i * f->qkv_layer : w.vqkv;
+        {
+            GemmArgs q;
+            q.A = w.vln; q.lda = H; q.W = L.qkv_w; q.ldw = H; q.C = qkv; q.ldc = 3 * H; q.ldr = 3 * H; q.M = M; q.N = 3 * H; q.K = H;
+            q.a_packed = p8; q.c_p8 = p8; q.a_exp = E.ln; q.c_exp = E.qkv;
+            if (part) q.cmap = rowmap(R, T, f->row0);
+            gemm(m, q, s, nullptr, plan_M);
+        }
+        if (f && f->kv_out) {
+            (void)hipMemcpy2DAsync(f->kv_out + (long)i * T * 2 * H, (size_t)2 * H * 4, qkv + H, (size_t)3 * H * 4, (size_t)2 * H * 4, (size_t)B * T,
+                                   hipMemcpyDeviceToDevice, s);
+            if (last) break;
+        }
+        const int q0 = part ? f->row0 : 0;
         AttnArgs a;
         a.qkv_p8 = p8; a.qkv_exp = E.qkv; a.o_exp = E.attn;
-        a.Q = w.vqkv; a.K = w.vqkv + H; a.V = w.vqkv + 2 * H; a.ldq = a.ldk = a.ldv = 3 * H;
+        a.Q = qkv + (long)q0 * 3 * H; a.K = qkv + H; a.V = qkv + 2 * H; a.ldq = a.ldk = a.ldv = 3 * H;
         a.q_bstride = a.k_bstride = a.v_bstride = (long)T * 3 * H;
-        a.O = w.vatt; a.ldo = H; a.o_bstride = (long)T * H;
-        a.B = B; a.H = c.vae_heads; a.HD = H / c.vae_heads; a.Lq = T; a.Lk = T;
+        a.O = w.vatt; a.ldo = H; a.o_bstride = (long)R * H;
+        a.B = B; a.H = c.vae_heads; a.HD = H / c.vae_heads; a.Lq = R; a.Lk = T;
         a.scale = 1.0f / std::sqrt((float)H);
-        audit(m, w.vqkv, M, 3 * H, 3 * H, p8, s, &E.qkv);
-        a.split_q = split; a.split_k = split; a.out_p8 = p8; a.split16 = p8; a.status = p8 ? w.status : nullptr; a.cus = m->n_cus;
+        audit(m, qkv, M, 3 * H, 3 * H, p8, s, &E.qkv);
+        if (!part) { a.split_q = split; a.split_k = split; }
+        a.out_p8 = p8; a.split16 = p8; a.status = p8 ? w.status : nullptr; a.cus = m->n_cus;
         launch_attention(a, s);
         audit(m, w.vatt, M, H, H, p8, s, &E.attn);
-        linear(m, w.vatt, H, L.out_w, L.out_b, w.vh, H, M, H, H, ACT_NONE, w.vh, s, AP, p8 ? w.vln : nullptr, E.attn, E.resid);
+        linear(m, w.vatt, H, L.out_w, L.out_b, w.vh, H, M, H, H, ACT_NONE, w.vh, s, AP, p8 ? w.vln : nullptr, E.attn, E.resid, plan_M);
         audit(m, p8 ? w.vln : w.vh, M, H, H, p8, s, &E.resid);
-        linear(m, p8 ? w.vln : w.vh, H, L.m1_w, L.m1_b, w.vmlp, F, M, F, H, ACT_GELU_TANH, nullptr, s, p8 ? (LF_A_P8 | LF_C_P8) : 0, nullptr, E.resid, E.mlp);
+        linear(m, p8 ? w.vln : w.vh, H, L.m1_w, L.m1_b, w.vmlp, F, M, F, H, ACT_GELU_TANH, nullptr, s, p8 ? (LF_A_P8 | LF_C_P8) : 0, nullptr, E.resid, E.mlp, plan_M);
         audit(m, w.vmlp, M, F, F, p8, s, &E.mlp);
-        linear(m, w.vmlp, F, L.m2_w, L.m2_b, w.vh, H, M, H, F, ACT_NONE, w.vh, s, AP, nullptr, E.mlp);
+        linear(m, w.vmlp, F, L.m2_w, L.m2_b, w.vh, H, M, H, F, ACT_NONE, w.vh, s, AP, nullptr, E.mlp, kActExp, plan_M);
     }
 }
 
@@ -751,6 +793,30 @@
     launch_broadcast16(ih.fdec, w.prev_fdec, nf, B, s);
     launch_broadcast16(ih.msfeat, w.msfeat, nm, B, s);
     launch_vq_embed(w.msfeat, kNTok - 1, m->vq_w, m->vq_b, m->prev_lvl_pos + kE, w.prev_in, kNTok, 1, w.style_cond, m->prev_lvl_pos, B, s);
+    return ARTALK_OK;
+}
+
+const artalk_model::HistKV* find_hist_kv(const artalk_model* m, int group) {
+    for (const auto& e : m->hist_kv[m->precision])
+        if (e.group == group) return e.valid ? &e : nullptr;
+    return nullptr;
+}
+int fill_hist_kv(artalk_model* m, artalk_model::HistKV& e, hipStream_t s) {
+    const artalk_config& c = m->cfg;
+    Workspace& w = m->ws;
+    const int H = c.vae_hidden;
+    kbucket(m, KB_VAE_DEC);
+    launch_dec_input_half(m->init_hist[m->precision].fdec, nullptr, nullptr, m->dec_pos, w.dec_x, 0, 1, s);
+    linear(m, w.dec_x, c.code_dim, m->dec.in_w, m->dec.in_b, w.vh, H, 100, H, c.code_dim, ACT_LEAKY02, nullptr, s, 0, nullptr, m->ex.vae_dec_in,
+           kActExp, e.group * 200);
+    StackRows f;
+    f.plan_M = e.group * 200; f.kv_out = e.kv;
+    run_vae_stack(m, m->dec, 1, 100, 0, s, &f);
+    kbucket(m, KB_OTHER);
+    int flags[4] = {0, 0, 0, 0};
+    HIPCHK(m, hipMemcpyAsync(flags, w.status, sizeof(int), hipMemcpyDeviceToHost, s));
+    HIPCHK(m, hipStreamSynchronize(s));
+    e.valid = flags[0] == 0;
     return ARTALK_OK;
 }
 
@@ -859,12 +925,27 @@
     const int H = c.vae_hidden;
     roctxRangePushA("artalk.vae.decode");
     kbucket(m, KB_VAE_DEC);
-    launch_dec_input(w.prev_fdec, w.fhat, w.bits, m->dec_pos, w.dec_x, B, s);
-    audit(m, w.dec_x, B * 200, c.code_dim, c.code_dim, false, s, &ex.vae_dec_in);
-    linear(m, w.dec_x, c.code_dim, m->dec.in_w, m->dec.in_b, w.vh, H, B * 200, H, c.code_dim, ACT_LEAKY02, nullptr, s, 0, nullptr, ex.vae_dec_in);
-    run_vae_stack(m, m->dec, B, 200, 100, s);
-    audit(m, w.vh, B * 200, H, H, false, s, &ex.vae_dec_head);
-    linear(m, w.vh, H, m->dec.out_w, m->dec.out_b, w.dec_out, c.motion_dim, B * 200, c.motion_dim, H, ACT_NONE, nullptr, s, 0, nullptr, ex.vae_dec_head);
+    const artalk_model::HistKV* hk = m->body_hist_cached ? find_hist_kv(m, B) : nullptr;
+    if (hk) {
+        const long dkv_l = (long)w.maxB * 200 * 3 * H;
+        launch_dec_input_half(nullptr, w.fhat, w.bits, m->dec_pos, w.dec_x, 1, B, s, hk->kv, w.dkv, dkv_l, H, c.vae_depth);
+        linear(m, w.dec_x, c.code_dim, m->dec.in_w, m->dec.in_b, w.vh, H, B * 100, H, c.code_dim, ACT_LEAKY02, nullptr, s, 0, nullptr, ex.vae_dec_in,
+               kActExp, B * 200);
+        StackRows f;
+        f.plan_M = B * 200; f.rows = 100; f.row0 = 100; f.qkv = w.dkv; f.qkv_layer = dkv_l;
+        run_vae_stack(m, m->dec, B, 200, 100, s, &f);
+        GemmArgs o;
+        o.A = w.vh; o.lda = H; o.W = m->dec.out_w; o.ldw = H; o.bias = m->dec.out_b; o.C = w.dec_out; o.ldc = c.motion_dim; o.ldr = c.motion_dim;
+        o.cmap = rowmap(100, 200, 100); o.M = B * 100; o.N = c.motion_dim; o.K = H; o.a_exp = ex.vae_dec_head;
+        gemm(m, o, s, nullptr, B * 200);
+    } else {
+        launch_dec_input(w.prev_fdec, w.fhat, w.bits, m->dec_pos, w.dec_x, B, s);
+        audit(m, w.dec_x, B * 200, c.code_dim, c.code_dim, false, s, &ex.vae_dec_in);
+        linear(m, w.dec_x, c.code_dim, m->dec.in_w, m->dec.in_b, w.vh, H, B * 200, H, c.code_dim, ACT_LEAKY02, nullptr, s, 0, nullptr, ex.vae_dec_in);
+        run_vae_stack(m, m->dec, B, 200, 100, s);
+        audit(m, w.vh, B * 200, H, H, false, s, &ex.vae_dec_head);
+        linear(m, w.vh, H, m->dec.out_w, m->dec.out_b, w.dec_out, c.motion_dim, B * 200, c.motion_dim, H, ACT_NONE, nullptr, s, 0, nullptr, ex.vae_dec_head);
+    }
     tap_copy(m, TAP_DEC_OUT, 0, w.dec_out, 200, c.motion_dim, B, s);
     launch_dec_finish(w.dec_out, m->vae_mean, m->vae_std, m->enc_pos, w.motion_chunk, 100L * c.motion_dim, 0, w.enc_in, B, s, w.status);
     roctxRangePop();
@@ -885,6 +966,7 @@
     v.prev_fdec += b * 100 * c.code_dim; v.msfeat += b * 180 * c.code_dim; v.dec_x += b * 200 * c.code_dim;
     const long H = c.vae_hidden;
     v.vh += b * 200 * H; v.vln += b * 200 * H; v.vqkv += b * 200 * 3 * H; v.vatt += b * 200 * H; v.vmlp += b * 200 * H * 3 / 2;
+    v.dkv += b * 200 * 3 * H;
     v.dec_out += b * 200 * c.motion_dim; v.enc_in += b * 100 * 128; v.enc_out += b * 100 * c.code_dim;
     v.motion_chunk += b * 100 * c.motion_dim;
     v.splitk = m->ws.splitk_b[branch];
@@ -938,42 +1020,83 @@
         const int gsz = g.b0[h + 1] - g.b0[h];
         const int need = std::max(0, std::min(n_next - g.b0[h], gsz));
         g.nre[h] = g.graphs ? std::min(gsz, (need + 7) / 8 * 8) : need;
-        g.key[h] = ((long long)(((B * 8 + g.n) * 4 + h) * 3 + m->precision)) * 4096 + g.nre[h];
+        g.key[h] = (((long long)(((B * 8 + g.n) * 4 + h) * 3 + m->precision)) * 4096 + g.nre[h]) * 2;
     }
     return g;
+}
+int hist_kv_ready(artalk_model* m, int B, int n_next, bool fill, hipStream_t s, bool* ready) {
+    *ready = false;
+    if (!m->decoder_split || m->audit || m->tap || B <= 0 || n_next != B) return ARTALK_OK;
+    const artalk_config& c = m->cfg;
+    if (c.vae_hidden % 8 || c.patch_nums[c.n_levels - 1] != 100) return ARTALK_OK;
+    if (fill && !m->init_hist[m->precision].valid) return ARTALK_OK;
+    const BodyGroups g = plan_body(m, B, n_next);
+    auto& tab = m->hist_kv[m->precision];
+    for (int h = 0; h < g.n; ++h) {
+        const int gsz = g.b0[h + 1] - g.b0[h];
+        if (find_hist_kv(m, gsz)) continue;
+        if (!fill) return ARTALK_OK;
+        auto it = std::find_if(tab.begin(), tab.end(), [gsz](const artalk_model::HistKV& e) { return e.group == gsz; });
+        if (it == tab.end()) {
+            if (tab.size() >= artalk_model::kMaxHistKV) return ARTALK_OK;
+            artalk_model::HistKV e;
+            e.group = gsz; e.kv = dalloc<float>(m, (int64_t)c.vae_depth * 100 * 2 * c.vae_hidden);
+            if (!e.kv) return fail(m, ARTALK_EHIP, "hipMalloc failed for the decoder's history K|V cache");
+            HIPCHK(m, hipDeviceSynchronize());
+            tab.push_back(e);
+            it = tab.end() - 1;
+        }
+        if (int rc = fill_hist_kv(m, *it, s)) return rc;
+        if (!it->valid) return ARTALK_OK;
+    }
+    *ready = true;
+    return ARTALK_OK;
 }
 int run_body(artalk_model* m, int B, hipStream_t s, int n_next) {
     const BodyGroups g = plan_body(m, B, n_next);
+    const bool cached = m->body_hist_cached;
     const bool fork = g.n > 1 && m->profiling != 3;
     if (fork) { if (int rc = ensure_side_streams(m, g.n - 1)) return rc; }
     hipStream_t st[4] = {s, s, s, s};
     for (int h = 1; fork && h < g.n; ++h) st[h] = m->side_stream[h - 1];
     Workspace views[4];
     for (int h = 0; h < g.n; ++h) views[h] = clip_view(m, g.b0[h], h);
-    auto launch_group = [&](int h) { m->view = &views[h]; run_chunk_body(m, g.b0[h + 1] - g.b0[h], st[h], g.nre[h]); m->view = nullptr; };
-    for (int h = 0; g.graphs && h < g.n; ++h) {
-        auto hit = m->graphs.find(g.key[h]);
-        if (hit != m->graphs.end()) { hit->second.last_use = ++m->graph_clock; continue; }
-        if (int rc = evict_graphs(m, g.key, g.n)) return rc;
+    auto launch_group = [&](int h, bool form_cached) {
+        m->view = &views[h]; m->body_hist_cached = form_cached;
+        run_chunk_body(m, g.b0[h + 1] - g.b0[h], st[h], g.nre[h]);
+        m->view = nullptr;
+    };
+    long long keys[8];
+    for (int h = 0; h < g.n; ++h) { keys[h] = g.key[h] + (cached ? 1 : 0); keys[g.n + h] = g.key[h]; }
+    auto capture = [&](int h, bool form_cached) -> int {
+        const long long key = g.key[h] + (form_cached ? 1 : 0);
+        auto hit = m->graphs.find(key);
+        if (hit != m->graphs.end()) { hit->second.last_use = ++m->graph_clock; return (int)ARTALK_OK; }
+        if (int rc = evict_graphs(m, keys, 2 * g.n)) return rc;
         hipGraph_t graph = nullptr;
         hipGraphExec_t exec = nullptr;
         HIPCHK(m, hipStreamBeginCapture(st[h], hipStreamCaptureModeThreadLocal));
         m->in_graph_body = true;
-        launch_group(h);
+        launch_group(h, form_cached);
         m->in_graph_body = false;
         HIPCHK(m, hipStreamEndCapture(st[h], &graph));
         HIPCHK(m, hipGraphInstantiate(&exec, graph, nullptr, nullptr, 0));
         (void)hipGraphDestroy(graph);
-        m->graphs.emplace(g.key[h], artalk_model::GraphEntry{exec, ++m->graph_clock});
+        m->graphs.emplace(key, artalk_model::GraphEntry{exec, ++m->graph_clock});
         ++m->graph_captures;
+        return (int)ARTALK_OK;
+    };
+    for (int h = 0; g.graphs && h < g.n; ++h) {
+        if (int rc = capture(h, cached)) return rc;
+        if (cached) { if (int rc = capture(h, false)) return rc; }
     }
     if (fork) {
         HIPCHK(m, hipEventRecord(m->fork_ev, s));
         for (int h = 1; h < g.n; ++h) HIPCHK(m, hipStreamWaitEvent(st[h], m->fork_ev, 0));
     }
     for (int h = 0; h < g.n; ++h) {
-        if (g.graphs) HIPCHK(m, hipGraphLaunch(m->graphs[g.key[h]].exec, st[h]));
-        else launch_group(h);
+        if (g.graphs) HIPCHK(m, hipGraphLaunch(m->graphs[keys[h]].exec, st[h]));
+        else launch_group(h, cached);
     }
     for (int h = 1; fork && h < g.n; ++h) {
         HIPCHK(m, hipEventRecord(m->join_ev[h - 1], st[h]));
@@ -1070,6 +1193,7 @@
     const int H = c.vae_hidden;
     w.dec_x = F((int64_t)maxB * 200 * c.code_dim); w.vh = F((int64_t)maxB * 200 * H); w.vln = F((int64_t)maxB * 200 * H);
     w.vqkv = F((int64_t)maxB * 200 * 3 * H); w.vatt = F((int64_t)maxB * 200 * H); w.vmlp = F((int64_t)maxB * 200 * H * 3 / 2);
+    w.dkv = F((int64_t)c.vae_depth * maxB * 200 * 3 * H);
     w.dec_out = F((int64_t)maxB * 200 * c.motion_dim); w.enc_in = F((int64_t)maxB * 100 * 128);
     w.enc_out = F((int64_t)maxB * 100 * c.code_dim); w.motion_chunk = F((int64_t)maxB * 100 * c.motion_dim);
     const int S = c.style_dim, SL = c.style_len;
@@ -1172,9 +1296,12 @@
     stage_mark(m, s, PB_STYLE);
     return ARTALK_OK;
 }
-int chunk_step(artalk_model* m, hipStream_t s, int cond_row0, int Bn, int n_next, int tap_chunk, float* out_motion_dev, int64_t out_stride) {
+int chunk_step(artalk_model* m, hipStream_t s, int cond_row0, int Bn, int n_next, int tap_chunk, float* out_motion_dev, int64_t out_stride,
+               bool initial_hist = false) {
     Workspace& w = m->ws;
     m->tap_chunk = tap_chunk;
+    m->body_hist_cached = false;
+    if (initial_hist) { if (int rc = hist_kv_ready(m, Bn, n_next, false, s, &m->body_hist_cached)) return rc; }
     roctxRangePushA("artalk.ar.adaln_table");
     kbucket(m, KB_ADA);
     linear(m, w.silu_cond + (long)cond_row0 * kNTok * kCond, kCond, m->ada_w, m->ada_b, w.ada, m->ada_n, Bn * kNTok, m->ada_n, kCond,
@@ -1498,6 +1625,7 @@
     HIPCHK(m, hipDeviceSynchronize());
     if (m->precision == 2) { if (int rc = ensure_bf16_copy(m)) return rc; }
     m->finalized = true;
+    m->invalidate_init_hist();
     return ARTALK_OK;
 }
 
@@ -1520,6 +1648,23 @@
     return ARTALK_OK;
 }
 int artalk_set_tail_skip(artalk_model* m, int on) { if (!m) return ARTALK_EINVAL; m->tail_skip = on != 0; return ARTALK_OK; }
+int artalk_set_decoder_split(artalk_model* m, int on) {
+    if (!m) return ARTALK_EINVAL;
+    if (m->decoder_split == (on != 0)) return ARTALK_OK;
+    (void)hipSetDevice(m->device); (void)hipDeviceSynchronize();
+    m->decoder_split = on != 0;
+    drop_graphs(m);
+    return ARTALK_OK;
+}
+int artalk_decoder_split_info(artalk_model* m, int* on, int* entries, int* valid) {
+    if (!m) return ARTALK_EINVAL;
+    if (on) *on = m->decoder_split ? 1 : 0;
+    int n = 0, v = 0;
+    for (const auto& e : m->hist_kv[m->precision]) { ++n; v += e.valid ? 1 : 0; }
+    if (entries) *entries = n;
+    if (valid) *valid = v;
+    return ARTALK_OK;
+}
 int artalk_set_graphs(artalk_model* m, int enable) {
     if (!m) return ARTALK_EINVAL;
     m->use_graphs = (enable & 0xff) != 0;
@@ -1760,6 +1905,8 @@
     for (int c0 = 0, gi = 0; c0 < C; c0 += w.G, ++gi)
         run_wav2vec(m, audio_dev, c0, (int)std::min<int64_t>(w.G, C - c0), out_w2v_dev, s, !passes.empty() && passes[gi].np ? &passes[gi] : nullptr);
     if (int rc = run_init_history(m, B, s)) return rc;
+    bool kv_ready = false;
+    if (maxch > 0) { if (int rc = hist_kv_ready(m, Bj[0], out_hist_bits_dev ? Bj[0] : (maxch > 1 ? Bj[1] : 0), true, s, &kv_ready)) return rc; }
     const size_t bits_row = (size_t)kNTok * c.code_dim;
     if (out_hist_bits_dev)
         HIPCHK(m, hipMemcpy2DAsync(out_hist_bits_dev, (size_t)(maxch + 1) * bits_row, w.hist_bits, bits_row, bits_row, B,
@@ -1768,7 +1915,7 @@
     for (int64_t j = 0; j < maxch; ++j) {
         const int Bn = Bj[j];
         const int n_next = out_hist_bits_dev ? Bn : (j + 1 < maxch ? Bj[j + 1] : 0);
-        if (int rc = chunk_step(m, s, base[j], Bn, n_next, (int)j, out_motion_dev + j * 100 * c.motion_dim, out_clip_stride)) return rc;
+        if (int rc = chunk_step(m, s, base[j], Bn, n_next, (int)j, out_motion_dev + j * 100 * c.motion_dim, out_clip_stride, j == 0)) return rc;
         if (out_bits_dev)
             HIPCHK(m, hipMemcpy2DAsync(out_bits_dev + j * bits_row, (size_t)maxch * bits_row, w.bits, bits_row, bits_row, Bn,
                                        hipMemcpyDeviceToDevice, s));
@@ -1815,8 +1962,10 @@
         ProfilingOff quiet(m);
         if (int rc = begin_clips(m, s, B, style_motion_dev, has_style, encode_style, stg)) return rc;
         if (int rc = run_init_history(m, B, s)) return rc;
-    }
-    m->stream_B = B; m->stream_scales_ended = false;
+        bool kv_ready = false;
+        if (int rc = hist_kv_ready(m, B, B, true, s, &kv_ready)) return rc;
+    }
+    m->stream_B = B; m->stream_scales_ended = false; m->hist_initial = true;
     if (int rc = publish_status(m, s)) return rc;
     return ARTALK_OK;
 }
@@ -1840,7 +1989,9 @@
     stg->used = true;
     ProfilingOff quiet(m);
     for (int c0 = 0; c0 < B; c0 += w.G) run_wav2vec(m, audio_dev, c0, std::min(w.G, B - c0), nullptr, s);
-    if (int rc = chunk_step(m, s, 0, B, B, m->tap_maxch, out_motion_dev, out_stride)) return rc;
+    const bool first = m->hist_initial;
+    m->hist_initial = false;
+    if (int rc = chunk_step(m, s, 0, B, B, m->tap_maxch, out_motion_dev, out_stride, first)) return rc;
     if (int rc = publish_status(m, s)) return rc;
     return ARTALK_OK;
 }
diff --git a/artalk_amd/csrc/kernels.h b/artalk_amd/csrc/kernels.h
--- a/artalk_amd/csrc/kernels.h
+++ b/artalk_amd/csrc/kernels.h
@@ -162,6 +162,9 @@
 void launch_ar_begin(const float* style_cond, const float* lvlpos, float* x0, float* fhat, int B, hipStream_t s);
 void launch_dec_input(const float* prev_fdec, const float* fhat, const uint8_t* bits, const float* dpos, float* X,
                       int B, hipStream_t s);
+void launch_dec_input_half(const float* prev_fdec, const float* fhat, const uint8_t* bits, const float* dpos, float* X, int cur, int B,
+                           hipStream_t s, const float* kv_src = nullptr, float* kv_dst = nullptr, long kv_lstride = 0, int H = 0,
+                           int n_layers = 0);
 void launch_dec_finish(const float* dec , const float* mean, const float* stdv, const float* epos,
                        float* out, long out_bstride, int chunk, float* E, int B, hipStream_t s, int* status = nullptr);
 void launch_enc_input_zero(const float* mean, const float* stdv, const float* epos, float* E, int B, hipStream_t s);
diff --git a/artalk_amd/model.py b/artalk_amd/model.py
--- a/artalk_amd/model.py
+++ b/artalk_amd/model.py
@@ -346,6 +346,16 @@
     def set_tail_skip(self, on: bool):
         if capi.lib().artalk_set_tail_skip(self._h, int(bool(on))) != capi.OK:
             raise RuntimeError("artalk_set_tail_skip failed")
+
+    def set_decoder_split(self, on: bool):
+        if capi.lib().artalk_set_decoder_split(self._h, int(bool(on))) != capi.OK:
+            raise RuntimeError("artalk_set_decoder_split failed")
+
+    def decoder_split_info(self):
+        v = [C.c_int(0) for _ in range(3)]
+        if capi.lib().artalk_decoder_split_info(self._h, *[C.byref(x) for x in v]) != capi.OK:
+            raise RuntimeError("artalk_decoder_split_info failed")
+        return bool(v[0].value), int(v[1].value), int(v[2].value)
 
     def graph_count(self):
         n = C.c_longlong(0)
diff --git a/include/artalk_hip.h b/include/artalk_hip.h
--- a/include/artalk_hip.h
+++ b/include/artalk_hip.h
@@ -52,6 +52,8 @@
                          const int64_t* n_samples, int B, const float* style_motion_dev, const uint8_t* has_style, float* out_motion_dev,
                          int64_t out_clip_stride, uint8_t* out_bits_dev, uint8_t* out_hist_bits_dev, float* out_w2v_dev, void* stream);
 int artalk_set_tail_skip(artalk_model* m, int on);
+int artalk_set_decoder_split(artalk_model* m, int on);
+int artalk_decoder_split_info(artalk_model* m, int* on, int* entries, int* valid);
 int artalk_conv_tail_geometry(int64_t valid, int samples_per_chunk, int n_conv, const int* kernel, const int* stride, int* t_const,
                               int* Tp, int* Sp, int* samples_read);
 int64_t artalk_conv_tail_class(int64_t valid, int samples_per_chunk);
```

After: 104,900 (median of 6 runs). About the same (+0.4%).
